# aclike/dynamic_multiview_3d

Measured on AMD Instinct MI355X. Metric: train images/sec, appearance-flow encoder-decoder 128x128x3 (fwd+bwd+Adam), higher is better.
Workload: dtype bf16x3; 1 GPU; appflow_offset: AppearanceFlowModel 128x128x3, batch 64 per GPU, Adam lr 1e-4, random-init weights (reference initialisers); global_batch=64, parallelism=dp1

## Files before the change

dynamic_multiview_3d_amd/_lib.py:

```python
import ctypes as C
import os

HERE = os.path.dirname(os.path.abspath(__file__))
LIB_PATH = os.environ.get("MV3D_LIB") or os.path.join(HERE, "libmv3d_hip.so")

ACT_NONE, ACT_LRELU, ACT_RELU, ACT_TANH = 0, 1, 2, 3
ACT_BY_NAME = {None: ACT_NONE, 'none': ACT_NONE, 'lrelu': ACT_LRELU, 'relu': ACT_RELU, 'tanh': ACT_TANH}
F32 = 0


class ConvGeom(C.Structure):
    _fields_ = [(n, C.c_int32) for n in
                ("N", "H", "W", "C", "Ho", "Wo", "K", "kh", "kw", "sh", "sw", "img_ld", "feat_ld", "dtype")]


class Epilogue(C.Structure):
    _fields_ = [("bias", C.c_void_p), ("act", C.c_int32), ("leak", C.c_float), ("gmask_act", C.c_int32),
                ("gmask_leak", C.c_float), ("gmask_ref", C.c_void_p), ("gmask_ld", C.c_int32)]


class FcChainLayer(C.Structure):
    _fields_ = [("M", C.c_void_p), ("bias", C.c_void_p), ("y", C.c_void_p), ("y_ld", C.c_int32), ("out", C.c_int32),
                ("act", C.c_int32), ("leak", C.c_float)]


class FcChain(C.Structure):
    _fields_ = [("B", C.c_int32), ("nlayers", C.c_int32), ("in_", C.c_int32), ("x_ld", C.c_int32), ("x", C.c_void_p),
                ("l", FcChainLayer * 4)]


class Mv3dError(RuntimeError):
    pass


_vp, _i, _i64, _f, _sz = C.c_void_p, C.c_int, C.c_int64, C.c_float, C.c_size_t
_G, _E = C.POINTER(ConvGeom), C.POINTER(Epilogue)

STATUS_FUNCS = {
    "mv3d_conv2d_fwd": [_G, _vp, _vp, _vp, _E, _vp, _sz, _vp],
    "mv3d_conv2d_dgrad": [_G, _vp, _vp, _vp, _E, _vp, _sz, _vp],
    "mv3d_conv2d_wgrad": [_G, _vp, _vp, _vp, _vp, _vp, _sz, _vp],
    "mv3d_deconv2d_fwd": [_G, _vp, _vp, _vp, _E, _vp, _sz, _vp],
    "mv3d_deconv2d_dgrad": [_G, _vp, _vp, _vp, _E, _vp, _sz, _vp],
    "mv3d_deconv2d_wgrad": [_G, _vp, _vp, _vp, _vp, _sz, _vp],
    "mv3d_fc_fwd": [_i, _i, _i, _vp, _i, _vp, _vp, _i, _E, _vp, _sz, _vp],
    "mv3d_fc_dgrad": [_i, _i, _i, _vp, _i, _vp, _vp, _i, _E, _vp, _sz, _vp],
    "mv3d_fc_wgrad": [_i, _i, _i, _vp, _i, _vp, _i, _vp, _vp, _vp, _sz, _vp],
    "mv3d_fc_wgrad_dgrad": [_i, _i, _i, _vp, _i, _vp, _i, _vp, _vp, _vp, _vp, _i, _E, _vp, _sz, _vp],
    "mv3d_fc_chain_fwd": [C.POINTER(FcChain), _vp],
    "mv3d_act_fwd": [_i64, _i, _vp, _i, _vp, _i, _i, _f, _vp],
    "mv3d_act_bwd": [_i64, _i, _vp, _i, _vp, _i, _vp, _i, _i, _f, _vp],
    "mv3d_copy2d": [_i64, _i, _vp, _i64, _i64, _vp, _i64, _i, _vp],
    "mv3d_group_sum": [_i64, _i, _i, _vp, _i64, _vp, _i64, _vp],
    "mv3d_warp_resample_fwd": [_i, _i, _i, _i, _i, _i, _vp, _vp, _i, _vp, _vp, _vp],
    "mv3d_warp_resample_bwd": [_i, _i, _i, _i, _i, _i, _vp, _vp, _i, _vp, _vp, _i, _vp],
    "mv3d_warp_resample_loss": [_i, _i, _i, _i, _i, _i, _vp, _vp, _i, _vp, _i, _i, _f, _vp, _vp, _vp, _i, _vp, _vp],
    "mv3d_resampler_fwd": [_i, _i, _i, _i, _i, _vp, _i, _vp, _i, _vp, _i, _vp],
    "mv3d_resampler_bwd": [_i, _i, _i, _i, _i, _vp, _i, _vp, _i, _vp, _i, _vp, _i, _vp, _i, _vp, _sz, _vp],
    "mv3d_image_metrics": [_i, _i, _i, _i, _vp, _i, _vp, _i, _f, _vp, _vp, _sz, _vp],
    "mv3d_ssim_loss": [_i, _i, _i, _i, _vp, _i, _vp, _i, _f, _f, _vp, _vp, _i, _i, _vp, _sz, _vp],
    "mv3d_flow_smoothness": [_i, _i, _i, _vp, _i, _vp, _i, _i, _f, _f, _f, _vp, _vp, _i, _i, _vp, _sz, _vp],
    "mv3d_pixel_loss": [_i64, _i, _vp, _vp, _vp, _i, _f, _vp, _vp, _vp],
    "mv3d_loss_overwrite_next": [],
    "mv3d_pixel_loss_strided": [_i64, _i, _vp, _i, _vp, _i, _f, _vp, _i, _i, _f, _vp, _vp, _i, _vp],
    "mv3d_tfrecord_open": [C.c_char_p, _i, C.POINTER(_vp)],
    "mv3d_tfrecord_read": [_vp, _i, _i, _i, C.POINTER(C.c_char_p), C.POINTER(C.c_int), C.POINTER(C.c_size_t), C.POINTER(_vp), C.POINTER(C.c_int)],
    "mv3d_u8_to_unit_f32": [_i64, _vp, _vp, _vp],
    "mv3d_u8_process_image": [_vp, _i, _i, _i, _i, _vp, _i, _i, _vp],
    "mv3d_fill": [_vp, _i64, _f, _vp],
    "mv3d_adam_step": [_i64, _vp, _vp, _vp, _vp, _f, _f, _f, _f, _f, _f, _f, _vp],
    "mv3d_adam_step_dev": [_i64, _vp, _vp, _vp, _vp, _vp, _i, C.POINTER(_i64), C.POINTER(_i64), _vp],
    "mv3d_adam_advance": [_vp, _vp],
    "mv3d_fc_wgrad_adam": [_i, _i, _i, _vp, _i, _vp, _i, _vp, _vp, _vp, _vp, _vp, _vp],
    "mv3d_sgd_step": [_i64, _vp, _vp, _vp, _f, _f, _i, _f, _vp],
    "mv3d_sgd_step_dev": [_i64, _vp, _vp, _vp, _vp, _i, C.POINTER(_i64), C.POINTER(_i64), _vp],
    "mv3d_fc_wgrad_sgd": [_i, _i, _i, _vp, _i, _vp, _i, _vp, _vp, _vp, _vp, _vp],
    "mv3d_grad_finalize_begin": [],
    "mv3d_grad_finalize_add": [_vp, _i64],
    "mv3d_grad_finalize_commit": [_vp, _sz, _vp, _vp, _vp, _vp, _vp, _vp],
    "mv3d_grad_finalize_commit_sgd": [_vp, _sz, _vp, _vp, _vp, _vp, _vp],
    "mv3d_grad_finalize_abort": [],
    "mv3d_comm_unique_id": [_vp],
    "mv3d_comm_init": [C.POINTER(_vp), _i, _i, _vp],
    "mv3d_comm_destroy": [_vp],
    "mv3d_comm_allreduce_sum": [_vp, _vp, _i64, _vp],
    "mv3d_comm_reduce_scatter_sum": [_vp, _vp, _vp, _i64, _vp],
    "mv3d_comm_allgather": [_vp, _vp, _vp, _i64, _vp],
    "mv3d_ipc_export": [_vp, _vp, C.POINTER(_i64)],
    "mv3d_ipc_open": [_vp, C.POINTER(_vp)],
    "mv3d_ipc_close": [_vp],
    "mv3d_mesh_reduce_sum": [C.POINTER(_vp), _i, _vp, _i64, _vp],
    "mv3d_mesh_copy": [_vp, _vp, _i64, _vp],
    "mv3d_filter_cache_bind": [_G, _i, _vp, _vp, _sz],
    "mv3d_filter_cache_commit": [_vp, _sz, _vp],
    "mv3d_filter_cache_refresh": [_vp],
    "mv3d_filter_cache_clear": [],
    "mv3d_plan_begin": [_vp],
    "mv3d_plan_end": [],
    "mv3d_plan_run": [_vp, _vp],
    "mv3d_plan_run_range": [_vp, _i, _i, _vp],
    "mv3d_plan_run_range_multi": [_vp, _i, _i, _vp, C.POINTER(_vp), _i, _i],
    "mv3d_plan_side": [_i],
    "mv3d_plan_profile": [_vp, _i],
    "mv3d_plan_profile_collect": [_vp],
    "mv3d_plan_profile_select": [_vp, C.c_char_p],
    "mv3d_plan_profile_reset": [_vp],
    "mv3d_plan_op_info": [_vp, _i, C.POINTER(C.c_char_p), C.POINTER(C.c_double), C.POINTER(C.c_double),
                          C.POINTER(C.c_double), C.POINTER(C.c_int)],
}
OTHER_FUNCS = {
    "mv3d_version": (C.c_char_p, []),
    "mv3d_last_error": (C.c_char_p, []),
    "mv3d_conv_workspace_bytes": (_sz, [_G]),
    "mv3d_conv_wgrad_workspace_bytes": (_sz, [_G]),
    "mv3d_fc_workspace_bytes": (_sz, [_i, _i, _i]),
    "mv3d_resampler_bwd_workspace_bytes": (_sz, [_i, _i, _i, _i, _i]),
    "mv3d_image_metrics_workspace_bytes": (_sz, [_i, _i, _i, _i]),
    "mv3d_ssim_loss_workspace_bytes": (_sz, [_i, _i, _i, _i]),
    "mv3d_flow_smoothness_workspace_bytes": (_sz, [_i, _i, _i]),
    "mv3d_crc32c": (C.c_uint32, [_vp, _sz]),
    "mv3d_set_diagnostics": (C.c_int, [_i]),
    "mv3d_set_wgrad_cus": (C.c_int, [_i]),
    "mv3d_tfrecord_close": (None, [_vp]),
    "mv3d_filter_prepared_bytes": (_sz, [_G, _i]),
    "mv3d_filter_cache_table_bytes": (_sz, []),
    "mv3d_grad_finalize_table_bytes": (_sz, []),
    "mv3d_plan_create": (_vp, []),
    "mv3d_plan_destroy": (None, [_vp]),
    "mv3d_plan_size": (_i, [_vp]),
    "mv3d_comm_available": (_i, []),
    "mv3d_fc_wgrad_adam_supported": (_i, [_i, _i, _i, _i, _i]),
    "mv3d_debug_cconv_stamps": (_i, [_vp, _sz]),
    "mv3d_debug_cwgrad_stamps": (_i, [_vp, _sz]),
    "mv3d_debug_band_stamps": (_i, [_vp, _sz]),
}
EXPORTS = sorted(list(STATUS_FUNCS) + list(OTHER_FUNCS))

_lib = None


class _Checked:

    def __init__(self, name, fn, dll):
        self.name, self.fn, self.dll = name, fn, dll

    def __call__(self, *args):
        rc = self.fn(*args)
        if rc != 0:
            raise Mv3dError("%s failed (%d): %s" % (self.name, rc, self.dll.mv3d_last_error().decode()))
        return rc


class _Lib:
    def __init__(self, path):
        if not os.path.exists(path):
            raise Mv3dError("%s not found: build it with `python -m dynamic_multiview_3d_amd.build` "
                            "(hipcc --offload-arch=gfx950); there is no fallback path" % path)
        import torch
        self.dll = C.CDLL(path)
        for name, (res, args) in OTHER_FUNCS.items():
            fn = getattr(self.dll, name)
            fn.restype, fn.argtypes = res, args
            if name[5:] != 'last_error':
                setattr(self, name[5:], fn)
        for name, args in STATUS_FUNCS.items():
            fn = getattr(self.dll, name)
            fn.restype, fn.argtypes = C.c_int, args
            setattr(self, name[5:], _Checked(name, fn, self.dll))
            setattr(self, "raw_" + name[5:], fn)

    def last_error(self):
        return self.dll.mv3d_last_error().decode()


def lib():
    global _lib
    if _lib is None:
        _lib = _Lib(LIB_PATH)
    return _lib


def plan_ops(plan):
    l = lib()
    out = []
    for i in range(l.plan_size(plan)):
        name, fl, by, ms, runs = C.c_char_p(), C.c_double(), C.c_double(), C.c_double(), C.c_int()
        l.plan_op_info(plan, i, C.byref(name), C.byref(fl), C.byref(by), C.byref(ms), C.byref(runs))
        out.append((name.value.decode(), fl.value, by.value, ms.value, runs.value))
    return out


def epilogue(bias=None, act=ACT_NONE, leak=0.2, gmask_act=ACT_NONE, gmask_leak=0.2, gmask_ref=None, gmask_ld=0):
    return Epilogue(bias, act, leak, gmask_act, gmask_leak, gmask_ref, gmask_ld)


def conv_geom(N, H, W, Cc, K, kh, kw, sh, sw, img_ld=None, feat_ld=None):
    Ho, Wo = -(-H // sh), -(-W // sw)
    return ConvGeom(N, H, W, Cc, Ho, Wo, K, kh, kw, sh, sw, Cc if img_ld is None else img_ld,
                    K if feat_ld is None else feat_ld, F32)
```

dynamic_multiview_3d_amd/csrc/common.h:

```cpp
#pragma once
#include <hip/hip_runtime.h>
#include <stdint.h>
#include <stdlib.h>
#include <functional>
#include "../../include/mv3d_hip.h"

namespace mv3d {

int fail(int code, const char* fmt, ...) __attribute__((format(printf, 2, 3)));
struct OpInfo {
    const char* name;
    double flops;
    double bytes;
};

const char* intern_label(const char* fmt, ...) __attribute__((format(printf, 1, 2)));

bool recording();
bool take_loss_overwrite();
void record(std::function<int(hipStream_t)> fn, const OpInfo& info);

enum OptKind { OPT_NONE = 0, OPT_ADAM = 1, OPT_MOMENTUM = 2, OPT_GD = 3 };

__device__ __forceinline__ void momentum_elem(float g, float& p, float& a, float lr, float mu, bool nesterov) {
#pragma clang fp contract(off)
    a = a * mu + g;
    if (nesterov) p = p - (g * lr + (a * mu) * lr);
    else p = p - a * lr;
}
__device__ __forceinline__ void gd_elem(float g, float& p, float lr) {
#pragma clang fp contract(off)
    p = p - g * lr;
}

template <class F>
inline int dispatch(void* stream, const OpInfo& info, F fn) {
    if (recording()) { record(std::function<int(hipStream_t)>(fn), info); return MV3D_OK; }
    return fn(reinterpret_cast<hipStream_t>(stream));
}

inline int launched(const char* what) {
    hipError_t e = hipGetLastError();
    if (e != hipSuccess) return fail(MV3D_E_HIP, "%s: %s", what, hipGetErrorString(e));
    return MV3D_OK;
}

struct FinSegHost { const float* part; int nslab; int64_t count; float* out; };
bool finalize_collecting();
void finalize_push(const float* part, int nslab, int64_t count, float* out);
void finalize_open();
}
#include <vector>
namespace mv3d {
const std::vector<FinSegHost>* finalize_peek();
void finalize_take(std::vector<FinSegHost>* out);

int disabled_paths();

static inline int cdiv(int a, int b) { return (a + b - 1) / b; }
static inline int64_t cdiv64(int64_t a, int64_t b) { return (a + b - 1) / b; }

static inline void same_pad(int size, int k, int s, int* out, int* before) {
    int o = (size + s - 1) / s;
    int total = (o - 1) * s + k - size;
    if (total < 0) total = 0;
    *out = o;
    *before = total / 2;
}

__device__ __forceinline__ float act_apply(float x, int act, float leak) {
    if (act == MV3D_ACT_LRELU) {
        float f1 = 0.5f * (1.0f + leak), f2 = 0.5f * (1.0f - leak);
        return __fadd_rn(__fmul_rn(f1, x), __fmul_rn(f2, fabsf(x)));
    }
    if (act == MV3D_ACT_RELU) {
        float y = __fadd_rn(__fmul_rn(0.5f, x), __fmul_rn(0.5f, fabsf(x)));
        return x < 0.0f ? -0.0f : y;
    }
    if (act == MV3D_ACT_TANH) return tanhf(x);
    return x;
}

__device__ __forceinline__ float act_grad_from_out(float y, int act, float leak) {
    if (act == MV3D_ACT_LRELU) {
        float f1 = 0.5f * (1.0f + leak), f2 = 0.5f * (1.0f - leak);
        float s = (y > 0.0f) ? 1.0f : ((y < 0.0f) ? -1.0f : 0.0f);
        return f1 + f2 * s;
    }
    if (act == MV3D_ACT_RELU) {
        if (y > 0.0f) return 1.0f;
        return (__float_as_uint(y) >> 31) ? 0.0f : 0.5f;
    }
    if (act == MV3D_ACT_TANH) return 1.0f - y * y;
    return 1.0f;
}

typedef float f32x16 __attribute__((ext_vector_type(16)));
typedef float f32x4 __attribute__((ext_vector_type(4)));

}
```

dynamic_multiview_3d_amd/csrc/conv.hip:

```cpp
#include "conv_common.h"
#include "reduce_common.h"
#include <algorithm>

namespace mv3d {

template <int WM, int MT, int NT, bool VEC, bool BKMAJOR>
__global__ __launch_bounds__(256) void igemm_kernel(const IgemmParams p) {
    constexpr int BK = 32;
    constexpr int WN = 4 / WM;
    constexpr int BM = WM * 32 * MT;
    constexpr int BN = WN * 32 * NT;
    constexpr int LDA = BK + 1;
    constexpr int LDB = BN + 1;
    constexpr int A_PASSES = VEC ? BM / 32 : BM / 8;
    constexpr int B_LOADS = BK * BN / 256;

    __shared__ float As[BM * LDA];
    __shared__ float Bs[BK * LDB];
    __shared__ int s_rowbase[BM], s_ih0[BM], s_iw0[BM], s_outpix[BM];

    const int tid = threadIdx.x;
    const int lane = tid & 63, wave = tid >> 6;
    const int li = lane & 31, lh = lane >> 5;
    const int wm = wave / WN, wn = wave % WN;
// ... 1225 lines not shown
            return dispatch(stream, OpInfo{"igemm_splitk_epilogue", 0.0, (double)total * 4.0 * (e.ksplit + 1)}, [=](hipStream_t s) {
                launch_splitk_epilogue(e, blocks, s);
                return launched("igemm_splitk_epilogue");
            });
        }
        if (hrc != 1) return hrc;
    }
    int cfg; dim3 grid;
    size_t need = igemm_plan(p, &cfg, &grid);
    if (need > ws_bytes || (need && !ws)) {
        p.ksplit = 1;
        grid.z = p.so_h * p.so_w;
        need = 0;
    }
    p.Part = (float*)ws;
    int rc = dispatch(stream, OpInfo{igemm_name(cfg, vec, bkmajor), flops, bytes}, [=](hipStream_t s) {
        if (cfg == 0) launch_igemm_cfg<4, 1, 1>(p, vec, bkmajor, grid, s);
        else if (cfg == 1) launch_igemm_cfg<4, 1, 2>(p, vec, bkmajor, grid, s);
        else launch_igemm_cfg<2, 1, 1>(p, vec, bkmajor, grid, s);
        return launched(who);
    });
    if (rc != MV3D_OK || p.ksplit == 1) return rc;
    const int64_t total = (int64_t)p.N * p.Hc * p.Wc * p.Cc;
    const int blocks = (int)std::min<int64_t>(cdiv64(total, 256), 4096);
    return dispatch(stream, OpInfo{"igemm_splitk_epilogue", 0.0, (double)total * 4.0 * (p.ksplit + 1)}, [=](hipStream_t s) {
        launch_splitk_epilogue(p, blocks, s);
        return launched("igemm_splitk_epilogue");
    });
}

static inline double conv_flops(const mv3d_conv_geom* g) {
    return 2.0 * g->N * g->Ho * g->Wo * g->kh * g->kw * (double)g->C * g->K;
}
static inline double conv_bytes(const mv3d_conv_geom* g) {
    return 4.0 * ((double)g->N * g->H * g->W * g->C + (double)g->N * g->Ho * g->Wo * g->K + (double)g->kh * g->kw * g->C * g->K);
}

static void i2f_params(const mv3d_conv_geom* g, IgemmParams& p, int* pt_out, int* pl_out) {
    int ho, wo, pt, pl;
    same_pad(g->H, g->kh, g->sh, &ho, &pt);
    same_pad(g->W, g->kw, g->sw, &wo, &pl);
    p.N = g->N; p.Ha = g->H; p.Wa = g->W; p.Ca = g->C; p.a_ld = g->img_ld;
    p.Hc = g->Ho; p.Wc = g->Wo; p.Cc = g->K; p.c_ld = g->feat_ld;
    p.sa_h = g->sh; p.sa_w = g->sw; p.so_h = 1; p.so_w = 1;
    p.Hp[0] = g->Ho; p.Wp[0] = g->Wo; p.Hp[1] = 0; p.Wp[1] = 0;
    p.fold = (g->C < 16 && g->img_ld == g->C && g->kw > 1) ? 1 : 0;
    int nt = 0;
    if (p.fold) {
        for (int pp = 0; pp < g->kh; ++pp) { p.taps[nt].dh = (int8_t)(pp - pt); p.taps[nt].dw = (int8_t)(-pl); p.taps[nt].widx = (int16_t)(pp * g->kw); ++nt; }
        p.Ka = g->kw * g->C;
    } else {
        for (int pp = 0; pp < g->kh; ++pp)
            for (int q = 0; q < g->kw; ++q) { p.taps[nt].dh = (int8_t)(pp - pt); p.taps[nt].dw = (int8_t)(q - pl); p.taps[nt].widx = (int16_t)(pp * g->kw + q); ++nt; }
        p.Ka = g->C;
    }
    p.tap_begin[0] = 0; p.tap_begin[1] = nt;
    p.w_tap_stride = g->C * g->K; p.w_ks = g->K; p.w_ns = 1;
    *pt_out = pt; *pl_out = pl;
}

static int img2feat(const mv3d_conv_geom* g, const void* img, const void* w, void* feat, const mv3d_epilogue* epi,
                    void* ws, size_t ws_bytes, void* stream, const char* who) {
    int rc = check_geom(g, who);
    if (rc == MV3D_OK) rc = check_epilogue(epi, who);
    if (rc != MV3D_OK) return rc;
    if (!img || !w || !feat) return fail(MV3D_E_INVAL, "%s: null tensor pointer", who);
    IgemmParams p = {};
    int pt, pl;
    i2f_params(g, p, &pt, &pl);
    p.A = (const float*)img; p.Wt = (const float*)w; p.Out = (float*)feat;
    fill_epilogue(p, epi);
    if (p.fold && g->C <= 4 && !(disabled_paths() & 64)) {
        const int brc = try_smallc_band(g, p, pt, pl, img, w, feat, stream, who, conv_flops(g), conv_bytes(g));
        if (brc != 1) return brc;
    }
    if (p.fold && g->C <= 4 && g->kw * g->C <= 20 && g->K <= 64 && !(disabled_paths() & 64)) {
        SmallCParams q = {};
        q.X = (const float*)img; q.Wt = (const float*)w; q.Y = (float*)feat;
        q.N = g->N; q.H = g->H; q.W = g->W; q.C = g->C; q.Ho = g->Ho; q.Wo = g->Wo; q.K = g->K; q.y_ld = g->feat_ld;
        q.kh = g->kh; q.kw = g->kw; q.sh = g->sh; q.sw = g->sw; q.pt = pt; q.pl = pl;
        q.wtiles = cdiv(g->Wo, 32);
        q.ep = p;
        const int items = g->N * g->Ho * q.wtiles;
        const bool two = g->K > 32;
        return dispatch(stream, OpInfo{two ? "smallc_img2feat<N64>" : "smallc_img2feat<N32>", conv_flops(g), conv_bytes(g)}, [=](hipStream_t s) {
            const bool b3 = !(disabled_paths() & 4096) && q.kw * q.C <= 16 && (q.kh == 5 || q.kh == 3) && !two;
            if (b3) {
                static int sc_blocks = -1;
                if (sc_blocks < 0) { const char* e = getenv("MV3D_SC_BLOCKS"); sc_blocks = e ? atoi(e) : 2048; }
                const int blocks = std::min(cdiv(items, 4), sc_blocks);
                auto pow2 = [](int v) { return v > 0 && (v & (v - 1)) == 0; };
                const bool lean = !(disabled_paths() & 8388608) && q.ep.gact == MV3D_ACT_NONE && q.Wo % 32 == 0 && q.K == 32 && pow2(q.wtiles) && pow2(q.Ho) &&
                                  (int64_t)q.N * q.H * q.W * q.C * 4 < 0x40000000 && (int64_t)q.N * q.Ho * q.Wo * q.y_ld * 4 < 0x7fffffff;
                if (lean) {
                    int ws_ = 0, hs_ = 0;
                    while ((1 << ws_) < q.wtiles) ++ws_;
                    while ((1 << hs_) < q.Ho) ++hs_;
                    if (q.kh == 5) smallc_b3s_kernel<5><<<blocks, 256, 0, s>>>(q, items, ws_, hs_);
                    else smallc_b3s_kernel<3><<<blocks, 256, 0, s>>>(q, items, ws_, hs_);
                } else if (q.kh == 5) smallc_b3_kernel<1, 5><<<blocks, 256, 0, s>>>(q, items);
                else smallc_b3_kernel<1, 3><<<blocks, 256, 0, s>>>(q, items);
            } else if (two) smallc_img2feat_kernel<2><<<cdiv(items, 4), 256, 0, s>>>(q);
            else smallc_img2feat_kernel<1><<<cdiv(items, 4), 256, 0, s>>>(q);
            return launched(who);
        });
    }
    return run_igemm(p, ws, ws_bytes, stream, who, conv_flops(g), conv_bytes(g));
}

static void f2i_params(const mv3d_conv_geom* g, IgemmParams& p) {
    int ho, wo, pt, pl;
    same_pad(g->H, g->kh, g->sh, &ho, &pt);
    same_pad(g->W, g->kw, g->sw, &wo, &pl);
    p.N = g->N; p.Ha = g->Ho; p.Wa = g->Wo; p.Ca = g->K; p.a_ld = g->feat_ld;
    p.Hc = g->H; p.Wc = g->W; p.Cc = g->C; p.c_ld = g->img_ld;
    p.sa_h = 1; p.sa_w = 1; p.so_h = g->sh; p.so_w = g->sw;
    for (int a = 0; a < 2; ++a) {
        p.Hp[a] = a < g->sh ? (g->H - a + g->sh - 1) / g->sh : 0;
        p.Wp[a] = a < g->sw ? (g->W - a + g->sw - 1) / g->sw : 0;
    }
    int nt = 0;
    for (int phh = 0; phh < g->sh; ++phh)
        for (int phw = 0; phw < g->sw; ++phw) {
            p.tap_begin[phh * g->sw + phw] = nt;
            const int p0 = (phh + pt) % g->sh, q0 = (phw + pl) % g->sw;
            for (int pp = p0; pp < g->kh; pp += g->sh)
                for (int q = q0; q < g->kw; q += g->sw) {
                    p.taps[nt].dh = (int8_t)((phh + pt - pp) / g->sh);
                    p.taps[nt].dw = (int8_t)((phw + pl - q) / g->sw);
                    p.taps[nt].widx = (int16_t)(pp * g->kw + q);
                    ++nt;
                }
        }
    p.tap_begin[g->sh * g->sw] = nt;
    p.fold = 0; p.Ka = g->K;
    p.w_tap_stride = g->C * g->K; p.w_ks = 1; p.w_ns = g->K;
}

static int feat2img(const mv3d_conv_geom* g, const void* feat, const void* w, void* img, const mv3d_epilogue* epi,
                    void* ws, size_t ws_bytes, void* stream, const char* who) {
    int rc = check_geom(g, who);
    if (rc == MV3D_OK) rc = check_epilogue(epi, who);
    if (rc != MV3D_OK) return rc;
    if (!img || !w || !feat) return fail(MV3D_E_INVAL, "%s: null tensor pointer", who);
    IgemmParams p = {};
    f2i_params(g, p);
    p.A = (const float*)feat; p.Wt = (const float*)w; p.Out = (float*)img;
    fill_epilogue(p, epi);
    return run_igemm(p, ws, ws_bytes, stream, who, conv_flops(g), conv_bytes(g));
}

struct WgTileParams;
bool wgrad_tile_plan(const mv3d_conv_geom* g, struct WgTileParams* out, int* nslab_out, int* cfg_out, size_t* lds_out);
int wgrad_tile_launch_erased(const mv3d_conv_geom* g, const void* img, const void* feat, void* out, void* bias_out, void* stream, const char* who, int* nslab_out);

static void filtgrad_plan(const mv3d_conv_geom* g, FiltgradParams& p, int* nt_out, int* nslab_out) {
    int ho, wo;
    same_pad(g->H, g->kh, g->sh, &ho, &p.pt);
    same_pad(g->W, g->kw, g->sw, &wo, &p.pl);
    p.N = g->N; p.H = g->H; p.W = g->W; p.C = g->C; p.img_ld = g->img_ld;
    p.Ho = g->Ho; p.Wo = g->Wo; p.K = g->K; p.feat_ld = g->feat_ld;
    p.kw = g->kw; p.sh = g->sh; p.sw = g->sw;
    p.fold = (g->C < 16 && g->img_ld == g->C && g->kw > 1) ? 1 : 0;
    p.Cf = p.fold ? g->kw * g->C : g->C;
    p.ntap = p.fold ? g->kh : g->kh * g->kw;
    const int NT = (g->K > 32) ? 2 : 1;
    p.ctiles = cdiv(p.Cf, 32);
    p.ktiles = cdiv(g->K, 32 * NT);
    p.rows_total = g->N * g->Ho;
    const int items = p.ctiles * p.ktiles * p.ntap;
    const int blocks_x = cdiv(items, 4);
    int nslab = cdiv(2048, blocks_x);
    if (nslab > p.rows_total) nslab = p.rows_total;
    int min_rows = cdiv(128, g->Wo);
    if (nslab > cdiv(p.rows_total, min_rows)) nslab = cdiv(p.rows_total, min_rows);
    if (nslab < 1) nslab = 1;
    p.rows_per_slab = cdiv(p.rows_total, nslab);
    nslab = cdiv(p.rows_total, p.rows_per_slab);
    *nt_out = NT;
    *nslab_out = nslab;
}

int wgrad_tile_nslab(const mv3d_conv_geom* g);
int set_wgrad_cus(int cus);

static size_t filtgrad_ws_bytes(const mv3d_conv_geom* g) {
    {
        const int tw = thin_wgrad_slabs(g);
        if (tw > 0) return (size_t)tw * ((size_t)g->kh * g->kw * g->C * g->K + g->K) * sizeof(float);
    }
    {
        ThinFgParams tp; int ns; size_t lds;
        if (thin_filtgrad_plan(g, tp, &ns, &lds)) return (size_t)ns * ((size_t)g->kh * g->kw * g->C * g->K + g->K) * sizeof(float);
    }
    FiltgradParams p = {};
    int NT, nslab;
    filtgrad_plan(g, p, &NT, &nslab);
    const int tiled = wgrad_tile_nslab(g);
    if (tiled > 0) nslab = tiled;
    if (nslab == 1) return 0;
    return (size_t)nslab * ((size_t)g->kh * g->kw * g->C * g->K + g->K) * sizeof(float);
}

static int filtgrad(const mv3d_conv_geom* g, const void* img, const void* feat, void* df, void* db,
                    void* ws, size_t ws_bytes, void* stream, const char* who) {
    int rc = check_geom(g, who);
    if (rc != MV3D_OK) return rc;
    if (!img || !feat || !df) return fail(MV3D_E_INVAL, "%s: null tensor pointer", who);
    const int64_t fcount = (int64_t)g->kh * g->kw * g->C * g->K;
    float* dfp = (float*)df; float* dbp = (float*)db;
    const int K = g->K;
    {
        const int tiled = wgrad_tile_nslab(g);
        if (tiled > 0 && (reinterpret_cast<uintptr_t>(img) & 15) == 0 && (reinterpret_cast<uintptr_t>(feat) & 15) == 0) {
            float* part = dfp; float* bpart = dbp;
            if (tiled > 1) {
                size_t need = (size_t)tiled * (fcount + K) * sizeof(float);
                if (!ws || ws_bytes < need) return fail(MV3D_E_WORKSPACE, "%s: workspace %zu < %zu bytes", who, ws_bytes, need);
                part = (float*)ws;
                bpart = db ? (float*)ws + (int64_t)tiled * fcount : nullptr;
            }
            int ns = 0;
            rc = wgrad_tile_launch_erased(g, img, feat, part, bpart, stream, who, &ns);
            if (rc == MV3D_OK && ns == 1 && finalize_collecting()) { finalize_push(nullptr, 0, fcount, dfp); if (dbp) finalize_push(nullptr, 0, K, dbp); }
            if (rc != MV3D_OK || ns == 1) return rc;
            return dispatch_reduce(stream, part, ns, fcount, dfp, bpart, K, dbp);
        }
    }
    {
        const int tw = thin_wgrad_slabs(g);
        if (tw > 0 && (reinterpret_cast<uintptr_t>(img) & 15) == 0) {
            const size_t need = (size_t)tw * (fcount + K) * sizeof(float);
            if (!ws || ws_bytes < need) return fail(MV3D_E_WORKSPACE, "%s: workspace %zu < %zu bytes", who, ws_bytes, need);
            float* part = (float*)ws;
            float* bpart = db ? (float*)ws + (int64_t)tw * fcount : nullptr;
            rc = thin_wgrad_launch(g, img, feat, part, bpart, stream, who, conv_flops(g), conv_bytes(g));
            if (rc == MV3D_OK) return dispatch_reduce(stream, part, tw, fcount, dfp, bpart, K, dbp);
            if (rc != 1) return rc;
        }
    }
    {
        ThinFgParams tp; int ns; size_t lds;
        if (thin_filtgrad_plan(g, tp, &ns, &lds) && (reinterpret_cast<uintptr_t>(feat) & 15) == 0) {
            const size_t need = (size_t)ns * (fcount + K) * sizeof(float);
            if (!ws || ws_bytes < need) return fail(MV3D_E_WORKSPACE, "%s: workspace %zu < %zu bytes", who, ws_bytes, need);
            tp.img = (const float*)img; tp.feat = (const float*)feat;
            tp.out = (float*)ws;
            tp.bias_out = db ? (float*)ws + (int64_t)ns * fcount : nullptr;
            dim3 grid(cdiv(g->K, 32), ns);
            const int nj = cdiv(tp.nrows, 16);
            rc = dispatch(stream, OpInfo{"thin_filtgrad", conv_flops(g), conv_bytes(g)}, [=](hipStream_t s) {
                if (nj <= 2) thin_filtgrad_kernel<2><<<grid, 256, lds, s>>>(tp);
                else if (nj <= 4) thin_filtgrad_kernel<4><<<grid, 256, lds, s>>>(tp);
                else if (nj <= 5) thin_filtgrad_kernel<5><<<grid, 256, lds, s>>>(tp);
                else thin_filtgrad_kernel<7><<<grid, 256, lds, s>>>(tp);
                return launched(who);
            });
            if (rc != MV3D_OK) return rc;
            return dispatch_reduce(stream, tp.out, ns, fcount, dfp, tp.bias_out, K, dbp);
        }
    }
    FiltgradParams p = {};
    int NT, nslab;
    filtgrad_plan(g, p, &NT, &nslab);
    p.img = (const float*)img; p.feat = (const float*)feat;
    if (nslab > 1) {
        size_t need = (size_t)nslab * (fcount + g->K) * sizeof(float);
        if (!ws || ws_bytes < need) return fail(MV3D_E_WORKSPACE, "%s: workspace %zu < %zu bytes", who, ws_bytes, need);
        p.out = (float*)ws;
        p.bias_out = db ? (float*)ws + (int64_t)nslab * fcount : nullptr;
    } else {
        p.out = (float*)df;
        p.bias_out = (float*)db;
    }
    dim3 grid(cdiv(p.ctiles * p.ktiles * p.ntap, 4), nslab);
    rc = dispatch(stream, OpInfo{NT == 2 ? "filtgrad<NT=2>" : "filtgrad<NT=1>", conv_flops(g), conv_bytes(g)}, [=](hipStream_t s) {
        const bool wide = p.Wo >= 16;
        if (NT == 2) { if (wide) filtgrad_kernel<2, 8><<<grid, 256, 0, s>>>(p); else filtgrad_kernel<2, 2><<<grid, 256, 0, s>>>(p); }
        else { if (wide) filtgrad_kernel<1, 8><<<grid, 256, 0, s>>>(p); else filtgrad_kernel<1, 2><<<grid, 256, 0, s>>>(p); }
        return launched(who);
    });
    if (rc == MV3D_OK && nslab == 1 && finalize_collecting()) { finalize_push(nullptr, 0, fcount, dfp); if (dbp) finalize_push(nullptr, 0, K, dbp); }
    if (rc != MV3D_OK || nslab == 1) return rc;
    return dispatch_reduce(stream, p.out, nslab, fcount, dfp, p.bias_out, K, dbp);
}

}

using namespace mv3d;

extern "C" {

int mv3d_conv2d_fwd(const mv3d_conv_geom* g, const void* x, const void* w, void* y, const mv3d_epilogue* epi,
                    void* ws, size_t wsb, void* stream) {
    return img2feat(g, x, w, y, epi, ws, wsb, stream, "mv3d_conv2d_fwd");
}
int mv3d_conv2d_dgrad(const mv3d_conv_geom* g, const void* dy, const void* w, void* dx, const mv3d_epilogue* epi,
                      void* ws, size_t wsb, void* stream) {
    return feat2img(g, dy, w, dx, epi, ws, wsb, stream, "mv3d_conv2d_dgrad");
}
int mv3d_conv2d_wgrad(const mv3d_conv_geom* g, const void* x, const void* dy, void* dw, void* db,
                      void* ws, size_t wsb, void* stream) {
    return filtgrad(g, x, dy, dw, db, ws, wsb, stream, "mv3d_conv2d_wgrad");
}
int mv3d_deconv2d_fwd(const mv3d_conv_geom* g, const void* x, const void* w, void* y, const mv3d_epilogue* epi,
                      void* ws, size_t wsb, void* stream) {
    return feat2img(g, x, w, y, epi, ws, wsb, stream, "mv3d_deconv2d_fwd");
}
int mv3d_deconv2d_dgrad(const mv3d_conv_geom* g, const void* dy, const void* w, void* dx, const mv3d_epilogue* epi,
                        void* ws, size_t wsb, void* stream) {
    return img2feat(g, dy, w, dx, epi, ws, wsb, stream, "mv3d_deconv2d_dgrad");
}
int mv3d_deconv2d_wgrad(const mv3d_conv_geom* g, const void* x, const void* dy, void* dw, void* ws, size_t wsb, void* stream) {
    return filtgrad(g, dy, x, dw, nullptr, ws, wsb, stream, "mv3d_deconv2d_wgrad");
}

static bool filter_op_params(const mv3d_conv_geom* g, int op, const void* w, IgemmParams& p, const char* who) {
    if (!g || check_geom(g, who) != MV3D_OK) return false;
    if (op == MV3D_FILTER_CONV_FWD || op == MV3D_FILTER_DECONV_DGRAD) { int pt, pl; i2f_params(g, p, &pt, &pl); }
    else if (op == MV3D_FILTER_CONV_DGRAD || op == MV3D_FILTER_DECONV_FWD) f2i_params(g, p);
    else { fail(MV3D_E_INVAL, "%s: unknown filter operation %d", who, op); return false; }
    p.Wt = (const float*)w;
    return true;
}

size_t mv3d_filter_prepared_bytes(const mv3d_conv_geom* g, int op) {
    IgemmParams p = {};
    if (!filter_op_params(g, op, nullptr, p, "mv3d_filter_prepared_bytes")) return 0;
    if (disabled_paths() & (1 | 4096)) return 0;
    return bconv_prepared_bytes(p);
}

int mv3d_filter_cache_bind(const mv3d_conv_geom* g, int op, const void* w, void* prepared, size_t prepared_bytes) {
    IgemmParams p = {};
    if (!w) return fail(MV3D_E_INVAL, "mv3d_filter_cache_bind: null filter pointer");
    if (!filter_op_params(g, op, w, p, "mv3d_filter_cache_bind")) return MV3D_E_INVAL;
    int rc = bconv_cache_bind(p, prepared, prepared_bytes);
    if (rc == 1) return fail(MV3D_E_UNSUPPORTED, "mv3d_filter_cache_bind: this operation does not take a prepared filter");
    return rc;
}

int mv3d_set_wgrad_cus(int cus) { return set_wgrad_cus(cus); }

size_t mv3d_conv_wgrad_workspace_bytes(const mv3d_conv_geom* g) {
    if (!g || check_geom(g, "mv3d_conv_wgrad_workspace_bytes") != MV3D_OK) return 0;
    return filtgrad_ws_bytes(g);
}

size_t mv3d_conv_workspace_bytes(const mv3d_conv_geom* g) {
    if (!g || check_geom(g, "mv3d_conv_workspace_bytes") != MV3D_OK) return 0;
    size_t out_img = (size_t)g->N * g->H * g->W * g->C, out_feat = (size_t)g->N * g->Ho * g->Wo * g->K;
    size_t big = out_img > out_feat ? out_img : out_feat;
    size_t igemm = 0;
    {
        IgemmParams p = {};
        int cfg; dim3 grid;
        p.N = g->N; p.Hc = g->Ho; p.Wc = g->Wo; p.Cc = g->K; p.so_h = p.so_w = 1; p.Hp[0] = g->Ho; p.Wp[0] = g->Wo;
        const bool fold = (g->C < 16 && g->img_ld == g->C && g->kw > 1);
        p.Ka = fold ? g->kw * g->C : g->C; p.tap_begin[0] = 0; p.tap_begin[1] = fold ? g->kh : g->kh * g->kw;
        size_t a = igemm_plan(p, &cfg, &grid);
        igemm = a;
        (void)big;
        IgemmParams q = {};
        q.N = g->N; q.Hc = g->H; q.Wc = g->W; q.Cc = g->C; q.so_h = g->sh; q.so_w = g->sw;
        for (int i = 0; i < 2; ++i) { q.Hp[i] = i < g->sh ? (g->H - i + g->sh - 1) / g->sh : 0; q.Wp[i] = i < g->sw ? (g->W - i + g->sw - 1) / g->sw : 0; }
        q.Ka = g->K;
        int ho, wo, pt, pl;
        same_pad(g->H, g->kh, g->sh, &ho, &pt);
        same_pad(g->W, g->kw, g->sw, &wo, &pl);
        int nt = 0;
        for (int phh = 0; phh < g->sh; ++phh)
            for (int phw = 0; phw < g->sw; ++phw) {
                q.tap_begin[phh * g->sw + phw] = nt;
                for (int pp = (phh + pt) % g->sh; pp < g->kh; pp += g->sh)
                    for (int qq = (phw + pl) % g->sw; qq < g->kw; qq += g->sw) ++nt;
            }
        q.tap_begin[g->sh * g->sw] = nt;
        size_t b = igemm_plan(q, &cfg, &grid);
        if (b > igemm) igemm = b;
    }
    size_t fg = filtgrad_ws_bytes(g);
    size_t filt = (size_t)g->kh * g->kw * ((g->C + 63) / 64 * 64) * ((g->K + 63) / 64 * 64) * sizeof(float);
    size_t m = igemm > fg ? igemm : fg;
    const size_t big_out = out_img > out_feat ? out_img : out_feat;
    size_t small = 0;
    if ((size_t)g->Ho * g->Wo <= 64 || (size_t)g->H * g->W <= 64) small = ((filt + 255) & ~(size_t)255) + 16 * big_out * sizeof(float);
    m = m > small ? m : small;
    return m > filt ? m : filt;
}

static void fc_geom(mv3d_conv_geom& g, int B, int in, int out, int x_ld, int y_ld) {
    g.N = 1; g.H = 1; g.W = B; g.C = in; g.Ho = 1; g.Wo = B; g.K = out;
    g.kh = g.kw = g.sh = g.sw = 1; g.img_ld = x_ld; g.feat_ld = y_ld; g.dtype = MV3D_F32;
}
int mv3d_fc_fwd(int B, int in, int out, const void* x, int x_ld, const void* M, void* y, int y_ld,
                const mv3d_epilogue* epi, void* ws, size_t wsb, void* stream) {
    mv3d_conv_geom g; fc_geom(g, B, in, out, x_ld, y_ld);
    if (B > 0 && in > 0 && out > 0 && x && M && y && is_small_fc(B, in, out)) {
        int rc = check_epilogue(epi, "mv3d_fc_fwd");
        if (rc != MV3D_OK) return rc;
        IgemmParams ep = {}; fill_epilogue(ep, epi);
        return dispatch(stream, OpInfo{"small_fc_fwd", 2.0 * B * in * out, 4.0 * (B * in + in * out + B * out)}, [=](hipStream_t s) {
            small_fc_fwd_kernel<<<cdiv(B * out, 256), 256, 0, s>>>(B, in, out, (const float*)x, x_ld, (const float*)M, (float*)y, y_ld, ep);
            return launched("small_fc_fwd_kernel");
        });
    }
    if (B > 0 && in > 0 && out > 0 && x && M && y && x_ld >= in && y_ld >= out && check_epilogue(epi, "mv3d_fc_fwd") == MV3D_OK) {
        int rc = try_fc_stream(false, B, in, out, x, x_ld, M, y, y_ld, epi, ws, wsb, stream, "mv3d_fc_fwd", fill_epilogue, launch_splitk_epilogue);
        if (rc != 1) return rc;
    }
    return img2feat(&g, x, M, y, epi, ws, wsb, stream, "mv3d_fc_fwd");
}
int mv3d_fc_dgrad(int B, int in, int out, const void* dy, int dy_ld, const void* M, void* dx, int dx_ld,
                  const mv3d_epilogue* epi, void* ws, size_t wsb, void* stream) {
    mv3d_conv_geom g; fc_geom(g, B, in, out, dx_ld, dy_ld);
    if (B > 0 && in > 0 && out > 0 && dy && M && dx && is_small_fc(B, in, out)) {
        int rc = check_epilogue(epi, "mv3d_fc_dgrad");
        if (rc != MV3D_OK) return rc;
        IgemmParams ep = {}; fill_epilogue(ep, epi);
        return dispatch(stream, OpInfo{"small_fc_dgrad", 2.0 * B * in * out, 4.0 * (B * in + in * out + B * out)}, [=](hipStream_t s) {
            small_fc_dgrad_kernel<<<cdiv(B * in, 256), 256, 0, s>>>(B, in, out, (const float*)dy, dy_ld, (const float*)M, (float*)dx, dx_ld, ep);
            return launched("small_fc_dgrad_kernel");
        });
    }
    if (B > 0 && in > 0 && out > 0 && dy && M && dx && dy_ld >= out && dx_ld >= in && check_epilogue(epi, "mv3d_fc_dgrad") == MV3D_OK) {
        int rc = try_fc_stream(true, B, in, out, dy, dy_ld, M, dx, dx_ld, epi, ws, wsb, stream, "mv3d_fc_dgrad", fill_epilogue, launch_splitk_epilogue);
        if (rc != 1) return rc;
    }
    return feat2img(&g, dy, M, dx, epi, ws, wsb, stream, "mv3d_fc_dgrad");
}
int mv3d_fc_wgrad(int B, int in, int out, const void* x, int x_ld, const void* dy, int dy_ld, void* dM, void* db,
                  void* ws, size_t wsb, void* stream) {
    mv3d_conv_geom g; fc_geom(g, B, in, out, x_ld, dy_ld);
    if (B > 0 && in > 0 && out > 0 && x && dy && dM && is_small_fc(B, in, out)) {
        return dispatch(stream, OpInfo{"small_fc_wgrad", 2.0 * B * in * out, 4.0 * (B * in + in * out + B * out)}, [=](hipStream_t s) {
            small_fc_wgrad_kernel<<<cdiv((in + 1) * out, 256), 256, 0, s>>>(B, in, out, (const float*)x, x_ld, (const float*)dy, dy_ld, (float*)dM, (float*)db);
            return launched("small_fc_wgrad_kernel");
        });
    }
    if (B > 0 && in > 0 && out > 0 && x && dy && dM && x_ld >= in && dy_ld >= out) {
        int rc = try_fc_wgrad(B, in, out, x, x_ld, dy, dy_ld, dM, db, stream, "mv3d_fc_wgrad");
        if (rc != 1) return rc;
    }
    return filtgrad(&g, x, dy, dM, db, ws, wsb, stream, "mv3d_fc_wgrad");
}
int mv3d_fc_wgrad_dgrad(int B, int in, int out, const void* x, int x_ld, const void* dy, int dy_ld, const void* M,
                        void* dM, void* db, void* dx, int dx_ld, const mv3d_epilogue* dx_epi, void* ws, size_t wsb, void* stream) {
    if (B > 0 && in > 0 && out > 0 && x && dy && M && dM && dx && is_small_fc(B, in, out)) {
        int rc = check_epilogue(dx_epi, "mv3d_fc_wgrad_dgrad");
        if (rc != MV3D_OK) return rc;
        IgemmParams ep = {}; fill_epilogue(ep, dx_epi);
        const int wblocks = cdiv((in + 1) * out, 256), dblocks = cdiv(B * in, 256);
        const size_t lds = ((size_t)B * out + std::max((size_t)B * in, (size_t)in * (out + 1))) * sizeof(float);
        if (lds <= 64 * 1024) {
            (void)hipFuncSetAttribute(reinterpret_cast<const void*>(&small_fc_bwd_kernel), hipFuncAttributeMaxDynamicSharedMemorySize, 64 * 1024);
            (void)hipGetLastError();
        }
        if (lds <= 64 * 1024)
        return dispatch(stream, OpInfo{"small_fc_bwd", 4.0 * B * in * out, 4.0 * (2.0 * B * in + 2.0 * in * out + 2.0 * B * out)}, [=](hipStream_t s) {
            small_fc_bwd_kernel<<<wblocks + dblocks, 256, lds, s>>>(B, in, out, (const float*)x, x_ld, (const float*)dy, dy_ld, (const float*)M,
                                                                  (float*)dM, (float*)db, (float*)dx, dx_ld, ep, wblocks);
            return launched("small_fc_bwd_kernel");
        });
    }
    int rc = mv3d_fc_wgrad(B, in, out, x, x_ld, dy, dy_ld, dM, db, ws, wsb, stream);
    if (rc != MV3D_OK) return rc;
    return mv3d_fc_dgrad(B, in, out, dy, dy_ld, M, dx, dx_ld, dx_epi, ws, wsb, stream);
// ... 60 lines not shown
```

dynamic_multiview_3d_amd/csrc/core.hip:

```cpp
#include "common.h"
#include <atomic>
#include <cstdlib>
#include <stdarg.h>
#include <stdio.h>
#include <string.h>
#include <vector>
#include <mutex>
#include <set>
#include <string>

struct PlanOp {
    std::function<int(hipStream_t)> fn;
    mv3d::OpInfo info;
    double total_ms;
    int runs;
    bool selected = true;
    int side = 0;
};

struct mv3d_plan {
    std::vector<PlanOp> ops;
    bool profile = false;
    std::vector<hipEvent_t> pool;
    size_t used = 0;
    hipEvent_t fork[MV3D_MAX_SIDE] = {}, join[MV3D_MAX_SIDE] = {};
    bool pass_open = false;
};

namespace mv3d {

static std::atomic<int> g_disabled{-1};
int disabled_paths() {
    int v = g_disabled.load(std::memory_order_relaxed);
    if (v < 0) {
        const char* e = getenv("MV3D_DISABLE");
        v = e ? atoi(e) : 0;
        g_disabled.store(v, std::memory_order_relaxed);
    }
    return v;
}

static thread_local char g_err[512] = "";
static thread_local mv3d_plan* g_rec = nullptr;
static thread_local int g_side = 0;

int fail(int code, const char* fmt, ...) {
    va_list ap;
    va_start(ap, fmt);
    vsnprintf(g_err, sizeof(g_err), fmt, ap);
    va_end(ap);
    return code;
}
const char* intern_label(const char* fmt, ...) {
    char buf[128];
    va_list ap;
    va_start(ap, fmt);
    vsnprintf(buf, sizeof(buf), fmt, ap);
    va_end(ap);
    static std::mutex mu;
    static std::set<std::string>* labels = new std::set<std::string>();
    std::lock_guard<std::mutex> lk(mu);
    return labels->insert(buf).first->c_str();
}
static thread_local std::vector<FinSegHost>* g_fin = nullptr;
bool finalize_collecting() { return g_fin != nullptr; }
void finalize_open() { if (!g_fin) g_fin = new std::vector<FinSegHost>(); }
void finalize_push(const float* part, int nslab, int64_t count, float* out) { if (g_fin) g_fin->push_back(FinSegHost{part, nslab, count, out}); }
const std::vector<FinSegHost>* finalize_peek() { return g_fin; }
void finalize_take(std::vector<FinSegHost>* out) {
    if (!g_fin) return;
    if (out) out->swap(*g_fin);
    delete g_fin;
    g_fin = nullptr;
}
bool recording() { return g_rec != nullptr; }
void record(std::function<int(hipStream_t)> fn, const OpInfo& info) { g_rec->ops.push_back(PlanOp{std::move(fn), info, 0.0, 0, true, g_side}); }
}

extern "C" {

const char* mv3d_version(void) { return "mv3d_hip 0.3 (gfx950, split-bf16 / fp32 MFMA)"; }
const char* mv3d_last_error(void) { return mv3d::g_err; }

mv3d_plan* mv3d_plan_create(void) { return new mv3d_plan(); }
void mv3d_plan_destroy(mv3d_plan* p) {
    if (!p) return;
    if (mv3d::g_rec == p) mv3d::g_rec = nullptr;
    for (hipEvent_t e : p->pool) (void)hipEventDestroy(e);
    for (int k = 0; k < MV3D_MAX_SIDE; ++k) {
        if (p->fork[k]) (void)hipEventDestroy(p->fork[k]);
        if (p->join[k]) (void)hipEventDestroy(p->join[k]);
    }
    delete p;
}
int mv3d_plan_begin(mv3d_plan* p) {
    if (!p) return mv3d::fail(MV3D_E_INVAL, "mv3d_plan_begin: null plan");
    if (mv3d::g_rec) return mv3d::fail(MV3D_E_INVAL, "mv3d_plan_begin: a plan is already recording on this thread");
    p->ops.clear();
    p->used = 0;
    mv3d::g_rec = p;
    mv3d::g_side = 0;
    return MV3D_OK;
}
int mv3d_plan_side(int side) {
    if (side < 0 || side > MV3D_MAX_SIDE) return mv3d::fail(MV3D_E_INVAL, "mv3d_plan_side: side %d not in [0, %d]", side, MV3D_MAX_SIDE);
    mv3d::g_side = side;
    return MV3D_OK;
}
int mv3d_plan_end(void) {
    if (!mv3d::g_rec) return mv3d::fail(MV3D_E_INVAL, "mv3d_plan_end: nothing is recording");
    mv3d::g_rec = nullptr;
    return MV3D_OK;
}
int mv3d_plan_size(const mv3d_plan* p) { return p ? (int)p->ops.size() : 0; }

int mv3d_plan_run_range(mv3d_plan* p, int begin, int end, void* stream) {
    return mv3d_plan_run_range_multi(p, begin, end, stream, nullptr, 0, 0);
}

int mv3d_plan_run_range_multi(mv3d_plan* p, int begin, int end, void* stream, void* const* side_streams, int nside, int flags) {
    if (!p) return mv3d::fail(MV3D_E_INVAL, "mv3d_plan_run_range: null plan");
    if (mv3d::g_rec) return mv3d::fail(MV3D_E_INVAL, "mv3d_plan_run_range: cannot run while recording");
    const int n = (int)p->ops.size();
    if (begin < 0 || end > n || begin > end) return mv3d::fail(MV3D_E_INVAL, "mv3d_plan_run_range: bad range [%d, %d) of %d", begin, end, n);
    if (nside < 0 || nside > MV3D_MAX_SIDE || (nside > 0 && !side_streams)) return mv3d::fail(MV3D_E_INVAL, "mv3d_plan_run_range_multi: bad side stream list");
    hipStream_t s = reinterpret_cast<hipStream_t>(stream);
    for (int k = 0; k < nside; ++k)
        if (!p->fork[k]) {
            if (hipEventCreateWithFlags(&p->fork[k], hipEventDisableTiming) != hipSuccess ||
                hipEventCreateWithFlags(&p->join[k], hipEventDisableTiming) != hipSuccess)
                return mv3d::fail(MV3D_E_HIP, "mv3d_plan_run_range_multi: hipEventCreate failed");
        }
    int prev_side = 0;
    bool used[MV3D_MAX_SIDE] = {};
    auto stream_of = [&](int i) -> hipStream_t {
        const int tag = p->ops[i].side;
        const int sd = (nside > 0 && tag > 0) ? 1 + (tag - 1) % nside : 0;
        hipStream_t so = sd ? reinterpret_cast<hipStream_t>(side_streams[sd - 1]) : s;
        if (sd && so == s) { prev_side = 0; return s; }
        if (sd && sd != prev_side) {
            (void)hipEventRecord(p->fork[sd - 1], s);
            (void)hipStreamWaitEvent(so, p->fork[sd - 1], 0);
            used[sd - 1] = true;
        }
        prev_side = sd;
        return so;
    };
    auto join = [&]() {
        if (flags & MV3D_RUN_NO_JOIN) return;
        for (int k = 0; k < nside; ++k)
            if (used[k]) {
                (void)hipEventRecord(p->join[k], reinterpret_cast<hipStream_t>(side_streams[k]));
                (void)hipStreamWaitEvent(s, p->join[k], 0);
            }
    };
    if (!p->profile) {
        for (int i = begin; i < end; ++i) {
            int rc = p->ops[i].fn(stream_of(i));
            if (rc != MV3D_OK) return rc;
        }
        join();
        return MV3D_OK;
    }
    const size_t need = p->used + 2 * (size_t)n;
    while (p->pool.size() < need) {
        hipEvent_t e;
        if (hipEventCreate(&e) != hipSuccess) return mv3d::fail(MV3D_E_HIP, "mv3d_plan_run: hipEventCreate failed");
        p->pool.push_back(e);
    }
    if (!p->pass_open) {
        for (int i = 0; i < begin; ++i)
            if (p->ops[i].selected) { (void)hipEventRecord(p->pool[p->used + 2 * i], s); (void)hipEventRecord(p->pool[p->used + 2 * i + 1], s); }
        p->pass_open = true;
    }
    for (int i = begin; i < end; ++i) {
        const bool sel = p->ops[i].selected;
        hipStream_t so = stream_of(i);
        if (sel) (void)hipEventRecord(p->pool[p->used + 2 * i], so);
        int rc = p->ops[i].fn(so);
        if (sel) (void)hipEventRecord(p->pool[p->used + 2 * i + 1], so);
        if (rc != MV3D_OK) return rc;
    }
    join();
    if (end == n) { p->used = need; p->pass_open = false; }
    return MV3D_OK;
}

int mv3d_plan_run(mv3d_plan* p, void* stream) {
    if (!p) return mv3d::fail(MV3D_E_INVAL, "mv3d_plan_run: null plan");
    return mv3d_plan_run_range(p, 0, (int)p->ops.size(), stream);
}

int mv3d_plan_profile(mv3d_plan* p, int enable) {
    if (!p) return mv3d::fail(MV3D_E_INVAL, "mv3d_plan_profile: null plan");
    p->profile = enable != 0;
    return MV3D_OK;
}

int mv3d_plan_profile_collect(mv3d_plan* p) {
    if (!p) return mv3d::fail(MV3D_E_INVAL, "mv3d_plan_profile_collect: null plan");
    const size_t n = p->ops.size();
    if (n == 0 || p->used == 0) return MV3D_OK;
    size_t last = n;
    for (size_t i = 0; i < n; ++i) if (p->ops[i].selected) last = i;
    if (last == n) { p->used = 0; return MV3D_OK; }
    if (hipEventSynchronize(p->pool[p->used - 2 * n + 2 * last + 1]) != hipSuccess)
        return mv3d::fail(MV3D_E_HIP, "mv3d_plan_profile_collect: hipEventSynchronize failed");
    for (size_t base = 0; base + 2 * n <= p->used; base += 2 * n)
        for (size_t i = 0; i < n; ++i) {
            if (!p->ops[i].selected) continue;
            float ms = 0.f;
            if (hipEventElapsedTime(&ms, p->pool[base + 2 * i], p->pool[base + 2 * i + 1]) == hipSuccess) {
                p->ops[i].total_ms += ms;
                p->ops[i].runs += 1;
            }
        }
    p->used = 0;
    (void)hipGetLastError();
    return MV3D_OK;
}

static bool label_matches(const char* label, const char* pats) {
    const size_t ll = strlen(label);
    for (const char* p = pats; *p;) {
        const char* e = strchr(p, '|');
        size_t n = e ? (size_t)(e - p) : strlen(p);
        if (n > 0 && p[n - 1] == '*') { if (ll >= n - 1 && strncmp(label, p, n - 1) == 0) return true; }
        else if (ll == n && strncmp(label, p, n) == 0) return true;
        p += n + (e ? 1 : 0);
    }
    return false;
}

int mv3d_plan_profile_select(mv3d_plan* p, const char* name) {
    if (!p) return mv3d::fail(MV3D_E_INVAL, "mv3d_plan_profile_select: null plan");
    if (p->used) return mv3d::fail(MV3D_E_INVAL, "mv3d_plan_profile_select: collect pending runs first");
    for (auto& o : p->ops) o.selected = (name == nullptr) || label_matches(o.info.name, name);
    return MV3D_OK;
}

int mv3d_plan_profile_reset(mv3d_plan* p) {
    if (!p) return mv3d::fail(MV3D_E_INVAL, "mv3d_plan_profile_reset: null plan");
    for (auto& o : p->ops) { o.total_ms = 0.0; o.runs = 0; }
    p->used = 0;
    return MV3D_OK;
}

int mv3d_set_diagnostics(int mask) {
    const int old = mv3d::disabled_paths();
    mv3d::g_disabled.store(mask < 0 ? 0 : mask, std::memory_order_relaxed);
    return old;
}

uint32_t mv3d_crc32c(const void* data, size_t n) {
    static uint32_t T[8][256];
    static bool ready = false;
    if (!ready) {
        for (uint32_t i = 0; i < 256; ++i) {
            uint32_t c = i;
            for (int k = 0; k < 8; ++k) c = (c & 1) ? (c >> 1) ^ 0x82F63B78u : c >> 1;
            T[0][i] = c;
        }
        for (uint32_t i = 0; i < 256; ++i)
            for (int t = 1; t < 8; ++t) T[t][i] = (T[t - 1][i] >> 8) ^ T[0][T[t - 1][i] & 0xFF];
// ... 29 lines not shown
```

dynamic_multiview_3d_amd/csrc/elem.hip:

```cpp
#include "common.h"
#include "reduce_common.h"
#include <vector>
#include <algorithm>
#include <cstdlib>
#include <atomic>

namespace mv3d {

constexpr int LOSS_ROWS = 32, LOSS_MAXB = 1024;
__device__ unsigned g_loss_part[LOSS_ROWS][LOSS_MAXB];
__device__ unsigned g_loss_ticket[LOSS_ROWS];

static thread_local bool g_loss_overwrite = false;
bool take_loss_overwrite() {
    const bool v = g_loss_overwrite;
    g_loss_overwrite = false;
    return v;
}
static int next_loss_row() {
    static std::atomic<unsigned> n{0};
    const int flag = take_loss_overwrite() ? 256 : 0;
    return (int)(n.fetch_add(1) % LOSS_ROWS) | flag;
}

// ... 679 lines not shown
    });
}

int mv3d_sgd_step(int64_t count, void* p, const void* g, void* accum, float lr, float momentum, int use_nesterov, float grad_scale,
                  void* stream) {
    if (count <= 0 || !p || !g) return fail(MV3D_E_INVAL, "mv3d_sgd_step: bad arguments");
    if (((uintptr_t)p | (uintptr_t)g | (uintptr_t)accum) & 15) return fail(MV3D_E_INVAL, "mv3d_sgd_step: buffers must be 16-byte aligned");
    if (!accum && (momentum != 0.0f || use_nesterov))
        return fail(MV3D_E_INVAL, "mv3d_sgd_step: momentum / use_nesterov need the accumulator (accum == NULL is gradient descent)");
    const bool mom = accum != nullptr;
    const int nest = use_nesterov ? 1 : 0;
    const int blocks = (int)std::min<int64_t>(cdiv64(count / 4 + 1, 256), 4096);
    return dispatch(stream, OpInfo{mom ? "momentum" : "sgd", 0.0, (mom ? 20.0 : 12.0) * count}, [=](hipStream_t s) {
        if (mom) sgd_kernel<true><<<blocks, 256, 0, s>>>(count, (float*)p, (const float*)g, (float*)accum, lr, momentum, nest, grad_scale);
        else sgd_kernel<false><<<blocks, 256, 0, s>>>(count, (float*)p, (const float*)g, nullptr, lr, 0.0f, 0, grad_scale);
        return launched("sgd_kernel");
    });
}

int mv3d_sgd_step_dev(int64_t count, void* p, const void* g, void* accum, const void* sgd_state, int nskip, const int64_t* skip_lo,
                      const int64_t* skip_hi, void* stream) {
    if (count <= 0 || (count & 3) || !p || !g || !sgd_state) return fail(MV3D_E_INVAL, "mv3d_sgd_step_dev: bad arguments (count must be a multiple of 4)");
    if (((uintptr_t)p | (uintptr_t)g | (uintptr_t)accum) & 15) return fail(MV3D_E_INVAL, "mv3d_sgd_step_dev: buffers must be 16-byte aligned");
    AdamSkips sk;
    int64_t skipped;
    if (int rc = parse_skips("mv3d_sgd_step_dev", count, nskip, skip_lo, skip_hi, sk, skipped)) return rc;
    const bool mom = accum != nullptr;
    const int blocks = (int)std::min<int64_t>(cdiv64((count - skipped) / 4 + 1, 256), 4096);
    return dispatch(stream, OpInfo{mom ? "momentum" : "sgd", 0.0, (mom ? 20.0 : 12.0) * (count - skipped)}, [=](hipStream_t s) {
        if (mom) sgd_dev_kernel<true><<<blocks, 256, 0, s>>>(count, (float*)p, (const float*)g, (float*)accum, (const float*)sgd_state, sk);
        else sgd_dev_kernel<false><<<blocks, 256, 0, s>>>(count, (float*)p, (const float*)g, nullptr, (const float*)sgd_state, sk);
        return launched("sgd_dev_kernel");
    });
}

int mv3d_act_fwd(int64_t rows, int ch, const void* x, int x_ld, void* y, int y_ld, int act, float leak, void* stream) {
    if (rows <= 0 || ch <= 0 || !x || !y || x_ld < ch || y_ld < ch) return fail(MV3D_E_INVAL, "mv3d_act_fwd: bad arguments");
    return dispatch(stream, OpInfo{"act_fwd", 0.0, 8.0 * rows * ch}, [=](hipStream_t s) {
        act_fwd_kernel<<<grid_for(rows * ch), 256, 0, s>>>(rows, ch, (const float*)x, x_ld, (float*)y, y_ld, act, leak);
        return launched("act_fwd_kernel");
    });
}

int mv3d_act_bwd(int64_t rows, int ch, const void* dy, int dy_ld, const void* ref, int ref_ld, void* dx, int dx_ld,
                 int act, float leak, void* stream) {
    if (rows <= 0 || ch <= 0 || !dy || !ref || !dx || dy_ld < ch || ref_ld < ch || dx_ld < ch) return fail(MV3D_E_INVAL, "mv3d_act_bwd: bad arguments");
    return dispatch(stream, OpInfo{"act_bwd", 0.0, 12.0 * rows * ch}, [=](hipStream_t s) {
        act_bwd_kernel<<<grid_for(rows * ch), 256, 0, s>>>(rows, ch, (const float*)dy, dy_ld, (const float*)ref, ref_ld, (float*)dx, dx_ld, act, leak);
        return launched("act_bwd_kernel");
    });
}

int mv3d_copy2d(int64_t rows, int ch, const void* src, int64_t src_ld, int64_t src_row_div, void* dst, int64_t dst_ld,
                int accumulate, void* stream) {
    if (rows <= 0 || ch <= 0 || !src || !dst || src_row_div < 1) return fail(MV3D_E_INVAL, "mv3d_copy2d: bad arguments");
    return dispatch(stream, OpInfo{"copy2d", 0.0, 8.0 * rows * ch}, [=](hipStream_t s) {
        copy2d_kernel<<<grid_for(rows * ch), 256, 0, s>>>(rows, ch, (const float*)src, src_ld, src_row_div, (float*)dst, dst_ld, accumulate);
        return launched("copy2d_kernel");
    });
}

int mv3d_group_sum(int64_t groups, int group, int ch, const void* src, int64_t src_ld, void* dst, int64_t dst_ld, void* stream) {
    if (groups <= 0 || group <= 0 || ch <= 0 || !src || !dst) return fail(MV3D_E_INVAL, "mv3d_group_sum: bad arguments");
    return dispatch(stream, OpInfo{"group_sum", 0.0, 4.0 * groups * ch * (group + 1)}, [=](hipStream_t s) {
        group_sum_kernel<<<grid_for(groups * ch), 256, 0, s>>>(groups, group, ch, (const float*)src, src_ld, (float*)dst, dst_ld);
        return launched("group_sum_kernel");
    });
}

int mv3d_loss_overwrite_next(void) { g_loss_overwrite = true; return MV3D_OK; }

int mv3d_grad_finalize_begin(void) {
    if (finalize_collecting()) return fail(MV3D_E_INVAL, "mv3d_grad_finalize_begin: a collection is already open on this thread");
    finalize_open();
    return MV3D_OK;
}
int mv3d_grad_finalize_add(void* grad, int64_t count) {
    if (!finalize_collecting()) return fail(MV3D_E_INVAL, "mv3d_grad_finalize_add: no open collection");
    if (!grad || count <= 0 || ((uintptr_t)grad & 15)) return fail(MV3D_E_INVAL, "mv3d_grad_finalize_add: bad range (16-byte aligned, count > 0)");
    finalize_push(nullptr, 0, count, (float*)grad);
    return MV3D_OK;
}
int mv3d_grad_finalize_abort(void) { finalize_take(nullptr); return MV3D_OK; }

static int fin_blocks(const FinSegHost& h) {
    if (h.nslab == 0) return (int)cdiv64(cdiv64(h.count, 4), 256);
    const bool vec = h.count % 4 == 0 && ((uintptr_t)h.part & 15) == 0;
    return (int)cdiv64(h.count, vec ? 64 : 16);
}
size_t mv3d_grad_finalize_table_bytes(void) {
    const std::vector<FinSegHost>* v = finalize_peek();
    if (!v) return 0;
    size_t blocks = 0;
    for (const FinSegHost& h : *v) blocks += fin_blocks(h);
    return ((v->size() * sizeof(FinSeg) + 255) & ~(size_t)255) + blocks * sizeof(int);
}
static int grad_finalize_launch(std::vector<FinSegHost>& segs, size_t need, void* table, size_t table_bytes, void* grads, void* params,
                                void* slot1, void* slot2, const void* state, int opt, void* stream) {
    const bool upd = opt != OPT_NONE;
    std::vector<FinSegHost> keep;
    for (size_t a = 0; a < segs.size(); ++a) {
        const FinSegHost& h = segs[a];
        bool dup = false;
        for (size_t b = 0; b < segs.size(); ++b) {
            if (b == a || segs[b].out != h.out) continue;
            if (h.nslab == 0 && (segs[b].nslab > 0 || b < a)) dup = true;
            if (h.nslab > 0 && segs[b].nslab > 0 && b < a) return fail(MV3D_E_INVAL, "mv3d_grad_finalize_commit: two filter gradients write the same range");
        }
        if (!dup && (upd || h.nslab > 0)) keep.push_back(h);
    }
    if (keep.empty()) return MV3D_OK;
    const bool dry = !table && recording();
    if (!dry && (!table || table_bytes < need || ((uintptr_t)table & 15))) return fail(MV3D_E_WORKSPACE, "mv3d_grad_finalize_commit: table %zu < %zu bytes", table_bytes, need);
    std::vector<FinSeg> dev(keep.size());
    std::vector<int> seg_of;
    double bytes = 0.0;
    for (size_t j = 0; j < keep.size(); ++j) {
        const FinSegHost& h = keep[j];
        FinSeg& d = dev[j];
        d.part = h.part; d.out = h.out; d.count = h.count; d.nslab = h.nslab; d.pad = 0;
        d.vec = h.nslab > 0 && h.count % 4 == 0 && ((uintptr_t)h.part & 15) == 0;
        d.off = 0;
        if (upd) {
            const int64_t off = h.out - (float*)grads;
            if (off < 0 || (h.nslab == 0 && (off & 3))) return fail(MV3D_E_INVAL, "mv3d_grad_finalize_commit: segment %zu is not inside the flat gradient buffer", j);
            d.off = off;
        }
        d.blk0 = (int)seg_of.size();
        const int nb = fin_blocks(h);
        seg_of.insert(seg_of.end(), nb, (int)j);
        bytes += 4.0 * h.count * (h.nslab + (opt == OPT_ADAM ? 6 : opt == OPT_MOMENTUM ? 4 : opt == OPT_GD ? 2 : 1));
    }
    const size_t seg_bytes = (dev.size() * sizeof(FinSeg) + 255) & ~(size_t)255;
    if (!dry && (hipMemcpy(table, dev.data(), dev.size() * sizeof(FinSeg), hipMemcpyHostToDevice) != hipSuccess ||
                 hipMemcpy((char*)table + seg_bytes, seg_of.data(), seg_of.size() * sizeof(int), hipMemcpyHostToDevice) != hipSuccess))
        return fail(MV3D_E_HIP, "mv3d_grad_finalize_commit: table upload failed");
    const FinSeg* dsegs = (const FinSeg*)table;
    const int* dmap = (const int*)((char*)table + seg_bytes);
    const int blocks = (int)seg_of.size();
    const char* label = opt == OPT_ADAM ? "grad_finalize_adam" : opt == OPT_MOMENTUM ? "grad_finalize_momentum" : opt == OPT_GD ? "grad_finalize_sgd" : "grad_finalize";
    return dispatch(stream, OpInfo{label, 0.0, bytes}, [=](hipStream_t s) {
        const float* G = (const float*)grads; float* P = (float*)params; const float* st = (const float*)state;
        if (opt == OPT_ADAM) grad_finalize_kernel<OPT_ADAM><<<blocks, 256, 0, s>>>(dsegs, dmap, G, P, (float*)slot1, (float*)slot2, st);
        else if (opt == OPT_MOMENTUM) grad_finalize_kernel<OPT_MOMENTUM><<<blocks, 256, 0, s>>>(dsegs, dmap, G, P, (float*)slot1, nullptr, st);
        else if (opt == OPT_GD) grad_finalize_kernel<OPT_GD><<<blocks, 256, 0, s>>>(dsegs, dmap, G, P, nullptr, nullptr, st);
        else grad_finalize_kernel<OPT_NONE><<<blocks, 256, 0, s>>>(dsegs, dmap, nullptr, nullptr, nullptr, nullptr, nullptr);
        return launched("grad_finalize_kernel");
    });
}

int mv3d_grad_finalize_commit(void* table, size_t table_bytes, void* grads, void* params, void* adam_m, void* adam_v,
                              const void* adam_state, void* stream) {
    if (!finalize_collecting()) return fail(MV3D_E_INVAL, "mv3d_grad_finalize_commit: no open collection");
    const size_t need = mv3d_grad_finalize_table_bytes();
    std::vector<FinSegHost> segs;
    finalize_take(&segs);
    const bool adam = adam_state != nullptr;
    if (adam && (!grads || !params || !adam_m || !adam_v || (((uintptr_t)grads | (uintptr_t)params | (uintptr_t)adam_m | (uintptr_t)adam_v) & 15)))
        return fail(MV3D_E_INVAL, "mv3d_grad_finalize_commit: the optimiser needs the four flat buffers (16-byte aligned)");
    return grad_finalize_launch(segs, need, table, table_bytes, grads, params, adam_m, adam_v, adam_state, adam ? OPT_ADAM : OPT_NONE, stream);
}

int mv3d_grad_finalize_commit_sgd(void* table, size_t table_bytes, void* grads, void* params, void* accum, const void* sgd_state,
                                  void* stream) {
    if (!finalize_collecting()) return fail(MV3D_E_INVAL, "mv3d_grad_finalize_commit_sgd: no open collection");
    const size_t need = mv3d_grad_finalize_table_bytes();
    std::vector<FinSegHost> segs;
    finalize_take(&segs);
    if (!grads || !params || !sgd_state || (((uintptr_t)grads | (uintptr_t)params | (uintptr_t)accum) & 15))
        return fail(MV3D_E_INVAL, "mv3d_grad_finalize_commit_sgd: the optimiser needs the flat gradient, parameter (and momentum) buffers, 16-byte aligned, and the state");
    return grad_finalize_launch(segs, need, table, table_bytes, grads, params, accum, nullptr, sgd_state, accum ? OPT_MOMENTUM : OPT_GD, stream);
}

}
```

dynamic_multiview_3d_amd/csrc/wgrad_tile.hip:

```cpp
#include "conv_common.h"
#include <algorithm>

namespace mv3d {

struct WgTileParams {
    const float* img; const float* feat;
    float* out; float* bias_out;
    int N, H, W, C, img_ld;
    int Ho, Wo, K, feat_ld;
    int sh, sw, pt, pl, kw;
    int TH, TW, tw_shift, tiles_h, tiles_w, HR, HC;
    int TPIX;
    int ntaps, nitems, ipw;
    int IW, PH;
    int ctiles;
    int ntiles_total, tiles_per_slab;
    int b3;
    int inv_hc, tpix8_shift;
    int G, img_shift, HRi, inv_hri;
    int tsplit;
};

__device__ float4 g_zero16[4];

// ... 25 lines not shown
    int offA[TPW], offB[TPW], item_tap[TPW], item_kt[TPW];
    bool item_ok[TPW];
#pragma unroll
    for (int i = 0; i < TPW; ++i) {
        int it = iw * p.ipw + i;
        item_ok[i] = (i < p.ipw) && (it < p.nitems);
        if (it >= p.nitems) it = p.nitems - 1;
        const int tap = it % p.ntaps, kt = it / p.ntaps;
        item_tap[i] = tap; item_kt[i] = kt;
        offA[i] = ((tap / p.kw) * p.HC + (tap % p.kw)) * 32 + lh * p.sw * 32 + li;
        offB[i] = (n_img_rows + kt * p.TPIX + lh) * 32 + li;
    }

    f32x16 acc[TPW];
#pragma unroll
    for (int i = 0; i < TPW; ++i)
#pragma unroll
        for (int r = 0; r < 16; ++r) acc[i][r] = 0.f;
    float sb[NKT];
#pragma unroll
    for (int y = 0; y < NKT; ++y) sb[y] = 0.f;
    const bool do_bias = p.bias_out != nullptr && ct == 0;

    auto stage = [&](int tile, float* buf) {
        int b = tile;
        const int tw_i = b % p.tiles_w; b /= p.tiles_w;
        const int th_i = b % p.tiles_h;
        const int n = b / p.tiles_h;
        const int oh0 = th_i * p.TH, ow0 = tw_i * p.TW;
        const int ih0 = oh0 * p.sh - p.pt, iw0 = ow0 * p.sw - p.pl;
        const int c4 = lane & 7;
        for (int chunk = wave; chunk < n_chunks; chunk += 8) {
            const int row = chunk * 8 + (lane >> 3);
            const float* src = reinterpret_cast<const float*>(g_zero16);
            if (row < n_img_rows) {
                const int hr = row / p.HC, hc = row - hr * p.HC;
                const int ih = ih0 + hr, iwc = iw0 + hc, ch = c0 + c4 * 4;
                if ((unsigned)ih < (unsigned)p.H && (unsigned)iwc < (unsigned)p.W && ch < p.C)
                    src = p.img + (int64_t)((n * p.H + ih) * p.W + iwc) * p.img_ld + ch;
            } else if (row < n_rows) {
                const int j = row - n_img_rows;
                const int kt = j / p.TPIX, q = j - kt * p.TPIX;
                const int oh = oh0 + (q >> p.tw_shift), ow = ow0 + (q & (p.TW - 1)), kk = k0 + kt * 32 + c4 * 4;
                if (oh < p.Ho && ow < p.Wo && kk < p.K)
                    src = p.feat + (int64_t)((n * p.Ho + oh) * p.Wo + ow) * p.feat_ld + kk;
            }
            dma16(src, buf + chunk * 256);
        }
    };

    const int jshift = p.tw_shift - 1;
    const int jmask = (p.TW >> 1) - 1;
    const int strideA = 2 * p.sw * 32, rowA = p.sh * p.HC * 32;
    const int nsteps = (p.TPIX >> 1) / p.PH;
    const int s_begin = ph * nsteps;

    if (tile_begin < tile_end) stage(tile_begin, smem);
    int cur = 0;
    for (int tile = tile_begin; tile < tile_end; ++tile, cur ^= 1) {
        asm volatile("s_waitcnt vmcnt(0)" ::: "memory");
        __syncthreads();
        const float* buf = smem + cur * buf_floats;
        if (tile + 1 < tile_end) stage(tile + 1, smem + (cur ^ 1) * buf_floats);

        float a0[TPW], b0[TPW], a1[TPW], b1[TPW];
        auto ld = [&](float (&a)[TPW], float (&b)[TPW], int s) {
            const float* pa = buf + (s >> jshift) * rowA + (s & jmask) * strideA;
            const float* pb = buf + s * 64;
#pragma unroll
            for (int i = 0; i < TPW; ++i) { a[i] = pa[offA[i]]; b[i] = pb[offB[i]]; }
        };
        auto mma = [&](const float (&a)[TPW], const float (&b)[TPW]) {
#pragma unroll
            for (int i = 0; i < TPW; ++i) acc[i] = __builtin_amdgcn_mfma_f32_32x32x2f32(a[i], b[i], acc[i], 0, 0, 0);
        };
        ld(a0, b0, s_begin);
        for (int s = 0; s < nsteps; s += 2) {
            ld(a1, b1, s_begin + s + 1);
            mma(a0, b0);
            ld(a0, b0, s_begin + ((s + 2) & (nsteps - 1)));
            mma(a1, b1);
        }
        if (do_bias && wave == 0) {
#pragma unroll
            for (int y = 0; y < NKT; ++y) {
                const float* pb = buf + (n_img_rows + y * p.TPIX + lh) * 32 + li;
                float t = 0.f;
                for (int s = 0; s < (p.TPIX >> 1); ++s) t += pb[s * 64];
                sb[y] += t;
            }
        }
    }

    __syncthreads();
    for (int r = 1; r < p.PH; ++r) {
        float* xch = smem + (iw * TPW) * 1024 + lane;
        if (ph == r) {
#pragma unroll
            for (int i = 0; i < TPW; ++i)
#pragma unroll
                for (int q = 0; q < 16; ++q) xch[(i * 16 + q) * 64] = acc[i][q];
        }
        __syncthreads();
        if (ph == 0) {
#pragma unroll
            for (int i = 0; i < TPW; ++i)
#pragma unroll
                for (int q = 0; q < 16; ++q) acc[i][q] += xch[(i * 16 + q) * 64];
        }
        __syncthreads();
    }
    if (ph == 0) {
#pragma unroll
        for (int i = 0; i < TPW; ++i) {
            if (!item_ok[i]) continue;
            float* out = p.out + ((int64_t)slab * p.ntaps + item_tap[i]) * p.C * p.K;
            const int k = k0 + item_kt[i] * 32 + li;
#pragma unroll
            for (int r = 0; r < 16; ++r) {
                const int c = c0 + (r & 3) + 8 * (r >> 2) + 4 * lh;
                if (c < p.C && k < p.K) out[(int64_t)c * p.K + k] = acc[i][r];
            }
        }
    }
    if (do_bias && wave == 0) {
#pragma unroll
        for (int y = 0; y < NKT; ++y) {
            const float s = sb[y] + __shfl_xor(sb[y], 32);
            const int k = k0 + y * 32 + li;
            if (lh == 0 && k < p.K) p.bias_out[(int64_t)slab * p.K + k] = s;
        }
    }
}


typedef __bf16 wbf16x8 __attribute__((ext_vector_type(8)));
typedef __bf16 wbf16x4 __attribute__((ext_vector_type(4)));
typedef short ws16x4 __attribute__((ext_vector_type(4)));

__device__ __forceinline__ void wsplit4(const float4& v, uint2& hi, uint2& lo) {
    wbf16x4 h, l;
    h[0] = (__bf16)v.x; h[1] = (__bf16)v.y; h[2] = (__bf16)v.z; h[3] = (__bf16)v.w;
    l[0] = (__bf16)(v.x - (float)h[0]); l[1] = (__bf16)(v.y - (float)h[1]);
    l[2] = (__bf16)(v.z - (float)h[2]); l[3] = (__bf16)(v.w - (float)h[3]);
    hi = __builtin_bit_cast(uint2, h);
    lo = __builtin_bit_cast(uint2, l);
}

__device__ __forceinline__ uint2 tr_read(const unsigned char* lds_ptr) {
    ws16x4 v = __builtin_amdgcn_ds_read_tr16_b64_v4i16((__attribute__((address_space(3))) ws16x4*)lds_ptr);
    return __builtin_bit_cast(uint2, v);
}

template <int TPW, int NKT, int NI>
__global__ __launch_bounds__(512) void wgrad_b3_kernel(const WgTileParams p) {
    extern __shared__ __attribute__((aligned(16))) unsigned char smb[];
    constexpr int NF = 4;
    const int tid = threadIdx.x;
    const int lane = tid & 63;
    const int wave = __builtin_amdgcn_readfirstlane(tid >> 6);
    const int iw = wave % p.IW;
    const int ph = wave / p.IW;
    const int tg_per_kt = p.IW / NKT;
    const int kt_w = iw / tg_per_kt, tg = iw - kt_w * tg_per_kt;
    const int li = lane & 31, lh = lane >> 5;
    const int ct = blockIdx.x % p.ctiles, kg = blockIdx.x / p.ctiles;
    const int c0 = ct * 32, k0 = kg * 32 * NKT;
    const int slab = blockIdx.y;
    const int tile_begin = slab * p.tiles_per_slab;
    const int tile_end = min(tile_begin + p.tiles_per_slab, p.ntiles_total);

    const int halo_pix = p.HR * p.HC;
    const int img_plane = halo_pix * 64;
    const int feat_plane = p.TPIX * 64;
    const int buf_bytes = 2 * img_plane + 2 * NKT * feat_plane;
    const int HCh = (p.HC + 1) >> 1;

    int tapoff[TPW], item_tap[TPW];
    bool item_ok[TPW];
    const int tg_total = tg_per_kt * p.tsplit, tgi = (int)blockIdx.z * tg_per_kt + tg;
    const int tap_lo = (p.ntaps * tgi) / tg_total, tap_n = (p.ntaps * (tgi + 1)) / tg_total - tap_lo;
#pragma unroll
    for (int i = 0; i < TPW; ++i) {
        int tap = tap_lo + i;
        item_ok[i] = i < tap_n;
        if (tap >= p.ntaps) tap = p.ntaps - 1;
        item_tap[i] = tap;
        const int dh = tap / p.kw, dw = tap - dh * p.kw;
        const int cs = (p.sw == 2) ? (dw & 1) * HCh + (dw >> 1) : dw;
        tapoff[i] = (dh * p.HC + cs) * 64;
    }

    f32x16 acc[TPW];
#pragma unroll
    for (int i = 0; i < TPW; ++i)
#pragma unroll
        for (int r = 0; r < 16; ++r) acc[i][r] = 0.f;

    const int g16 = (lane >> 4) & 1, q = (lane >> 2) & 3, pp = lane & 3;
    const int col_bytes = (16 * g16 + 4 * pp) * 2;

    float4 vi[NI], vf[NF];
    float4 bsum[NF];
#pragma unroll
    for (int j = 0; j < NF; ++j) bsum[j] = make_float4(0.f, 0.f, 0.f, 0.f);
    const bool do_bias = p.bias_out != nullptr && ct == 0 && blockIdx.z == 0;
    const int n_img4 = halo_pix * 8, n_feat4 = p.TPIX * NKT * 8;
    auto fetch = [&](int tile) {
        int b = tile;
        const int tw_i = b % p.tiles_w; b /= p.tiles_w;
        const int th_i = b % p.tiles_h;
        const int n = (b / p.tiles_h) * p.G;
        const int oh0 = th_i * p.TH, ow0 = tw_i * p.TW;
        const int ih0 = oh0 * p.sh - p.pt, iw0 = ow0 * p.sw - p.pl;
#pragma unroll
        for (int j = 0; j < NI; ++j) {
            const int idx = j * 512 + tid;
            const int pix = idx >> 3, c4 = idx & 7;
            const int hrt = (int)(((unsigned)pix * (unsigned)p.inv_hc) >> 20), hc = pix - hrt * p.HC;
            const int gi = p.G > 1 ? (int)(((unsigned)hrt * (unsigned)p.inv_hri) >> 20) : 0;
            const int hr = hrt - gi * p.HRi;
            const int ih = ih0 + hr, iwc = iw0 + hc, ch = c0 + c4 * 4;
            const bool ok = idx < n_img4 && n + gi < p.N && (unsigned)ih < (unsigned)p.H && (unsigned)iwc < (unsigned)p.W && ch < p.C;
            const float* src = ok ? p.img + (int64_t)(((n + gi) * p.H + ih) * p.W + iwc) * p.img_ld + ch : p.img;
            const float4 t4 = *reinterpret_cast<const float4*>(src);
            vi[j] = ok ? t4 : make_float4(0.f, 0.f, 0.f, 0.f);
        }
#pragma unroll
        for (int j = 0; j < NF; ++j) {
            const int idx = j * 512 + tid;
            const int kt = idx >> p.tpix8_shift, rem = idx & ((1 << p.tpix8_shift) - 1);
            const int pq = rem >> 3, c4 = rem & 7;
            const int gi = pq >> p.img_shift, pr = pq & ((1 << p.img_shift) - 1);
            const int oh = oh0 + (pr >> p.tw_shift), ow = ow0 + (pr & (p.TW - 1)), kk = k0 + kt * 32 + c4 * 4;
            const bool ok = idx < n_feat4 && n + gi < p.N && oh < p.Ho && ow < p.Wo && kk < p.K;
            const float* src = ok ? p.feat + (int64_t)(((n + gi) * p.Ho + oh) * p.Wo + ow) * p.feat_ld + kk : p.feat;
            const float4 t4 = *reinterpret_cast<const float4*>(src);
            vf[j] = ok ? t4 : make_float4(0.f, 0.f, 0.f, 0.f);
        }
    };
    auto commit = [&](unsigned char* buf) {
#pragma unroll
        for (int j = 0; j < NI; ++j) {
            const int idx = j * 512 + tid;
            if (idx < n_img4) {
                const int pix = idx >> 3, c4 = idx & 7;
                const int hr = (int)(((unsigned)pix * (unsigned)p.inv_hc) >> 20), hc = pix - hr * p.HC;
                const int cs = (p.sw == 2) ? (hc & 1) * HCh + (hc >> 1) : hc;
                unsigned char* d = buf + (hr * p.HC + cs) * 64 + c4 * 8;
                uint2 hi, lo;
                wsplit4(vi[j], hi, lo);
                *reinterpret_cast<uint2*>(d) = hi;
                *reinterpret_cast<uint2*>(d + img_plane) = lo;
            }
        }
#pragma unroll
        for (int j = 0; j < NF; ++j) {
            const int idx = j * 512 + tid;
            if (idx < n_feat4) {
                const int kt = idx >> p.tpix8_shift, rem = idx & ((1 << p.tpix8_shift) - 1);
                unsigned char* d = buf + 2 * img_plane + kt * 2 * feat_plane + (rem >> 3) * 64 + (rem & 7) * 8;
                uint2 hi, lo;
                wsplit4(vf[j], hi, lo);
                *reinterpret_cast<uint2*>(d) = hi;
                *reinterpret_cast<uint2*>(d + feat_plane) = lo;
                bsum[j].x += vf[j].x; bsum[j].y += vf[j].y; bsum[j].z += vf[j].z; bsum[j].w += vf[j].w;
            }
        }
    };

    const int steps_total = p.TPIX >> 4;
    const int nsteps = steps_total / p.PH;
    const int s_begin = ph * nsteps;

    if (tile_begin < tile_end) { fetch(tile_begin); commit(smb); }
    int cur = 0;
    for (int tile = tile_begin; tile < tile_end; ++tile, cur ^= 1) {
        __syncthreads();
        const unsigned char* buf = smb + cur * buf_bytes;
        const bool has_next = tile + 1 < tile_end;
        if (has_next) fetch(tile + 1);

        const unsigned char* fb = buf + 2 * img_plane + kt_w * 2 * feat_plane + col_bytes;
        for (int s = s_begin; s < s_begin + nsteps; ++s) {
            const int px0 = 16 * s + 8 * lh + q, px1 = px0 + 4;
            const int im = (1 << p.img_shift) - 1;
            const int r0 = px0 & im, r1 = px1 & im;
            const int a0 = (((px0 >> p.img_shift) * p.HRi + (r0 >> p.tw_shift) * p.sh) * p.HC + (r0 & (p.TW - 1))) * 64 + col_bytes;
            const int a1 = (((px1 >> p.img_shift) * p.HRi + (r1 >> p.tw_shift) * p.sh) * p.HC + (r1 & (p.TW - 1))) * 64 + col_bytes;
            const uint2 bh0 = tr_read(fb + px0 * 64), bh1 = tr_read(fb + px1 * 64);
            const uint2 bl0 = tr_read(fb + feat_plane + px0 * 64), bl1 = tr_read(fb + feat_plane + px1 * 64);
            const wbf16x8 bh = __builtin_bit_cast(wbf16x8, make_uint4(bh0.x, bh0.y, bh1.x, bh1.y));
            const wbf16x8 bl = __builtin_bit_cast(wbf16x8, make_uint4(bl0.x, bl0.y, bl1.x, bl1.y));
            uint2 ar[2][4];
            auto lda = [&](int i, uint2 (&a)[4]) {
                const unsigned char* pa = buf + tapoff[i];
                a[0] = tr_read(pa + a0); a[1] = tr_read(pa + a1);
                a[2] = tr_read(pa + img_plane + a0); a[3] = tr_read(pa + img_plane + a1);
            };
            lda(0, ar[0]);
#pragma unroll
            for (int i = 0; i < TPW; ++i) {
                if (i + 1 < TPW) lda(i + 1, ar[(i + 1) & 1]);
                const uint2 (&a)[4] = ar[i & 1];
                const wbf16x8 ah = __builtin_bit_cast(wbf16x8, make_uint4(a[0].x, a[0].y, a[1].x, a[1].y));
                const wbf16x8 al = __builtin_bit_cast(wbf16x8, make_uint4(a[2].x, a[2].y, a[3].x, a[3].y));
                acc[i] = __builtin_amdgcn_mfma_f32_32x32x16_bf16(al, bh, acc[i], 0, 0, 0);
                acc[i] = __builtin_amdgcn_mfma_f32_32x32x16_bf16(ah, bl, acc[i], 0, 0, 0);
                acc[i] = __builtin_amdgcn_mfma_f32_32x32x16_bf16(ah, bh, acc[i], 0, 0, 0);
            }
        }
        if (has_next) commit(smb + (cur ^ 1) * buf_bytes);
    }

    __syncthreads();
    float* smem = reinterpret_cast<float*>(smb);
    for (int r = 1; r < p.PH; ++r) {
        float* xch = smem + (iw * TPW) * 1024 + lane;
        if (ph == r) {
#pragma unroll
            for (int i = 0; i < TPW; ++i)
#pragma unroll
                for (int e = 0; e < 16; ++e) xch[(i * 16 + e) * 64] = acc[i][e];
        }
        __syncthreads();
        if (ph == 0) {
#pragma unroll
            for (int i = 0; i < TPW; ++i)
#pragma unroll
                for (int e = 0; e < 16; ++e) acc[i][e] += xch[(i * 16 + e) * 64];
        }
        __syncthreads();
    }
    if (ph == 0) {
#pragma unroll
        for (int i = 0; i < TPW; ++i) {
            if (!item_ok[i]) continue;
            float* out = p.out + ((int64_t)slab * p.ntaps + item_tap[i]) * p.C * p.K;
            const int k = k0 + kt_w * 32 + li;
#pragma unroll
            for (int r = 0; r < 16; ++r) {
                const int c = c0 + (r & 3) + 8 * (r >> 2) + 4 * lh;
                if (c < p.C && k < p.K) out[(int64_t)c * p.K + k] = acc[i][r];
            }
        }
    }
    if (do_bias) {
        __syncthreads();
        float4* bx = reinterpret_cast<float4*>(smb);
#pragma unroll
        for (int j = 0; j < NF; ++j) bx[j * 512 + tid] = bsum[j];
        __syncthreads();
        if (tid < 32 * NKT) {
            const int kt = tid >> 5, kk = tid & 31;
            const float* bf = reinterpret_cast<const float*>(smb);
            float t = 0.f;
            for (int pq = 0; pq < p.TPIX; ++pq) t += bf[((kt * p.TPIX + pq) * 8 + (kk >> 2)) * 4 + (kk & 3)];
            const int k = k0 + kt * 32 + kk;
            if (k < p.K) p.bias_out[(int64_t)slab * p.K + k] = t;
        }
    }
}

struct CwParams {
    const float* img; const float* feat; float* out; float* bias_out;
    int N, H, W, C, img_ld, Ho, Wo, K, feat_ld;
    int pt, pl, tiles_h, tiles_w, ctiles, ntiles_total, tiles_per_slab, ntaps;
    int dbg;
};

constexpr int CW_NSTAMP = 64;
__device__ unsigned long long w_stamps[128 * 8 * CW_NSTAMP];
__device__ __forceinline__ void wstamp(bool on, int wave, int lane, int& k) {
    if (on) {
        const unsigned long long t = __builtin_readcyclecounter();
        if (lane == 0 && k < CW_NSTAMP && blockIdx.x == 0 && blockIdx.y < 128) w_stamps[((int)blockIdx.y * 8 + wave) * CW_NSTAMP + k] = t;
        ++k;
    }
}

__device__ __forceinline__ void cw_barrier() { asm volatile("s_waitcnt lgkmcnt(0)\n\ts_barrier" ::: "memory"); }

template <int KW>
__global__ __launch_bounds__(512) void cwgrad_kernel(const CwParams p) {
    constexpr int NTAPS = KW * KW;
    constexpr int TPW = (NTAPS + 3) / 4;
    constexpr int HR = 7 + KW, HC = 15 + KW;
    constexpr int HPIX = HR * HC;
    constexpr int XPL = HPIX * 64, FPL = 128 * 64;
    constexpr int BUF = 2 * XPL + 2 * FPL;
    constexpr int XPIECES = (HPIX + 7) / 8, NPIECES = XPIECES + 16;
    constexpr int PPW = (NPIECES + 3) / 4;
    extern __shared__ __attribute__((aligned(16))) unsigned char smc[];
    const int tid = threadIdx.x;
    const int lane = tid & 63;
    const int wave = __builtin_amdgcn_readfirstlane(tid >> 6);
    const int ct = blockIdx.x % p.ctiles, kt = blockIdx.x / p.ctiles;
    const int c0 = ct * 32, k0 = kt * 32;
    const int slab = blockIdx.y;
    const int tile_begin = slab * p.tiles_per_slab;
    const int tile_end = min(tile_begin + p.tiles_per_slab, p.ntiles_total);
    const int nstages = max(tile_end - tile_begin, 0);
    auto origin = [&](int stage, int& n, int& oh0, int& ow0) {
        int b = tile_begin + stage;
        const int tw_i = b % p.tiles_w; b /= p.tiles_w;
        const int th_i = b % p.tiles_h;
        n = b / p.tiles_h; oh0 = th_i * 8; ow0 = tw_i * 16;
    };

    if (wave >= 4) {
        const int dwv = wave - 4;
        __builtin_amdgcn_s_setprio(2);
        const int c4 = lane & 7, psub = lane >> 3;
        const int64_t xb = (int64_t)p.N * p.H * p.W * p.img_ld * 4, fb = (int64_t)p.N * p.Ho * p.Wo * p.feat_ld * 4;
        const __amdgpu_buffer_rsrc_t xr = __builtin_amdgcn_make_buffer_rsrc(const_cast<float*>(p.img), 0, (int)(xb < 0x7fffffff ? xb : 0x7fffffff), 0x00020000);
        const __amdgpu_buffer_rsrc_t fr = __builtin_amdgcn_make_buffer_rsrc(const_cast<float*>(p.feat), 0, (int)(fb < 0x7fffffff ? fb : 0x7fffffff), 0x00020000);
        constexpr int NXJ = (XPIECES + 3) / 4, NFJ = 4;
        int xvoff[NXJ], xrc[NXJ];
        int fvoff[NFJ], frc[NFJ];
#pragma unroll
        for (int j = 0; j < NXJ; ++j) {
            const int pix = (dwv + 4 * j) * 8 + psub;
            const int hr = pix / HC, hc = pix - hr * HC;
            xvoff[j] = ((hr * p.W + hc) * p.img_ld + c4 * 4) * 4;
            xrc[j] = pix < HPIX ? (hr << 8 | hc) : 0x7fff00;
        }
#pragma unroll
        for (int j = 0; j < NFJ; ++j) {
            const int pq = (dwv + 4 * j) * 8 + psub;
            const int r = pq >> 4, c = pq & 15;
            fvoff[j] = ((r * p.Wo + c) * p.feat_ld + c4 * 4) * 4;
            frc[j] = r << 8 | c;
        }
        const bool xch_ok = c0 + c4 * 4 < p.C, fch_ok = k0 + c4 * 4 < p.K;
        typedef unsigned int wu4 __attribute__((ext_vector_type(4)));
        struct Regs { wu4 x[NXJ]; wu4 f[NFJ]; };
        auto fetch = [&](int stage, Regs& R) {
            int n, oh0, ow0;
            origin(stage, n, oh0, ow0);
            const int ih0 = oh0 - p.pt, iw0 = ow0 - p.pl;
            const int xso = (((n * p.H + ih0) * p.W + iw0) * p.img_ld + c0) * 4;
            const int fso = (((n * p.Ho + oh0) * p.Wo + ow0) * p.feat_ld + k0) * 4;
#pragma unroll
            for (int j = 0; j < NXJ; ++j) {
                const int r = xrc[j] >> 8, c = xrc[j] & 255;
                const bool ok = xch_ok && (unsigned)(ih0 + r) < (unsigned)p.H && (unsigned)(iw0 + c) < (unsigned)p.W;
                const int off = ok ? xvoff[j] + xso : (int)0x80000000;
                R.x[j] = __builtin_amdgcn_raw_buffer_load_b128(xr, off, 0, 0);
            }
#pragma unroll
            for (int j = 0; j < NFJ; ++j) {
                const int r = frc[j] >> 8, c = frc[j] & 255;
                const bool ok = fch_ok && oh0 + r < p.Ho && ow0 + c < p.Wo;
                const int off = ok ? fvoff[j] + fso : (int)0x80000000;
                R.f[j] = __builtin_amdgcn_raw_buffer_load_b128(fr, off, 0, 0);
            }
        };
        float4 bsum[NFJ];
#pragma unroll
        for (int j = 0; j < NFJ; ++j) bsum[j] = make_float4(0.f, 0.f, 0.f, 0.f);
        auto convert = [&](int stage, const Regs& R) {
            unsigned char* const b = smc + (stage & 1) * BUF;
#pragma unroll
            for (int j = 0; j < NXJ; ++j) {
                const float4 v = make_float4(__uint_as_float(R.x[j][0]), __uint_as_float(R.x[j][1]), __uint_as_float(R.x[j][2]), __uint_as_float(R.x[j][3]));
                uint2 hi, lo;
                wsplit4(v, hi, lo);
                if (xrc[j] != 0x7fff00) {
                    unsigned char* d = b + ((dwv + 4 * j) * 8 + psub) * 64 + c4 * 8;
                    *reinterpret_cast<uint2*>(d) = hi;
                    *reinterpret_cast<uint2*>(d + XPL) = lo;
                }
            }
#pragma unroll
            for (int j = 0; j < NFJ; ++j) {
                const float4 v = make_float4(__uint_as_float(R.f[j][0]), __uint_as_float(R.f[j][1]), __uint_as_float(R.f[j][2]), __uint_as_float(R.f[j][3]));
                uint2 hi, lo;
                wsplit4(v, hi, lo);
                unsigned char* d = b + 2 * XPL + ((dwv + 4 * j) * 8 + psub) * 64 + c4 * 8;
                *reinterpret_cast<uint2*>(d) = hi;
                *reinterpret_cast<uint2*>(d + FPL) = lo;
                bsum[j].x += v.x; bsum[j].y += v.y; bsum[j].z += v.z; bsum[j].w += v.w;
            }
        };
        const bool stp = (p.dbg & 32) != 0;
        int sk = 0;
        wstamp(stp, wave, lane, sk);
        Regs R0, R1;
        auto clamp = [&](int st) { return st < nstages ? st : nstages - 1; };
        if (nstages > 0) {
            fetch(0, R0);
            fetch(clamp(1), R1);
            convert(0, R0);
            fetch(clamp(2), R0);
        }
        cw_barrier();
        wstamp(stp, wave, lane, sk);
        for (int s = 0; s < nstages; s += 2) {
#ifdef CW_EXP_WAITSTAMP
            asm volatile("s_waitcnt vmcnt(%0)" :: "n"(NXJ + NFJ) : "memory");
            wstamp(stp, wave, lane, sk);
#endif
            if (s + 1 < nstages) convert(s + 1, R1);
            wstamp(stp, wave, lane, sk);
            fetch(clamp(s + 3), R1);
            cw_barrier();
            wstamp(stp, wave, lane, sk);
            if (s + 1 >= nstages) break;
            if (s + 2 < nstages) convert(s + 2, R0);
            wstamp(stp, wave, lane, sk);
            fetch(clamp(s + 4), R0);
            cw_barrier();
            wstamp(stp, wave, lane, sk);
        }
// ... 30 lines not shown
    }
    f32x16 acc[TPW];
#pragma unroll
    for (int i = 0; i < TPW; ++i)
#pragma unroll
        for (int r = 0; r < 16; ++r) acc[i][r] = 0.f;

    cw_barrier();
    const bool stp = (p.dbg & 32) != 0;
    int stk = 0;
    wstamp(stp, wave, lane, stk);
    for (int s = 0; s < nstages; ++s) {
        const unsigned char* const buf = smc + (s & 1) * BUF;
        const unsigned char* va[TPW];
#pragma unroll
        for (int i = 0; i < TPW; ++i) va[i] = buf + lane_a + tapoff[i];
        const unsigned char* const vb = buf + 2 * XPL + lane_a;
        constexpr int PD = 2;
        constexpr int NSEQ = 8 * TPW;
        uint2 ar[PD + 1][4];
        uint2 br[2][4];
        auto lda = [&](int seq, uint2 (&a)[4]) {
            const int st = seq / TPW, i = seq % TPW;
            const unsigned char* pa = va[i] + st * HC * 64;
            a[0] = tr_read(pa); a[1] = tr_read(pa + 256);
            a[2] = tr_read(pa + XPL); a[3] = tr_read(pa + XPL + 256);
        };
        auto ldb = [&](int st, uint2 (&b)[4]) {
            b[0] = tr_read(vb + st * 1024); b[1] = tr_read(vb + st * 1024 + 256);
            b[2] = tr_read(vb + FPL + st * 1024); b[3] = tr_read(vb + FPL + st * 1024 + 256);
        };
        auto live = [&](int seq) { return seq % TPW < BASE || ((seq / TPW) >> 1) == wave; };
        ldb(0, br[0]);
#pragma unroll
        for (int u = 0; u < PD; ++u) if (live(u)) lda(u, ar[u]);
#pragma unroll
        for (int seq = 0; seq < NSEQ; ++seq) {
            const int st = seq / TPW, i = seq % TPW;
            if (seq + PD < NSEQ && live(seq + PD)) lda(seq + PD, ar[(seq + PD) % (PD + 1)]);
            if (i == 0 && st + 1 < 8) ldb(st + 1, br[(st + 1) & 1]);
            __builtin_amdgcn_sched_barrier(0);
            if (!live(seq)) continue;
            const uint2 (&a)[4] = ar[seq % (PD + 1)];
            const uint2 (&b)[4] = br[st & 1];
            const wbf16x8 ah = __builtin_bit_cast(wbf16x8, make_uint4(a[0].x, a[0].y, a[1].x, a[1].y));
            const wbf16x8 al = __builtin_bit_cast(wbf16x8, make_uint4(a[2].x, a[2].y, a[3].x, a[3].y));
            const wbf16x8 bh = __builtin_bit_cast(wbf16x8, make_uint4(b[0].x, b[0].y, b[1].x, b[1].y));
            const wbf16x8 bl = __builtin_bit_cast(wbf16x8, make_uint4(b[2].x, b[2].y, b[3].x, b[3].y));
            acc[i] = __builtin_amdgcn_mfma_f32_32x32x16_bf16(al, bh, acc[i], 0, 0, 0);
            acc[i] = __builtin_amdgcn_mfma_f32_32x32x16_bf16(ah, bl, acc[i], 0, 0, 0);
            acc[i] = __builtin_amdgcn_mfma_f32_32x32x16_bf16(ah, bh, acc[i], 0, 0, 0);
        }
        wstamp(stp, wave, lane, stk);
        cw_barrier();
        wstamp(stp, wave, lane, stk);
    }
    float* const tp = reinterpret_cast<float*>(smc + 8192);
#pragma unroll
    for (int r = 0; r < 16; ++r) tp[(wave * 16 + r) * 64 + lane] = acc[BASE][r];
    cw_barrier();
    cw_barrier();
    const int k = k0 + li;
#pragma unroll
    for (int i = 0; i < BASE; ++i) {
        float* out = p.out + ((int64_t)slab * p.ntaps + tap_lo + i) * p.C * p.K;
#pragma unroll
        for (int r = 0; r < 16; ++r) {
            const int c = c0 + (r & 3) + 8 * (r >> 2) + 4 * lh;
            if (c < p.C && k < p.K) out[(int64_t)c * p.K + k] = acc[i][r];
        }
    }
    {
        float* out = p.out + ((int64_t)slab * p.ntaps + NTAPS - 1) * p.C * p.K;
#pragma unroll
        for (int q = 0; q < 4; ++q) {
            const int r = wave * 4 + q;
            const float v = ((tp[(0 * 16 + r) * 64 + lane] + tp[(1 * 16 + r) * 64 + lane]) + tp[(2 * 16 + r) * 64 + lane]) + tp[(3 * 16 + r) * 64 + lane];
            const int c = c0 + (r & 3) + 8 * (r >> 2) + 4 * lh;
            if (c < p.C && k < p.K) out[(int64_t)c * p.K + k] = v;
        }
    }
}

static int g_wg_cus_override = 0;
static int wgrad_cus(int kh = 5) {
    static int wg_cus = -1, wg_cus3 = -1;
    if (wg_cus < 0) { const char* e = getenv("MV3D_WG_CUS"); wg_cus = e ? atoi(e) : 128; }
    if (wg_cus3 < 0) { const char* e = getenv("MV3D_WG_CUS_3X3"); wg_cus3 = e ? atoi(e) : wg_cus; }
    return g_wg_cus_override > 0 ? g_wg_cus_override : (kh == 3 ? wg_cus3 : wg_cus);
}
int set_wgrad_cus(int cus) { const int old = g_wg_cus_override; g_wg_cus_override = cus > 0 ? cus : 0; return old; }

static int cwgrad_plan(const mv3d_conv_geom* g, CwParams* out) {
    if ((disabled_paths() & (2 | 4096 | 2097152)) || g->sh != 1 || g->sw != 1 || g->kh != g->kw || (g->kh != 5 && g->kh != 3)) return 0;
    if (g->Ho < 8 || g->Wo < 16 || g->Ho % 8 || g->Wo % 16 || g->C % 32 || g->K % 32 || g->img_ld % 4 || g->feat_ld % 4) return 0;
    if ((int64_t)g->N * g->H * g->W * g->img_ld * 4 >= 0x7fffffff || (int64_t)g->N * g->Ho * g->Wo * g->feat_ld * 4 >= 0x7fffffff) return 0;
    CwParams p = {};
    int ho, wo;
    same_pad(g->H, g->kh, 1, &ho, &p.pt);
    same_pad(g->W, g->kw, 1, &wo, &p.pl);
    p.N = g->N; p.H = g->H; p.W = g->W; p.C = g->C; p.img_ld = g->img_ld; p.Ho = g->Ho; p.Wo = g->Wo; p.K = g->K; p.feat_ld = g->feat_ld;
    p.tiles_h = g->Ho / 8; p.tiles_w = g->Wo / 16; p.ctiles = g->C / 32; p.ntaps = g->kh * g->kw;
    p.ntiles_total = g->N * p.tiles_h * p.tiles_w;
    { static int d = -1; if (d < 0) { const char* e = getenv("MV3D_DBG"); d = e ? atoi(e) : 0; } p.dbg = d; }
    static int min_tiles = -1;
    if (min_tiles < 0) { const char* e = getenv("MV3D_CW_MINTILES"); min_tiles = e ? atoi(e) : 64; }
    if (p.ntiles_total < min_tiles) return 0;
    const int blocks_xy = p.ctiles * (g->K / 32);
    int nslab = std::max(1, wgrad_cus(g->kh) / blocks_xy);
    if (nslab > p.ntiles_total) nslab = p.ntiles_total;
    p.tiles_per_slab = cdiv(p.ntiles_total, nslab);
    nslab = cdiv(p.ntiles_total, p.tiles_per_slab);
    *out = p;
    return nslab;
}

template <int KW>
static int cwgrad_launch_t(const mv3d_conv_geom* g, CwParams p, int nslab, void* stream, const char* who) {
    const double flops = 2.0 * g->N * g->Ho * g->Wo * g->kh * g->kw * (double)g->C * g->K;
    const double bytes = 4.0 * ((double)g->N * g->H * g->W * g->C + (double)g->N * g->Ho * g->Wo * g->K + (double)g->kh * g->kw * g->C * g->K);
    dim3 grid(p.ctiles * (g->K / 32), nslab);
    constexpr int hpix = (7 + KW) * (15 + KW);
    const size_t lds = 2 * (size_t)(2 * hpix * 64 + 2 * 128 * 64);
    static bool attr_set = false;
    if (!attr_set) {
        (void)hipFuncSetAttribute(reinterpret_cast<const void*>(&cwgrad_kernel<KW>), hipFuncAttributeMaxDynamicSharedMemorySize, 160 * 1024);
        attr_set = true;
    }
    return dispatch(stream, OpInfo{KW == 5 ? "cwgrad<5x5>" : "cwgrad<3x3>", flops, bytes}, [=](hipStream_t s) {
        cwgrad_kernel<KW><<<grid, 512, lds, s>>>(p);
        return launched(who);
    });
}

static int cwgrad_launch(const mv3d_conv_geom* g, CwParams p, int nslab, void* stream, const char* who) {
    return g->kw == 5 ? cwgrad_launch_t<5>(g, p, nslab, stream, who) : cwgrad_launch_t<3>(g, p, nslab, stream, who);
}

template <int TPW, int NKT>
static int launch_wgt(const WgTileParams& p, dim3 grid, size_t lds, void* stream, const char* name, const char* who,
                      double flops, double bytes) {
    static bool attr_set = false;
    if (!attr_set) {
        (void)hipFuncSetAttribute(reinterpret_cast<const void*>(&wgrad_tile_kernel<TPW, NKT>),
                                  hipFuncAttributeMaxDynamicSharedMemorySize, 160 * 1024);
        attr_set = true;
    }
    return dispatch(stream, OpInfo{name, flops, bytes}, [=](hipStream_t s) {
        wgrad_tile_kernel<TPW, NKT><<<grid, 512, lds, s>>>(p);
        return launched(who);
    });
}

template <int TPW, int NKT, int NI>
static int launch_wgb(const WgTileParams& p, dim3 grid, size_t lds, void* stream, const char* name, const char* who,
                      double flops, double bytes) {
    static bool attr_set = false;
    if (!attr_set) {
        (void)hipFuncSetAttribute(reinterpret_cast<const void*>(&wgrad_b3_kernel<TPW, NKT, NI>),
                                  hipFuncAttributeMaxDynamicSharedMemorySize, 160 * 1024);
        attr_set = true;
    }
    return dispatch(stream, OpInfo{name, flops, bytes}, [=](hipStream_t s) {
        wgrad_b3_kernel<TPW, NKT, NI><<<grid, 512, lds, s>>>(p);
        return launched(who);
    });
}

bool wgrad_tile_plan(const mv3d_conv_geom* g, WgTileParams* out, int* nslab_out, int* cfg_out, size_t* lds_out) {
    if (disabled_paths() & 2) return false;
    if (g->C < 16 || g->C % 4 != 0 || g->K % 4 != 0 || g->img_ld % 4 != 0 || g->feat_ld % 4 != 0) return false;
    const bool b3_on = !(disabled_paths() & 4096);
    const bool small = b3_on && ((g->Ho == 4 && g->Wo == 4 && g->N >= 8) || (g->Ho == 8 && g->Wo == 8 && g->N >= 2));
    if (!small && (g->Ho * g->Wo < 64 || g->Wo < 8)) return false;
    const int ntaps = g->kh * g->kw;
    int NKT, TPW, IW, PH, cfg;
    if (ntaps == 25) {
        if (g->K > 32) { NKT = 2; IW = 8; PH = 1; TPW = 7; cfg = 1; }
        else { NKT = 1; IW = 4; PH = 2; TPW = 7; cfg = 0; }
    } else if (ntaps == 9) {
        if (g->K > 32) { NKT = 2; IW = 4; PH = 2; TPW = 5; cfg = 3; }
        else { NKT = 1; IW = 2; PH = 4; TPW = 5; cfg = 2; }
    } else return false;
    const bool b3 = !(disabled_paths() & 4096);
    WgTileParams p = {};
    p.b3 = b3 ? 1 : 0;
    int ho, wo;
    same_pad(g->H, g->kh, g->sh, &ho, &p.pt);
    same_pad(g->W, g->kw, g->sw, &wo, &p.pl);
    int64_t best = -1;
    const size_t xchg = (PH > 1) ? (size_t)IW * TPW * 4096 : 0;
    p.G = 1; p.img_shift = 7; p.HRi = 0;
    if (small) {
        const int side = g->Ho, ipx = side * side, sshift = side == 4 ? 2 : 3;
        for (int G = 128 / ipx; G >= std::max(1, 64 / ipx) && best < 0; G >>= 1) {
            const int tpix = G * ipx;
            if ((tpix >> 4) % PH != 0) continue;
            const int HRi = (side - 1) * g->sh + g->kh, HC = (side - 1) * g->sw + g->kw, HR = G * HRi;
            const size_t lds = std::max(2 * (size_t)(((HR * HC + tpix * NKT + 7) / 8) * 1024), xchg);
            if (lds > 160 * 1024 || HR * HC * 8 > 8 * 512) continue;
            p.G = G; p.img_shift = 2 * sshift; p.TH = side; p.TW = side; p.tw_shift = sshift; p.tiles_h = p.tiles_w = 1; p.TPIX = tpix;
            p.HRi = HRi; p.HC = HC; p.HR = HR;
            best = 1;
        }
    }
    for (int tpix = 128; tpix >= 64 && best < 0; tpix >>= 1) {
        if (b3 ? ((tpix >> 4) % PH != 0) : ((tpix >> 1) / PH < 2)) break;
        for (int sh = 3; sh <= 6; ++sh) {
            const int TW = 1 << sh, TH = tpix / TW;
            if (TH < 1 || TH > g->Ho * 2 || TW > g->Wo * 2) continue;
            const int th = cdiv(g->Ho, TH), tw = cdiv(g->Wo, TW);
            const int HR = (TH - 1) * g->sh + g->kh, HC = (TW - 1) * g->sw + g->kw;
            const size_t lds = std::max(2 * (size_t)(((HR * HC + tpix * NKT + 7) / 8) * 1024), xchg);
            if (lds > 160 * 1024) continue;
            if (b3 && HR * HC * 8 > 8 * 512) continue;
            const int64_t cost = (int64_t)th * tw * (tpix * 64 + HR * HC);
            if (best < 0 || cost < best) {
                best = cost;
                p.TH = TH; p.TW = TW; p.tw_shift = sh; p.tiles_h = th; p.tiles_w = tw; p.HR = HR; p.HC = HC; p.TPIX = tpix;
            }
        }
    }
    if (best < 0) return false;
    p.N = g->N; p.H = g->H; p.W = g->W; p.C = g->C; p.img_ld = g->img_ld;
    p.Ho = g->Ho; p.Wo = g->Wo; p.K = g->K; p.feat_ld = g->feat_ld;
    p.sh = g->sh; p.sw = g->sw; p.kw = g->kw;
    p.ntaps = ntaps; p.nitems = ntaps * NKT; p.ipw = cdiv(p.nitems, IW); p.IW = IW; p.PH = PH;
    (void)TPW;
    p.ctiles = cdiv(g->C, 32);
    const int kgroups = cdiv(g->K, 32 * NKT);
    if (p.G == 1) { p.HRi = p.HR; p.img_shift = p.TPIX == 128 ? 7 : 6; }
    p.inv_hri = ((1 << 20) + p.HRi - 1) / p.HRi;
    p.ntiles_total = cdiv(g->N, p.G) * p.tiles_h * p.tiles_w;
    const int blocks_xy = p.ctiles * kgroups;
    int nslab = std::max(1, wgrad_cus(g->kh) / blocks_xy);
    if (nslab > p.ntiles_total) nslab = p.ntiles_total;
    p.tiles_per_slab = cdiv(p.ntiles_total, nslab);
    nslab = cdiv(p.ntiles_total, p.tiles_per_slab);
    p.inv_hc = ((1 << 20) + p.HC - 1) / p.HC;
    p.tpix8_shift = p.TPIX == 128 ? 10 : 9;
    p.tsplit = 1;
    {
        static int ts = -1;
        if (ts < 0) { const char* e = getenv("MV3D_WG_TAPSPLIT"); ts = e ? atoi(e) : 2; }
        if (b3 && ts == 2) p.tsplit = 2;
    }
    *out = p;
    *nslab_out = nslab;
    *cfg_out = cfg;
    *lds_out = std::max(2 * (size_t)(((p.HR * p.HC + p.TPIX * NKT + 7) / 8) * 1024), xchg);
    if (b3) *lds_out = std::max(*lds_out, (size_t)32 * 1024);
    return true;
}

int wgrad_tile_launch(const mv3d_conv_geom* g, WgTileParams p, int nslab, int cfg, size_t lds, void* stream, const char* who) {
    const double flops = 2.0 * g->N * g->Ho * g->Wo * g->kh * g->kw * (double)g->C * g->K;
    const double bytes = 4.0 * ((double)g->N * g->H * g->W * g->C + (double)g->N * g->Ho * g->Wo * g->K + (double)g->kh * g->kw * g->C * g->K);
    const int NKTv = (cfg & 1) ? 2 : 1;
    dim3 grid(p.ctiles * cdiv(g->K, 32 * NKTv), nslab, p.b3 ? p.tsplit : 1);
    if (p.b3) {
        const bool ni4 = p.HR * p.HC * 8 <= 4 * 512;
        if (p.tsplit == 2) {
            if (cfg == 0) return ni4 ? launch_wgb<4, 1, 4>(p, grid, lds, stream, "wgrad_b3<5x5,K32,taps/2>", who, flops, bytes) : launch_wgb<4, 1, 8>(p, grid, lds, stream, "wgrad_b3<5x5,K32,taps/2>", who, flops, bytes);
            if (cfg == 1) return ni4 ? launch_wgb<4, 2, 4>(p, grid, lds, stream, "wgrad_b3<5x5,K64,taps/2>", who, flops, bytes) : launch_wgb<4, 2, 8>(p, grid, lds, stream, "wgrad_b3<5x5,K64,taps/2>", who, flops, bytes);
            if (cfg == 2) return ni4 ? launch_wgb<3, 1, 4>(p, grid, lds, stream, "wgrad_b3<3x3,K32,taps/2>", who, flops, bytes) : launch_wgb<3, 1, 8>(p, grid, lds, stream, "wgrad_b3<3x3,K32,taps/2>", who, flops, bytes);
            return ni4 ? launch_wgb<3, 2, 4>(p, grid, lds, stream, "wgrad_b3<3x3,K64,taps/2>", who, flops, bytes) : launch_wgb<3, 2, 8>(p, grid, lds, stream, "wgrad_b3<3x3,K64,taps/2>", who, flops, bytes);
        }
        switch (cfg) {
            case 0: return ni4 ? launch_wgb<7, 1, 4>(p, grid, lds, stream, "wgrad_b3<5x5,K32>", who, flops, bytes) : launch_wgb<7, 1, 8>(p, grid, lds, stream, "wgrad_b3<5x5,K32>", who, flops, bytes);
            case 1: return ni4 ? launch_wgb<7, 2, 4>(p, grid, lds, stream, "wgrad_b3<5x5,K64>", who, flops, bytes) : launch_wgb<7, 2, 8>(p, grid, lds, stream, "wgrad_b3<5x5,K64>", who, flops, bytes);
            case 2: return ni4 ? launch_wgb<5, 1, 4>(p, grid, lds, stream, "wgrad_b3<3x3,K32>", who, flops, bytes) : launch_wgb<5, 1, 8>(p, grid, lds, stream, "wgrad_b3<3x3,K32>", who, flops, bytes);
            default: return ni4 ? launch_wgb<5, 2, 4>(p, grid, lds, stream, "wgrad_b3<3x3,K64>", who, flops, bytes) : launch_wgb<5, 2, 8>(p, grid, lds, stream, "wgrad_b3<3x3,K64>", who, flops, bytes);
        }
    }
    switch (cfg) {
        case 0: return launch_wgt<7, 1>(p, grid, lds, stream, "wgrad_tile<5x5,K32>", who, flops, bytes);
        case 1: return launch_wgt<7, 2>(p, grid, lds, stream, "wgrad_tile<5x5,K64>", who, flops, bytes);
        case 2: return launch_wgt<5, 1>(p, grid, lds, stream, "wgrad_tile<3x3,K32>", who, flops, bytes);
        default: return launch_wgt<5, 2>(p, grid, lds, stream, "wgrad_tile<3x3,K64>", who, flops, bytes);
    }
}

int wgrad_tile_nslab(const mv3d_conv_geom* g) {
    { CwParams cp; const int ns = cwgrad_plan(g, &cp); if (ns > 0) return ns; }
    WgTileParams p; int nslab, cfg; size_t lds;
    return wgrad_tile_plan(g, &p, &nslab, &cfg, &lds) ? nslab : 0;
}

int wgrad_tile_launch_erased(const mv3d_conv_geom* g, const void* img, const void* feat, void* out, void* bias_out, void* stream,
                             const char* who, int* nslab_out) {
    {
        CwParams cp;
        const int ns = cwgrad_plan(g, &cp);
        if (ns > 0) {
            cp.img = (const float*)img; cp.feat = (const float*)feat; cp.out = (float*)out; cp.bias_out = (float*)bias_out;
            *nslab_out = ns;
            return cwgrad_launch(g, cp, ns, stream, who);
        }
    }
    WgTileParams p; int nslab, cfg; size_t lds;
    if (!wgrad_tile_plan(g, &p, &nslab, &cfg, &lds)) return fail(MV3D_E_INVAL, "%s: tiled wgrad not applicable", who);
    p.img = (const float*)img; p.feat = (const float*)feat; p.out = (float*)out; p.bias_out = (float*)bias_out;
    *nslab_out = nslab;
    return wgrad_tile_launch(g, p, nslab, cfg, lds, stream, who);
}

}

extern "C" int mv3d_debug_cwgrad_stamps(void* dst, size_t bytes) {
    if (!dst || bytes > sizeof(unsigned long long) * 128 * 8 * mv3d::CW_NSTAMP) return mv3d::fail(MV3D_E_INVAL, "mv3d_debug_cwgrad_stamps: bad buffer");
    hipError_t e = hipMemcpyFromSymbol(dst, HIP_SYMBOL(mv3d::w_stamps), bytes, 0, hipMemcpyDeviceToHost);
    if (e != hipSuccess) return mv3d::fail(MV3D_E_HIP, "mv3d_debug_cwgrad_stamps: %s", hipGetErrorString(e));
    return MV3D_OK;
}
```

dynamic_multiview_3d_amd/graph.py:

```python
import ctypes as C
import os
import math
from collections import OrderedDict

import numpy as np
import torch

from . import _lib
from ._lib import ACT_NONE, ACT_LRELU, ACT_RELU, ACT_TANH

_current = []


def current_graph():
    if not _current:
        raise RuntimeError("no Graph is active: build models inside `with Graph(...) as g:`")
    return _current[-1]


class Storage:

    def __init__(self, rows, ch, alias_of=None):
        self.rows, self.ch = rows, ch
        self.parent, self.ch_off = None, 0
        self.alias_of = alias_of
        self.has_alias = False
        self.data = None
        self.grad = None
        self.needs_grad = False
        self.external = False
        if alias_of is not None:
            alias_of.has_alias = True

    def resolve(self):
        s, off = self, 0
        while s.parent is not None:
            off += s.ch_off
            s = s.parent
        return s, off

    def can_be_adopted(self):
        return self.parent is None and self.alias_of is None and not self.has_alias and not self.external


class Tensor:
    def __init__(self, graph, shape, storage=None, ch_off=0, producer=None, act=ACT_NONE, leak=0.2,
                 requires_grad=False, name=None):
        self.graph = graph
        self.shape = tuple(int(s) for s in shape)
        self.C = self.shape[-1]
        self.rows = int(np.prod(self.shape[:-1])) if len(self.shape) > 1 else 1
        self.storage = storage if storage is not None else Storage(self.rows, self.C)
        self.ch_off = ch_off
        self.producer = producer
        self.act, self.leak = act, leak
        self.requires_grad = requires_grad
        self.name = name
        self.fused_into = None
        self.grad_consumers = 0
        self.grad_written = False
        self.grad_masked = False
        if requires_grad:
            self.storage.needs_grad = True

    def get_shape(self):
        return list(self.shape)

    def _root(self):
        s = self.storage
        if s.alias_of is not None:
            root, off = s.alias_of.resolve()
            assert off == 0 and root.ch == s.alias_of.ch
            return root, 0, s.ch
        root, off = s.resolve()
        return root, off, root.ch

    @property
    def ld(self):
        return self._root()[2]

    @property
    def ptr(self):
        root, off, _ = self._root()
        return root.data.data_ptr() + 4 * (off + self.ch_off)

    @property
    def grad_ptr(self):
        root, off, _ = self._root()
        return root.grad.data_ptr() + 4 * (off + self.ch_off)

    def _view(self, buf):
        root, off, ld = self._root()
        v = buf.view(-1, ld)[:, off + self.ch_off: off + self.ch_off + self.C]
        return v.reshape(self.shape) if v.is_contiguous() else v.unflatten(0, self.shape[:-1])

    def value(self):
        return self._view(self._root()[0].data)

    def grad_value(self):
        return self._view(self._root()[0].grad)

    def numpy(self):
        return self.value().detach().cpu().numpy().copy()

    def set(self, array):
        t = torch.as_tensor(np.ascontiguousarray(array, dtype=np.float32)) if not torch.is_tensor(array) else array
        self.value().copy_(t.reshape(self.shape), non_blocking=True)


class Variable:
    def __init__(self, name, shape, init):
        self.name, self.shape, self.init = name, tuple(shape), init
        self.size = int(np.prod(shape))
        self.offset = None
        self.graph = None
        self.has_grad = False

    @property
    def ptr(self):
        return self.graph.params.data_ptr() + 4 * self.offset

    @property
    def grad_ptr(self):
        return self.graph.grads.data_ptr() + 4 * self.offset

    def value(self):
        self.graph._settle()
        return self.graph.params[self.offset:self.offset + self.size].view(self.shape)

    def grad_value(self):
        self.graph._settle()
        return self.graph.grads[self.offset:self.offset + self.size].view(self.shape)


class ScalarExpr:

    def __init__(self, terms=()):
        self.terms = list(terms)

    def __add__(self, o):
        if isinstance(o, (int, float)):
            if o != 0:
                raise NotImplementedError("adding a non-zero constant to a loss")
            return ScalarExpr(self.terms)
        return ScalarExpr(self.terms + o.terms)

    __radd__ = __add__

    def __mul__(self, c):
        return ScalarExpr([(w * float(c), t) for w, t in self.terms])

    __rmul__ = __mul__


# ... 206 lines not shown
                    _ensure_premasked(g, o)
        for i in self.ins:
            if i.requires_grad:
                if want_mask and i.act == ACT_NONE:
                    raise RuntimeError("view of mixed activation / linear tensors cannot carry a masked gradient")
                _note_grad_written(i, want_mask)


class CopyConcatNode(Node):

    def __init__(self, ins, out):
        self.ins, self.out = ins, out

    def forward(self, g):
        off = 0
        for t in self.ins:
            g.lib.copy2d(t.rows, t.C, t.ptr, t.ld, 1, self.out.ptr + 4 * off, self.out.ld, 0, g.stream)
            off += t.C

    def backward(self, g):
        o = self.out
        if not o.grad_written:
            return
        off = 0
        for t in self.ins:
            if t.requires_grad:
                g.lib.copy2d(t.rows, t.C, o.grad_ptr + 4 * off, o.ld, 1, t.grad_ptr, t.ld, 0, g.stream)
                _note_grad_written(t, o.grad_masked and t.act != ACT_NONE)
                if o.grad_masked and t.act == ACT_NONE:
                    raise RuntimeError("masked gradient reached a linear tensor through concat")
            off += t.C


class TileNode(Node):

    def __init__(self, x, y, reps):
        self.x, self.y, self.reps = x, y, reps

    def forward(self, g):
        x, y = self.x, self.y
        g.lib.copy2d(y.rows, y.C, x.ptr, x.ld, self.reps, y.ptr, y.ld, 0, g.stream)

    def backward(self, g):
        x, y = self.x, self.y
        if not y.grad_written or not x.requires_grad:
            return
        g.lib.group_sum(x.rows, self.reps, x.C, y.grad_ptr, y.ld, x.grad_ptr, x.ld, g.stream)
        _note_grad_written(x, y.grad_masked)


class ResampleNode(Node):

    def __init__(self, src, flow, warp, gen):
        self.src, self.flow, self.warp, self.gen = src, flow, warp, gen
        self.fused_loss = None

    def workspace_bytes(self, g):
        if not self.src.requires_grad:
            return 0
        n, h, w, _ = self.flow.shape
        _, hs, ws, c = self.src.shape
        return g.lib.resampler_bwd_workspace_bytes(n, h * w, hs, ws, c)

    def forward(self, g):
        n, h, w, _ = self.flow.shape
        _, hs, ws, c = self.src.shape
        if self.fused_loss is not None:
            wgt, term = self.fused_loss
            want_grad = self.flow.requires_grad
            g.lib.warp_resample_loss(n, h, w, hs, ws, c, self.src.ptr, self.flow.ptr, self.flow.ld, term.b.ptr, term.b.ld,
                                     term.kind, float(wgt), self.warp.ptr, self.gen.ptr,
                                     self.flow.grad_ptr if want_grad else None, self.flow.ld, g.loss_buf.data_ptr(), g.stream)
            if want_grad:
                _note_grad_written(self.flow, False)
            return
        g.lib.warp_resample_fwd(n, h, w, hs, ws, c, self.src.ptr, self.flow.ptr, self.flow.ld,
                                self.warp.ptr, self.gen.ptr, g.stream)

    def backward(self, g):
        if self.fused_loss is not None or not self.gen.grad_written:
            return
        n, h, w, _ = self.flow.shape
        _, hs, ws, c = self.src.shape
        if self.flow.requires_grad:
            g.lib.warp_resample_bwd(n, h, w, hs, ws, c, self.src.ptr, self.flow.ptr, self.flow.ld,
                                    self.gen.grad_ptr, self.flow.grad_ptr, self.flow.ld, g.stream)
            _note_grad_written(self.flow, False)
        if self.src.requires_grad:
            g.lib.resampler_bwd(n, h * w, hs, ws, c, self.src.ptr, self.src.ld, self.warp.ptr, 2, self.gen.grad_ptr, self.gen.ld,
                                None, 0, self.src.grad_ptr, self.src.ld, g.ws_ptr, g.ws_bytes, g.stream)
            _note_grad_written(self.src, False)


class ResamplerNode(Node):

    def __init__(self, src, warp, out):
        self.src, self.warp, self.out = src, warp, out

    def _dims(self):
        n, hs, ws, c = self.src.shape
        return n, self.warp.rows // n, hs, ws, c

    def workspace_bytes(self, g):
        return g.lib.resampler_bwd_workspace_bytes(*self._dims()) if self.src.requires_grad else 0

    def forward(self, g):
        src, warp, out = self.src, self.warp, self.out
        g.lib.resampler_fwd(*self._dims(), src.ptr, src.ld, warp.ptr, warp.ld, out.ptr, out.ld, g.stream)

    def backward(self, g):
        src, warp, out = self.src, self.warp, self.out
        if not out.grad_written or not (warp.requires_grad or src.requires_grad):
            return
        g.lib.resampler_bwd(*self._dims(), src.ptr, src.ld, warp.ptr, warp.ld, out.grad_ptr, out.ld,
                            warp.grad_ptr if warp.requires_grad else None, warp.ld,
                            src.grad_ptr if src.requires_grad else None, src.ld, g.ws_ptr, g.ws_bytes, g.stream)
        for t in (warp, src):
            if t.requires_grad:
                _note_grad_written(t, False)


class Graph:

    ALIGN = 64

    def __init__(self, device=None, seed=1234):
        self.device = torch.device(device if device is not None else 'cuda')
        self.rng = np.random.default_rng(seed)
        self.nodes = []
        self.tensors = []
        self.inputs = OrderedDict()
        self.variables = OrderedDict()
        self._scope = []
        self.loss_expr = None
        self.lr = None
        self.finalized = False
        self.lib = None
        self.stream = None
        self.ws = None
        self.ws_ptr, self.ws_bytes = None, 0
        self.n_side = max(0, min(4, int(os.environ.get('MV3D_SIDE_STREAMS', '2'))))
        self.ws_side = []
        self.side_streams = None
        self.adam_stream = None
        self.adam_timing = None
        self.overlap_adam = os.environ.get('MV3D_OVERLAP_ADAM', '1') != '0'
        self.fuse_fc_adam = os.environ.get('MV3D_FUSE_FC_ADAM', '1') != '0'
        self._fusing = False
        self.fuse_finalize = os.environ.get('MV3D_FUSE_FINALIZE', '1') != '0'
        self.finalize_chunk_bytes = int(float(os.environ.get('MV3D_FINALIZE_CHUNK_MB', '48')) * 1e6)
        self._finalizing = False
        self._finalized_in_plan = False
        self._part_arena = self._fin_table = None
        self._fused_vars = []
        self.pipeline_fc = os.environ.get('MV3D_PIPELINE_FCADAM', '1') != '0'
        self.pipeline_dp = os.environ.get('MV3D_PIPELINE_DP', '1') != '0'
        self.pipeline_dp_min_idx = 8
        self._fused_nodes = []
        self._fwd_wait_idx = 0
        self._fc_event = None
        self._fc_pending = False
        self._pending_idx = 0
        self.plan_bwd_fused = None
        self.opt_state = None
        self.plan_fwd = self.plan_bwd = None
        self._smooth_deferred = []
        self.optimizer = 'adam'
        self.momentum, self.use_nesterov = 0.0, False
        self.adam_m = self.adam_v = self.accum = None
        self.beta1, self.beta2, self.eps = 0.9, 0.999, 1e-8
        self.beta1_power = np.float32(self.beta1)
        self.beta2_power = np.float32(self.beta2)
        self.world_size, self.dist_group = 1, None
        self.comm = None
        self.dp_mode = 'sharded'
        self.comm_stream = None
        self.bucket_elems = 16 * 1024 * 1024

    OPTIMIZERS = ('adam', 'momentum', 'sgd')

    @property
    def adam_state(self):
        return self.opt_state

    def __enter__(self):
        _current.append(self)
        return self

    def __exit__(self, *a):
        _current.pop()

    def scope_name(self, name):
        return '/'.join(self._scope + [name])

    def variable(self, name, shape, init):
        full = self.scope_name(name)
        if full in self.variables:
            raise ValueError("variable %s already exists" % full)
        v = Variable(full, shape, init)
        v.graph = self
        self.variables[full] = v
        return v

    def placeholder(self, shape, name):
        t = Tensor(self, shape, name=name)
        t.storage.external = True
        self.inputs[name] = t
        self.tensors.append(t)
        return t

    def new_tensor(self, shape, **kw):
        t = Tensor(self, shape, **kw)
        self.tensors.append(t)
        return t

    def add(self, node):
        self.nodes.append(node)
        return node

    def finalize(self):
        if self.finalized:
            return
        self.lib = _lib.lib()
        dev = self.device
        roots = []
        for t in self.tensors:
            s = t.storage
            base = s.alias_of if s.alias_of is not None else s
            root, _ = base.resolve()
            if s.needs_grad:
                root.needs_grad = True
            if root not in roots:
                roots.append(root)
        act_bytes = 0
        for r in roots:
            r.data = torch.zeros(r.rows * r.ch, dtype=torch.float32, device=dev)
            act_bytes += r.rows * r.ch * 4
            if r.needs_grad:
                r.grad = torch.zeros(r.rows * r.ch, dtype=torch.float32, device=dev)
                act_bytes += r.rows * r.ch * 4
        self.activation_bytes = act_bytes
        off = 0
        for v in self.variables.values():
            v.offset = off
            off += -(-v.size // self.ALIGN) * self.ALIGN
        self.flat_size = off
        host = np.zeros(off, dtype=np.float32)
        for v in self.variables.values():
            host[v.offset:v.offset + v.size] = v.init(self.rng, v.shape).reshape(-1)
        self.params = torch.from_numpy(host).to(dev)
        self.grads = torch.zeros(off, dtype=torch.float32, device=dev)
        if self.optimizer not in self.OPTIMIZERS:
            raise ValueError("unknown optimizer %r (have %s)" % (self.optimizer, ', '.join(self.OPTIMIZERS)))
        if self.optimizer == 'adam':
            self.adam_m = torch.zeros(off, dtype=torch.float32, device=dev)
            self.adam_v = torch.zeros(off, dtype=torch.float32, device=dev)
        elif self.optimizer == 'momentum':
            self.accum = torch.zeros(off, dtype=torch.float32, device=dev)
        self.opt_state = torch.zeros(16, dtype=torch.float32, device=dev)
        self.loss_buf = torch.zeros(4, dtype=torch.float32, device=dev)
        self.zero_buf = torch.zeros(1024, dtype=torch.float32, device=dev)
        self.zero_ptr = self.zero_buf.data_ptr()
        self.finalized = True
        need = 0
        for n in self.nodes:
            if hasattr(n, 'workspace_bytes'):
                need = max(need, int(n.workspace_bytes(self)))
        self.ws_bytes = need
        self.ws = torch.empty(max(need // 4, 4), dtype=torch.float32, device=dev)
        self.ws_ptr = self.ws.data_ptr()
        self.ws_side = [torch.empty(max(need // 4, 4), dtype=torch.float32, device=dev) for _ in range(self.n_side)]

    def _fuse_resample_losses(self):
        self.fused_terms = set()
        enabled = os.environ.get('MV3D_FUSE_RESAMPLE', '1') != '0'
        for n in self.nodes:
            if not isinstance(n, ResampleNode):
                continue
            n.fused_loss = None
            if not enabled or self.loss_expr is None or n.src.requires_grad:
                continue
            gen = n.gen
            uses = [(w, t) for w, t in self.loss_expr.terms if t.a is gen or t.b is gen or t.mask is gen]
            if len(uses) != 1:
                continue
            w, t = uses[0]
            if t.kind == LOSS_SSIM:
                continue
            if t.a is not gen or t.mask is not None or t.b_scale != 1.0 or t.b.requires_grad or t.b.rows != gen.rows or t.b.C != gen.C:
                continue
            if gen.C > 4 or gen.ld != gen.C or gen.storage.has_alias or gen.storage.alias_of is not None:
                continue
            read_elsewhere = False
            for m in self.nodes:
                if m is n:
                    continue
                for v in vars(m).values():
                    vs = v if isinstance(v, (list, tuple)) else (v,)
                    if any(x is gen for x in vs):
                        read_elsewhere = True
            if read_elsewhere:
                continue
            n.fused_loss = (w, t)
            self.fused_terms.add(id(t))

    def _find_fc_chains(self):
# ... 58 lines not shown
                self.lib.ssim_loss(n, h, wd, c, a.ptr, a.ld, b.ptr, b.ld, term.max_val, float(w), self.loss_buf.data_ptr(), grad, a.ld,
                                   1 if grad in written else 0, term.ws.data_ptr(), term.ws.numel(), self.stream)
            else:
                self.lib.pixel_loss_strided(a.rows, a.C, a.ptr, a.ld, b.ptr, b.ld, term.b_scale,
                                            m.ptr if m is not None else None, m.ld if m is not None else 1,
                                            term.kind, float(w), self.loss_buf.data_ptr(), grad, a.ld, self.stream)
            if grad is not None:
                written.add(grad)
                _note_grad_written(a, False)

    def _smooth_launch(self, w, term, value, grad, accumulate):
        a, b = term.a, term.b
        if grad and accumulate and a.grad_masked:
            raise NotImplementedError("flow_smoothness_loss on a tensor whose gradient buffer already holds d/d(pre-activation)")
        n, h, wd, _ = a.shape
        self.lib.flow_smoothness(n, h, wd, a.ptr, a.ld, b.ptr if b is not None else None, b.C if b is not None else 0,
                                 b.ld if b is not None else 0, term.edge_alpha, term.eps, float(w),
                                 self.loss_buf.data_ptr() if value else None, a.grad_ptr if grad else None, a.ld,
                                 1 if (grad and accumulate) else 0, term.ws.data_ptr(), term.ws.numel(), self.stream)
        if grad:
            _note_grad_written(a, False)

    def _smooth_before(self, n, pending):
        for wt in [wt for wt in pending if wt[1].a.producer is n]:
            self._smooth_launch(wt[0], wt[1], value=False, grad=True, accumulate=wt[1].a.grad_written)
            pending.remove(wt)

    def _smooth_after(self, pending):
        for wt in [wt for wt in pending if wt[1].a.grad_written]:
            self._smooth_launch(wt[0], wt[1], value=False, grad=True, accumulate=True)
            pending.remove(wt)

    def _backward_node(self, n, pending):
        self._smooth_before(n, pending)
        n.backward(self)
        self._smooth_after(pending)

    @staticmethod
    def _smooth_all_placed(pending):
        if pending:
            raise RuntimeError("flow_smoothness_loss: the reverse pass has no place for the gradient of %d term(s): no node of "
                               "this graph produces the tensor" % len(pending))

    def compile(self, stream=None):
        self.finalize()
        self.stream = stream
        lib = self.lib
        for t in self.tensors:
            t.grad_written = t.grad_masked = False
        self._smooth_deferred = []
        self._bind_prepared_filters()
        self._fuse_resample_losses()
        for _, term in (self.loss_expr.terms if self.loss_expr is not None else ()):
            if term.kind == LOSS_SSIM and term.ws is None:
                nbytes = int(lib.ssim_loss_workspace_bytes(*term.a.shape))
                if not nbytes:
                    raise ValueError("ssim_loss: operands of shape %s are outside what mv3d_ssim_loss takes" % (term.a.shape,))
                term.ws = torch.empty(nbytes, dtype=torch.uint8, device=self.device)
            if term.kind == LOSS_SMOOTH and term.ws is None:
                nbytes = int(lib.flow_smoothness_workspace_bytes(*term.a.shape[:3]))
                if not nbytes:
                    raise ValueError("flow_smoothness_loss: a flow of shape %s is outside what mv3d_flow_smoothness takes" % (term.a.shape,))
                term.ws = torch.empty(nbytes, dtype=torch.uint8, device=self.device)
        self._find_fc_chains()
        self.plan_fwd = lib.plan_create()
        lib.plan_begin(self.plan_fwd)
        try:
            lib.filter_cache_refresh(None)
            if self.loss_expr is not None and self.loss_expr.terms:
                lib.loss_overwrite_next()
            else:
                lib.fill(self.loss_buf.data_ptr(), 1, 0.0, self.stream)
            self._fwd_first_op = {}
            for n in self.nodes:
                self._fwd_first_op[id(n)] = lib.plan_size(self.plan_fwd)
                n.forward(self)
            self._emit_losses(with_grad=True)
        finally:
            lib.plan_end()
        flags_after_forward = [(t.grad_written, t.grad_masked) for t in self.tensors]
        self.plan_bwd = lib.plan_create()
        lib.plan_begin(self.plan_bwd)
        self.grad_buckets = []
        try:
            done = set()
            order = list(self.variables.values())
            suffix = len(order)
            cut_hi = self.flat_size
            gate = 0
            pending = list(self._smooth_deferred)
            for n in reversed(self.nodes):
                self._backward_node(n, pending)
                if isinstance(n, LinearNode):
                    gate = lib.plan_size(self.plan_bwd)
                for v in (getattr(n, 'w', None), getattr(n, 'b', None), getattr(n, 'm', None)):
                    if isinstance(v, Variable):
                        done.add(v.name)
                while suffix > 0 and order[suffix - 1].name in done:
                    suffix -= 1
                lo = order[suffix].offset if suffix < len(order) else self.flat_size
                boundary = False
                if isinstance(n, ConvNode) and cut_hi > lo:
                    for prev in reversed(self.nodes[:self.nodes.index(n)]):
                        if any(isinstance(v, Variable) for v in vars(prev).values()):
                            boundary = isinstance(prev, LinearNode)
                            break
                if cut_hi - lo >= self.bucket_elems or boundary:
                    self.grad_buckets.append((lib.plan_size(self.plan_bwd), lo, cut_hi))
                    cut_hi = lo
            self._smooth_all_placed(pending)
        finally:
            lib.plan_end()
        nbwd = lib.plan_size(self.plan_bwd)
        if cut_hi > 0 or not self.grad_buckets:
            self.grad_buckets.append((nbwd, 0, cut_hi))
        else:
            end, lo, hi = self.grad_buckets[-1]
            self.grad_buckets[-1] = (nbwd, lo, hi)
        mode = os.environ.get('MV3D_ADAM_GATE', '0.9')
        if mode == 'none':
            gate = 0
        elif mode != 'fc':
            gate = int(float(mode) * nbwd)
        self.adam_gate = gate if 0 < gate < nbwd else 0
        if self.adam_gate and all(b[0] != self.adam_gate for b in self.grad_buckets):
            i = next(j for j, b in enumerate(self.grad_buckets) if b[0] > self.adam_gate)
            hi = self.grad_buckets[i][2]
            self.grad_buckets.insert(i, (self.adam_gate, hi, hi))
        self.n_launch_fwd = lib.plan_size(self.plan_fwd)
        self.n_launch_bwd = lib.plan_size(self.plan_bwd)
        self._bucket_first_use = [self._first_param_use(lo, hi) for _, lo, hi in self.grad_buckets]
        self.plan_bwd_fused = None
        self._fused_vars = []
        self._fused_nodes = []
        if self.fuse_fc_adam and self.lr is not None and any(isinstance(n, LinearNode) for n in self.nodes):
            for t, (gw, gm) in zip(self.tensors, flags_after_forward):
                t.grad_written, t.grad_masked = gw, gm
            plan = lib.plan_create()
            self._finalized_in_plan = False
            if self.fuse_finalize:
                off = 0
                for n in self.nodes:
                    if isinstance(n, ConvNode):
                        n._part_off, n._part_bytes = off, n.wgrad_partial_bytes(self)
                        off += -(-n._part_bytes // 256) * 256
                self._part_arena = torch.empty(max(off // 4, 4), dtype=torch.float32, device=self.device)
                lib.grad_finalize_begin()
                self._finalizing = True
                self._fin_pending, self._fin_vars, self._fin_done, self._fin_tables = 0, [], set(), []
            lib.plan_begin(plan)
            self._fusing = True
            pending = list(self._smooth_deferred)
            try:
                for n in reversed(self.nodes):
                    self._backward_node(n, pending)
                    if self._finalizing and isinstance(n, ConvNode) and n.w.has_grad:
                        self._fin_pending += n._part_bytes
                        self._fin_vars += [n.w] + ([n.b] if n.b is not None else [])
                        if self._fin_pending >= self.finalize_chunk_bytes:
                            self._finalize_commit()
                            lib.grad_finalize_begin()
                self._smooth_all_placed(pending)
                for n in self._fused_nodes:
                    n.record_fused_update(self)
                if self._finalizing and self._fused_vars:
                    fused = {id(v) for v in self._fused_vars} | {id(n.b) for n in self._fused_nodes}
                    for v in self.variables.values():
                        if v.has_grad and id(v) not in fused and id(v) not in self._fin_done:
                            lib.grad_finalize_add(v.grad_ptr, -(-v.size // 4) * 4)
                    self._finalize_commit()
                    self._finalizing = False
                    self._finalized_in_plan = True
            finally:
                self._fusing = False
                if self._finalizing:
                    lib.grad_finalize_abort()
                    self._finalizing = False
                lib.plan_end()
            if self._fused_vars:
                self.plan_bwd_fused = plan
                self.n_launch_bwd_fused = lib.plan_size(plan)
                def merged(ranges):
                    out = []
                    for lo, hi in sorted(ranges):
                        if out and lo <= out[-1][1]:
                            out[-1][1] = max(out[-1][1], hi)
                        else:
                            out.append([lo, hi])
                    return out
                pad4 = lambda v: (v.offset, v.offset + -(-v.size // 4) * 4)
                biases = merged(pad4(n.b) for n in self._fused_nodes)
                skips = merged([pad4(v) for v in self._fused_vars] + [tuple(b) for b in biases])
                assert len(skips) <= 8, "mv3d_adam_step_dev leaves at most 8 ranges untouched"
                self._skip_lo = (C.c_int64 * len(skips))(*[a for a, _ in skips])
                self._skip_hi = (C.c_int64 * len(skips))(*[b for _, b in skips])
                self._bias_span = (biases[0][0], biases[-1][1])
                gaps = [(biases[i][1] - biases[0][0], biases[i + 1][0] - biases[0][0]) for i in range(len(biases) - 1)]
                assert len(gaps) <= 8
                self._bias_skip = (len(gaps), (C.c_int64 * max(1, len(gaps)))(*[a for a, _ in gaps] or [0]),
                                   (C.c_int64 * max(1, len(gaps)))(*[b for _, b in gaps] or [0]))
                self._fwd_wait_idx = self._first_fc_hazard()
            else:
                lib.plan_destroy(plan)
        self.upload_optimizer_state()
        return self

    def _finalize_commit(self):
        lib = self.lib
        on_gpu = torch.device(self.device).type == 'cuda'
        tb = int(lib.grad_finalize_table_bytes())
        table = torch.empty(max(tb, 16), dtype=torch.uint8, device=self.device) if on_gpu else None
        self._fin_tables.append(table)
        self.begin_side()
        try:
            tp = table.data_ptr() if on_gpu else None
            if self.optimizer == 'adam':
                lib.grad_finalize_commit(tp, tb, self.grads.data_ptr(), self.params.data_ptr(),
                                         self.adam_m.data_ptr(), self.adam_v.data_ptr(), self.opt_state.data_ptr(), self.stream)
            else:
                lib.grad_finalize_commit_sgd(tp, tb, self.grads.data_ptr(), self.params.data_ptr(),
                                             self.accum.data_ptr() if self.accum is not None else None, self.opt_state.data_ptr(),
                                             self.stream)
        finally:
            self.end_side()
        self._fin_done |= {id(v) for v in self._fin_vars}
        self._fin_pending, self._fin_vars = 0, []

    def _bind_prepared_filters(self):
        lib = self.lib
        lib.filter_cache_clear()
        self._prepared = []
        if torch.device(self.device).type != 'cuda':
            return
        for n in self.nodes:
            if not isinstance(n, ConvNode):
                continue
            geom = n.geom()
            ops = [2 if n.transposed else 0]
            if n.x.requires_grad:
                ops.append(3 if n.transposed else 1)
            for op in ops:
                nbytes = int(lib.filter_prepared_bytes(C.byref(geom), op))
                if nbytes > 0:
                    buf = torch.empty(nbytes, dtype=torch.uint8, device=self.device)
                    self._prepared.append(buf)
                    lib.filter_cache_bind(C.byref(geom), op, n.w.ptr, buf.data_ptr(), nbytes)
        tb = int(lib.filter_cache_table_bytes())
        self._prepared_table = torch.empty(max(tb, 16), dtype=torch.uint8, device=self.device)
        lib.filter_cache_commit(self._prepared_table.data_ptr(), tb, None)

    def _stream_ptr(self):
        return torch.cuda.current_stream(self.device).cuda_stream

    def _first_param_use(self, lo, hi):
        first = self.n_launch_fwd
        for n in self.nodes:
            for name, val in vars(n).items():
                if isinstance(val, Variable) and val.offset is not None and lo <= val.offset < hi:
                    first = min(first, 0 if (isinstance(n, ConvNode) and name == 'w') else self._fwd_first_op[id(n)])
        return first

    def _first_fc_hazard(self):
        roots = set()
        for n in self._fused_nodes:
            root = n.x._root()[0]
            if root.external or n.x.storage.external:
                return None
            roots.add(id(root))
        def tensors_of(node):
            for val in vars(node).values():
                for t in (val if isinstance(val, (list, tuple)) else (val,)):
                    if isinstance(t, Tensor):
                        yield t
        fused = {id(n) for n in self._fused_nodes}
        idx = self.n_launch_fwd
        for n in self.nodes:
            if id(n) in fused or any(id(t._root()[0]) in roots for t in tensors_of(n)):
                idx = min(idx, self._fwd_first_op[id(n)])
        return idx

    def _settle(self):
        if self._fc_pending:
            torch.cuda.current_stream(self.device).wait_event(self._fc_event)
            self._fc_pending = False

    settle = _settle

    def run_forward(self):
        st = self._stream_ptr()
        if self._fc_pending and 0 < self._pending_idx < self.n_launch_fwd:
            self.lib.plan_run_range(self.plan_fwd, 0, self._pending_idx, st)
            self._settle()
            self.lib.plan_run_range(self.plan_fwd, self._pending_idx, self.n_launch_fwd, st)
            return
        self._settle()
        self.lib.plan_run(self.plan_fwd, st)

    def begin_side(self, cls=1):
        if self.n_side == 0:
            return self.ws_ptr
        k = (cls - 1) % self.n_side
        self.lib.plan_side(k + 1)
        return self.ws_side[k].data_ptr()

    def end_side(self):
        if self.n_side:
            self.lib.plan_side(0)

    def _side_ptrs(self):
        if self.n_side == 0 or torch.device(self.device).type != 'cuda':
            return None, 0
        if self.side_streams is None:
            self.side_streams = [torch.cuda.Stream(device=self.device) for _ in range(self.n_side)]
            self._side_arr = (C.c_void_p * self.n_side)(*[st.cuda_stream for st in self.side_streams])
        return self._side_arr, self.n_side

    def run_backward(self):
        self._settle()
        sides, ns = self._side_ptrs()
        self.lib.plan_run_range_multi(self.plan_bwd, 0, self.n_launch_bwd, self._stream_ptr(), sides, ns, 0)

    def allreduce_grads(self):
        self._settle()
        if self.world_size > 1:
            self.comm.allreduce_sum_(self.grads, 0, self.flat_size, self._stream_ptr())

    def upload_optimizer_state(self):
        if self.opt_state is None or self.lr is None:
            return
        if self.optimizer == 'adam':
            vals = [self.lr, self.beta1, self.beta2, self.eps, self.beta1_power, self.beta2_power]
        else:
            vals = [self.lr, self.momentum, 1.0 if self.use_nesterov else 0.0, 0.0, 0.0, 0.0]
        vals = np.array(vals + [1.0 / self.world_size, 0.0], np.float32)
        self._settle()
        self.opt_state.copy_(torch.from_numpy(np.concatenate([vals, vals])))

    upload_adam_state = upload_optimizer_state

    def _opt_range(self, lo, hi, stream, skips=None, state=None):
        off = lo * 4
        n, slo, shi = (0, None, None) if skips is None else skips
        state = self.opt_state.data_ptr() if state is None else state
        if self.optimizer == 'adam':
            self.lib.adam_step_dev(hi - lo, self.params.data_ptr() + off, self.grads.data_ptr() + off, self.adam_m.data_ptr() + off,
                                   self.adam_v.data_ptr() + off, state, n, slo, shi, stream)
        else:
            self.lib.sgd_step_dev(hi - lo, self.params.data_ptr() + off, self.grads.data_ptr() + off,
                                  self.accum.data_ptr() + off if self.accum is not None else None, state, n, slo, shi, stream)

    _adam_range = _opt_range

    def _adam_advance(self, stream=None, both=True):
        if self.optimizer != 'adam':
            return
        st = self._stream_ptr() if stream is None else stream
        self.lib.adam_advance(self.opt_state.data_ptr(), st)
        if both:
# ... 247 lines not shown
```

include/mv3d_hip.h:

```cpp
#ifndef MV3D_HIP_H
#define MV3D_HIP_H
#include <stddef.h>
#include <stdint.h>

#ifdef __cplusplus
extern "C" {
#endif

enum { MV3D_OK = 0, MV3D_E_INVAL = -1, MV3D_E_HIP = -2, MV3D_E_WORKSPACE = -3, MV3D_E_UNSUPPORTED = -4 };
enum { MV3D_F32 = 0 };
enum { MV3D_ACT_NONE = 0, MV3D_ACT_LRELU = 1, MV3D_ACT_RELU = 2, MV3D_ACT_TANH = 3 };

typedef struct mv3d_conv_geom {
    int32_t N;
    int32_t H, W, C;
    int32_t Ho, Wo, K;
    int32_t kh, kw, sh, sw;
    int32_t img_ld, feat_ld;
    int32_t dtype;
} mv3d_conv_geom;

typedef struct mv3d_epilogue {
    const void* bias;
    int32_t act;
    float leak;
    int32_t gmask_act;
    float gmask_leak;
    const void* gmask_ref;
    int32_t gmask_ld;
} mv3d_epilogue;

const char* mv3d_version(void);
const char* mv3d_last_error(void);
int mv3d_set_diagnostics(int mask);
int mv3d_set_wgrad_cus(int cus);

typedef struct mv3d_tfrecord_reader mv3d_tfrecord_reader;
int mv3d_tfrecord_open(const char* path, int verify_crc, mv3d_tfrecord_reader** out);
int mv3d_tfrecord_read(mv3d_tfrecord_reader* r, int max_records, int first, int nfeat, const char* const* names, const int* kinds,
                       const size_t* sizes, void* const* dst, int* nread);
void mv3d_tfrecord_close(mv3d_tfrecord_reader* r);
int mv3d_u8_to_unit_f32(int64_t count, const void* src, void* dst, void* stream);

int mv3d_u8_process_image(const void* src, int n, int hs, int ws, int c, void* dst, int ho, int wo, void* stream);

uint32_t mv3d_crc32c(const void* data, size_t n);

int mv3d_conv2d_fwd(const mv3d_conv_geom* g, const void* x, const void* w, void* y,
                    const mv3d_epilogue* epi, void* workspace, size_t workspace_bytes, void* stream);
int mv3d_conv2d_dgrad(const mv3d_conv_geom* g, const void* dy, const void* w, void* dx,
                      const mv3d_epilogue* epi, void* workspace, size_t workspace_bytes, void* stream);
int mv3d_conv2d_wgrad(const mv3d_conv_geom* g, const void* x, const void* dy, void* dw, void* db,
                      void* workspace, size_t workspace_bytes, void* stream);

int mv3d_deconv2d_fwd(const mv3d_conv_geom* g, const void* x, const void* w, void* y,
                      const mv3d_epilogue* epi, void* workspace, size_t workspace_bytes, void* stream);
int mv3d_deconv2d_dgrad(const mv3d_conv_geom* g, const void* dy, const void* w, void* dx,
                        const mv3d_epilogue* epi, void* workspace, size_t workspace_bytes, void* stream);
int mv3d_deconv2d_wgrad(const mv3d_conv_geom* g, const void* x, const void* dy, void* dw,
                        void* workspace, size_t workspace_bytes, void* stream);
size_t mv3d_conv_workspace_bytes(const mv3d_conv_geom* g);
size_t mv3d_conv_wgrad_workspace_bytes(const mv3d_conv_geom* g);

enum { MV3D_FILTER_CONV_FWD = 0, MV3D_FILTER_CONV_DGRAD = 1, MV3D_FILTER_DECONV_FWD = 2, MV3D_FILTER_DECONV_DGRAD = 3 };
size_t mv3d_filter_prepared_bytes(const mv3d_conv_geom* g, int op);
int mv3d_filter_cache_bind(const mv3d_conv_geom* g, int op, const void* w, void* prepared, size_t prepared_bytes);
size_t mv3d_filter_cache_table_bytes(void);
int mv3d_filter_cache_commit(void* table_dev, size_t table_bytes, void* stream);
int mv3d_filter_cache_refresh(void* stream);
int mv3d_filter_cache_clear(void);

int mv3d_fc_fwd(int B, int in, int out, const void* x, int x_ld, const void* M, void* y, int y_ld,
                const mv3d_epilogue* epi, void* workspace, size_t workspace_bytes, void* stream);
int mv3d_fc_dgrad(int B, int in, int out, const void* dy, int dy_ld, const void* M, void* dx, int dx_ld,
                  const mv3d_epilogue* epi, void* workspace, size_t workspace_bytes, void* stream);
int mv3d_fc_wgrad(int B, int in, int out, const void* x, int x_ld, const void* dy, int dy_ld,
                  void* dM, void* db, void* workspace, size_t workspace_bytes, void* stream);
int mv3d_fc_wgrad_dgrad(int B, int in, int out, const void* x, int x_ld, const void* dy, int dy_ld, const void* M,
                        void* dM, void* db, void* dx, int dx_ld, const mv3d_epilogue* dx_epi,
                        void* workspace, size_t workspace_bytes, void* stream);
#define MV3D_FC_CHAIN_MAX 4
typedef struct mv3d_fc_chain_layer {
    const void* M;
    const void* bias;
    void* y;
    int32_t y_ld, out;
    int32_t act;
    float leak;
} mv3d_fc_chain_layer;
typedef struct mv3d_fc_chain {
    int32_t B, nlayers, in, x_ld;
    const void* x;
    mv3d_fc_chain_layer l[MV3D_FC_CHAIN_MAX];
} mv3d_fc_chain;
int mv3d_fc_chain_fwd(const mv3d_fc_chain* chain, void* stream);
size_t mv3d_fc_workspace_bytes(int B, int in, int out);

int mv3d_act_fwd(int64_t rows, int ch, const void* x, int x_ld, void* y, int y_ld, int act, float leak, void* stream);
int mv3d_act_bwd(int64_t rows, int ch, const void* dy, int dy_ld, const void* ref, int ref_ld,
                 void* dx, int dx_ld, int act, float leak, void* stream);
int mv3d_copy2d(int64_t rows, int ch, const void* src, int64_t src_ld, int64_t src_row_div,
                void* dst, int64_t dst_ld, int accumulate, void* stream);
int mv3d_group_sum(int64_t groups, int group, int ch, const void* src, int64_t src_ld, void* dst, int64_t dst_ld, void* stream);

int mv3d_warp_resample_fwd(int N, int H, int W, int Hs, int Ws, int C, const void* src, const void* flow, int flow_ld,
                           void* warp_out, void* gen, void* stream);
int mv3d_warp_resample_bwd(int N, int H, int W, int Hs, int Ws, int C, const void* src, const void* flow, int flow_ld,
                           const void* dgen, void* dflow, int dflow_ld, void* stream);
int mv3d_warp_resample_loss(int N, int H, int W, int Hs, int Ws, int C, const void* src, const void* flow, int flow_ld,
                            const void* target, int target_ld, int kind, float weight, void* warp_out, void* gen,
                            void* dflow, int dflow_ld, void* loss_accum, void* stream);

int mv3d_resampler_fwd(int N, int P, int Hs, int Ws, int C, const void* data, int data_ld,
                       const void* warp, int warp_ld, void* out, int out_ld, void* stream);
size_t mv3d_resampler_bwd_workspace_bytes(int N, int P, int Hs, int Ws, int C);
int mv3d_resampler_bwd(int N, int P, int Hs, int Ws, int C, const void* data, int data_ld,
                       const void* warp, int warp_ld, const void* dout, int dout_ld,
                       void* dwarp, int dwarp_ld, void* ddata, int ddata_ld,
                       void* workspace, size_t workspace_bytes, void* stream);

int mv3d_pixel_loss(int64_t pixels, int ch, const void* a, const void* b, const void* mask, int kind, float weight,
                    void* loss_accum, void* grad, void* stream);
int mv3d_pixel_loss_strided(int64_t pixels, int ch, const void* a, int a_ld, const void* b, int b_ld, float b_scale,
                            const void* mask, int mask_ld, int kind, float weight, void* loss_accum, void* grad, int grad_ld,
                            void* stream);
int mv3d_fill(void* dst, int64_t count, float value, void* stream);
int mv3d_loss_overwrite_next(void);

size_t mv3d_image_metrics_workspace_bytes(int N, int H, int W, int C);
int mv3d_image_metrics(int N, int H, int W, int C, const void* a, int a_ld, const void* b, int b_ld, float max_val, void* out,
                       void* workspace, size_t workspace_bytes, void* stream);

size_t mv3d_ssim_loss_workspace_bytes(int N, int H, int W, int C);
int mv3d_ssim_loss(int N, int H, int W, int C, const void* a, int a_ld, const void* b, int b_ld, float max_val, float weight,
                   void* loss_accum, void* grad, int grad_ld, int grad_accumulate, void* workspace, size_t workspace_bytes,
                   void* stream);

size_t mv3d_flow_smoothness_workspace_bytes(int N, int H, int W);
int mv3d_flow_smoothness(int N, int H, int W, const void* flow, int flow_ld, const void* guide, int guide_c, int guide_ld,
                         float edge_alpha, float eps, float weight, void* loss_accum, void* grad, int grad_ld, int grad_accumulate,
                         void* workspace, size_t workspace_bytes, void* stream);

int mv3d_adam_step(int64_t count, void* p, const void* g, void* m, void* v, float lr, float beta1, float beta2,
                   float eps, float beta1_power, float beta2_power, float grad_scale, void* stream);

enum { MV3D_ADAM_LR = 0, MV3D_ADAM_BETA1 = 1, MV3D_ADAM_BETA2 = 2, MV3D_ADAM_EPS = 3, MV3D_ADAM_BETA1_POWER = 4, MV3D_ADAM_BETA2_POWER = 5,
       MV3D_ADAM_GSCALE = 6, MV3D_ADAM_STATE_FLOATS = 8 };
int mv3d_adam_step_dev(int64_t count, void* p, const void* g, void* m, void* v, const void* adam_state, int nskip,
                       const int64_t* skip_lo, const int64_t* skip_hi, void* stream);
int mv3d_adam_advance(void* adam_state, void* stream);
int mv3d_fc_wgrad_adam(int B, int in, int out, const void* x, int x_ld, const void* dy, int dy_ld, void* M, void* adam_m, void* adam_v,
                       void* db, const void* adam_state, void* stream);
int mv3d_fc_wgrad_adam_supported(int B, int in, int out, int x_ld, int dy_ld);

int mv3d_sgd_step(int64_t count, void* p, const void* g, void* accum, float lr, float momentum, int use_nesterov,
                  float grad_scale, void* stream);
enum { MV3D_SGD_LR = 0, MV3D_SGD_MOMENTUM = 1, MV3D_SGD_NESTEROV = 2, MV3D_SGD_GSCALE = 6, MV3D_SGD_STATE_FLOATS = 8 };
int mv3d_sgd_step_dev(int64_t count, void* p, const void* g, void* accum, const void* sgd_state, int nskip,
                      const int64_t* skip_lo, const int64_t* skip_hi, void* stream);
int mv3d_fc_wgrad_sgd(int B, int in, int out, const void* x, int x_ld, const void* dy, int dy_ld, void* M, void* accum,
                      void* db, const void* sgd_state, void* stream);

int mv3d_grad_finalize_begin(void);
int mv3d_grad_finalize_add(void* grad, int64_t count);
size_t mv3d_grad_finalize_table_bytes(void);
int mv3d_grad_finalize_commit(void* table, size_t table_bytes, void* grads, void* params, void* adam_m, void* adam_v,
                              const void* adam_state, void* stream);
int mv3d_grad_finalize_commit_sgd(void* table, size_t table_bytes, void* grads, void* params, void* accum, const void* sgd_state,
                                  void* stream);
int mv3d_grad_finalize_abort(void);

typedef struct mv3d_comm mv3d_comm;
int mv3d_comm_available(void);
int mv3d_comm_unique_id(void* id128);
int mv3d_comm_init(mv3d_comm** out, int rank, int world, const void* id128);
int mv3d_comm_destroy(mv3d_comm* comm);
int mv3d_comm_allreduce_sum(mv3d_comm* comm, void* buf, int64_t count, void* stream);
int mv3d_comm_reduce_scatter_sum(mv3d_comm* comm, const void* send, void* recv, int64_t recv_count, void* stream);
int mv3d_comm_allgather(mv3d_comm* comm, const void* send, void* recv, int64_t send_count, void* stream);

#define MV3D_MESH_MAX_RANKS 8
int mv3d_ipc_export(const void* ptr, void* handle64, int64_t* offset);
int mv3d_ipc_open(const void* handle64, void** base);
int mv3d_ipc_close(void* base);
int mv3d_mesh_reduce_sum(const void* const* srcs, int nsrc, void* dst, int64_t count, void* stream);
int mv3d_mesh_copy(void* dst, const void* src, int64_t count, void* stream);

typedef struct mv3d_plan mv3d_plan;
mv3d_plan* mv3d_plan_create(void);
void mv3d_plan_destroy(mv3d_plan* p);
int mv3d_plan_begin(mv3d_plan* p);
int mv3d_plan_end(void);
int mv3d_plan_size(const mv3d_plan* p);
int mv3d_plan_run(mv3d_plan* p, void* stream);
int mv3d_plan_run_range(mv3d_plan* p, int begin, int end, void* stream);
#define MV3D_MAX_SIDE 4
int mv3d_plan_side(int side);
#define MV3D_RUN_NO_JOIN 1
int mv3d_plan_run_range_multi(mv3d_plan* p, int begin, int end, void* stream, void* const* side_streams, int nside, int flags);
int mv3d_plan_profile(mv3d_plan* p, int enable);
int mv3d_plan_profile_collect(mv3d_plan* p);
int mv3d_plan_profile_select(mv3d_plan* p, const char* name);
int mv3d_plan_profile_reset(mv3d_plan* p);
int mv3d_plan_op_info(const mv3d_plan* p, int i, const char** name, double* flops, double* bytes,
                      double* total_ms, int* runs);

int mv3d_debug_cconv_stamps(void* host_dst, size_t bytes);
int mv3d_debug_cwgrad_stamps(void* host_dst, size_t bytes);
int mv3d_debug_band_stamps(void* host_dst, size_t bytes);

#ifdef __cplusplus
}
#endif
#endif
```

Before: 40060 images/sec.

## Batch consecutive conv weight-gradient kernels into one grouped launch

Adds a grouping mechanism that queues up to four consecutive tiled wgrad (b3) jobs sharing the same kernel configuration and launches them as one kernel. Each block looks up its job from a block-range table. The aim is to cut launch overhead and fill the GPU better when individual small wgrad grids underfill it. The grouped launch is issued on the side stream inside the recorded plan. It adds host-side queue state, error-path cleanup, and a runtime NI branch inside the kernel that may raise register pressure.

```diff
diff --git a/dynamic_multiview_3d_amd/_lib.py b/dynamic_multiview_3d_amd/_lib.py
--- a/dynamic_multiview_3d_amd/_lib.py
+++ b/dynamic_multiview_3d_amd/_lib.py
@@ -43,6 +43,8 @@
     "mv3d_deconv2d_fwd": [_G, _vp, _vp, _vp, _E, _vp, _sz, _vp],
     "mv3d_deconv2d_dgrad": [_G, _vp, _vp, _vp, _E, _vp, _sz, _vp],
     "mv3d_deconv2d_wgrad": [_G, _vp, _vp, _vp, _vp, _sz, _vp],
+    "mv3d_conv_wgrad_group_begin": [],
+    "mv3d_conv_wgrad_group_end": [_vp],
     "mv3d_fc_fwd": [_i, _i, _i, _vp, _i, _vp, _vp, _i, _E, _vp, _sz, _vp],
     "mv3d_fc_dgrad": [_i, _i, _i, _vp, _i, _vp, _vp, _i, _E, _vp, _sz, _vp],
     "mv3d_fc_wgrad": [_i, _i, _i, _vp, _i, _vp, _i, _vp, _vp, _vp, _sz, _vp],
@@ -113,6 +115,7 @@
     "mv3d_last_error": (C.c_char_p, []),
     "mv3d_conv_workspace_bytes": (_sz, [_G]),
     "mv3d_conv_wgrad_workspace_bytes": (_sz, [_G]),
+    "mv3d_conv_wgrad_group_key": (_i, [_G]),
     "mv3d_fc_workspace_bytes": (_sz, [_i, _i, _i]),
     "mv3d_resampler_bwd_workspace_bytes": (_sz, [_i, _i, _i, _i, _i]),
     "mv3d_image_metrics_workspace_bytes": (_sz, [_i, _i, _i, _i]),
diff --git a/dynamic_multiview_3d_amd/csrc/common.h b/dynamic_multiview_3d_amd/csrc/common.h
--- a/dynamic_multiview_3d_amd/csrc/common.h
+++ b/dynamic_multiview_3d_amd/csrc/common.h
@@ -55,6 +55,11 @@
 const std::vector<FinSegHost>* finalize_peek();
 void finalize_take(std::vector<FinSegHost>* out);
 
+bool wgrad_group_collecting();
+int wgrad_group_pending();
+int wgrad_group_open();
+int wgrad_group_close(void* stream, bool launch);
+
 int disabled_paths();
 
 static inline int cdiv(int a, int b) { return (a + b - 1) / b; }
diff --git a/dynamic_multiview_3d_amd/csrc/conv.hip b/dynamic_multiview_3d_amd/csrc/conv.hip
--- a/dynamic_multiview_3d_amd/csrc/conv.hip
+++ b/dynamic_multiview_3d_amd/csrc/conv.hip
@@ -1401,7 +1401,8 @@
 
 struct WgTileParams;
 bool wgrad_tile_plan(const mv3d_conv_geom* g, struct WgTileParams* out, int* nslab_out, int* cfg_out, size_t* lds_out);
-int wgrad_tile_launch_erased(const mv3d_conv_geom* g, const void* img, const void* feat, void* out, void* bias_out, void* stream, const char* who, int* nslab_out);
+int wgrad_tile_launch_erased(const mv3d_conv_geom* g, const void* img, const void* feat, void* out, void* bias_out, void* stream, const char* who, int* nslab_out, bool own_ws);
+int wgrad_group_key(const mv3d_conv_geom* g);
 
 static void filtgrad_plan(const mv3d_conv_geom* g, FiltgradParams& p, int* nt_out, int* nslab_out) {
     int ho, wo;
@@ -1470,7 +1471,7 @@
                 bpart = db ? (float*)ws + (int64_t)tiled * fcount : nullptr;
             }
             int ns = 0;
-            rc = wgrad_tile_launch_erased(g, img, feat, part, bpart, stream, who, &ns);
+            rc = wgrad_tile_launch_erased(g, img, feat, part, bpart, stream, who, &ns, finalize_collecting());
             if (rc == MV3D_OK && ns == 1 && finalize_collecting()) { finalize_push(nullptr, 0, fcount, dfp); if (dbp) finalize_push(nullptr, 0, K, dbp); }
             if (rc != MV3D_OK || ns == 1) return rc;
             return dispatch_reduce(stream, part, ns, fcount, dfp, bpart, K, dbp);
@@ -1548,9 +1549,13 @@
                       void* ws, size_t wsb, void* stream) {
     return feat2img(g, dy, w, dx, epi, ws, wsb, stream, "mv3d_conv2d_dgrad");
 }
+static int wgrad_checked(int rc) {
+    if (rc != MV3D_OK) (void)wgrad_group_close(nullptr, false);
+    return rc;
+}
 int mv3d_conv2d_wgrad(const mv3d_conv_geom* g, const void* x, const void* dy, void* dw, void* db,
                       void* ws, size_t wsb, void* stream) {
-    return filtgrad(g, x, dy, dw, db, ws, wsb, stream, "mv3d_conv2d_wgrad");
+    return wgrad_checked(filtgrad(g, x, dy, dw, db, ws, wsb, stream, "mv3d_conv2d_wgrad"));
 }
 int mv3d_deconv2d_fwd(const mv3d_conv_geom* g, const void* x, const void* w, void* y, const mv3d_epilogue* epi,
                       void* ws, size_t wsb, void* stream) {
@@ -1561,7 +1566,16 @@
     return img2feat(g, dy, w, dx, epi, ws, wsb, stream, "mv3d_deconv2d_dgrad");
 }
 int mv3d_deconv2d_wgrad(const mv3d_conv_geom* g, const void* x, const void* dy, void* dw, void* ws, size_t wsb, void* stream) {
-    return filtgrad(g, dy, x, dw, nullptr, ws, wsb, stream, "mv3d_deconv2d_wgrad");
+    return wgrad_checked(filtgrad(g, dy, x, dw, nullptr, ws, wsb, stream, "mv3d_deconv2d_wgrad"));
+}
+int mv3d_conv_wgrad_group_begin(void) { return wgrad_group_open(); }
+int mv3d_conv_wgrad_group_end(void* stream) {
+    if (!wgrad_group_collecting()) return fail(MV3D_E_INVAL, "mv3d_conv_wgrad_group_end: no open collection");
+    return wgrad_group_close(stream, true);
+}
+int mv3d_conv_wgrad_group_key(const mv3d_conv_geom* g) {
+    if (!g || check_geom(g, "mv3d_conv_wgrad_group_key") != MV3D_OK) return 0;
+    return wgrad_group_key(g);
 }
 
 static bool filter_op_params(const mv3d_conv_geom* g, int op, const void* w, IgemmParams& p, const char* who) {
diff --git a/dynamic_multiview_3d_amd/csrc/core.hip b/dynamic_multiview_3d_amd/csrc/core.hip
--- a/dynamic_multiview_3d_amd/csrc/core.hip
+++ b/dynamic_multiview_3d_amd/csrc/core.hip
@@ -109,7 +109,10 @@
 }
 int mv3d_plan_end(void) {
     if (!mv3d::g_rec) return mv3d::fail(MV3D_E_INVAL, "mv3d_plan_end: nothing is recording");
+    const int lost = mv3d::wgrad_group_pending();
+    (void)mv3d::wgrad_group_close(nullptr, false);
     mv3d::g_rec = nullptr;
+    if (lost) return mv3d::fail(MV3D_E_INVAL, "mv3d_plan_end: %d filter-gradient job(s) were still queued (mv3d_conv_wgrad_group_end missing)", lost);
     return MV3D_OK;
 }
 int mv3d_plan_size(const mv3d_plan* p) { return p ? (int)p->ops.size() : 0; }
diff --git a/dynamic_multiview_3d_amd/csrc/elem.hip b/dynamic_multiview_3d_amd/csrc/elem.hip
--- a/dynamic_multiview_3d_amd/csrc/elem.hip
+++ b/dynamic_multiview_3d_amd/csrc/elem.hip
@@ -855,6 +855,7 @@
 int mv3d_grad_finalize_commit(void* table, size_t table_bytes, void* grads, void* params, void* adam_m, void* adam_v,
                               const void* adam_state, void* stream) {
     if (!finalize_collecting()) return fail(MV3D_E_INVAL, "mv3d_grad_finalize_commit: no open collection");
+    if (wgrad_group_pending()) { finalize_take(nullptr); (void)wgrad_group_close(nullptr, false); return fail(MV3D_E_INVAL, "mv3d_grad_finalize_commit: filter-gradient jobs are still queued (mv3d_conv_wgrad_group_end first)"); }
     const size_t need = mv3d_grad_finalize_table_bytes();
     std::vector<FinSegHost> segs;
     finalize_take(&segs);
@@ -867,6 +868,7 @@
 int mv3d_grad_finalize_commit_sgd(void* table, size_t table_bytes, void* grads, void* params, void* accum, const void* sgd_state,
                                   void* stream) {
     if (!finalize_collecting()) return fail(MV3D_E_INVAL, "mv3d_grad_finalize_commit_sgd: no open collection");
+    if (wgrad_group_pending()) { finalize_take(nullptr); (void)wgrad_group_close(nullptr, false); return fail(MV3D_E_INVAL, "mv3d_grad_finalize_commit_sgd: filter-gradient jobs are still queued (mv3d_conv_wgrad_group_end first)"); }
     const size_t need = mv3d_grad_finalize_table_bytes();
     std::vector<FinSegHost> segs;
     finalize_take(&segs);
diff --git a/dynamic_multiview_3d_amd/csrc/wgrad_tile.hip b/dynamic_multiview_3d_amd/csrc/wgrad_tile.hip
--- a/dynamic_multiview_3d_amd/csrc/wgrad_tile.hip
+++ b/dynamic_multiview_3d_amd/csrc/wgrad_tile.hip
@@ -201,9 +201,16 @@
     return __builtin_bit_cast(uint2, v);
 }
 
+constexpr int WG_MAXJ = 4;
+struct WgGroup {
+    int njobs;
+    int block_end[WG_MAXJ];
+    int gx[WG_MAXJ], gy[WG_MAXJ];
+    WgTileParams job[WG_MAXJ];
+};
+
 template <int TPW, int NKT, int NI>
-__global__ __launch_bounds__(512) void wgrad_b3_kernel(const WgTileParams p) {
-    extern __shared__ __attribute__((aligned(16))) unsigned char smb[];
+__device__ __forceinline__ void wgrad_b3_body(const WgTileParams& p, const int bx, const int by, const int bz, unsigned char* const smb) {
     constexpr int NF = 4;
     const int tid = threadIdx.x;
     const int lane = tid & 63;
@@ -213,9 +220,9 @@
     const int tg_per_kt = p.IW / NKT;
     const int kt_w = iw / tg_per_kt, tg = iw - kt_w * tg_per_kt;
     const int li = lane & 31, lh = lane >> 5;
-    const int ct = blockIdx.x % p.ctiles, kg = blockIdx.x / p.ctiles;
+    const int ct = bx % p.ctiles, kg = bx / p.ctiles;
     const int c0 = ct * 32, k0 = kg * 32 * NKT;
-    const int slab = blockIdx.y;
+    const int slab = by;
     const int tile_begin = slab * p.tiles_per_slab;
     const int tile_end = min(tile_begin + p.tiles_per_slab, p.ntiles_total);
 
@@ -227,7 +234,7 @@
 
     int tapoff[TPW], item_tap[TPW];
     bool item_ok[TPW];
-    const int tg_total = tg_per_kt * p.tsplit, tgi = (int)blockIdx.z * tg_per_kt + tg;
+    const int tg_total = tg_per_kt * p.tsplit, tgi = bz * tg_per_kt + tg;
     const int tap_lo = (p.ntaps * tgi) / tg_total, tap_n = (p.ntaps * (tgi + 1)) / tg_total - tap_lo;
 #pragma unroll
     for (int i = 0; i < TPW; ++i) {
@@ -253,7 +260,7 @@
     float4 bsum[NF];
 #pragma unroll
     for (int j = 0; j < NF; ++j) bsum[j] = make_float4(0.f, 0.f, 0.f, 0.f);
-    const bool do_bias = p.bias_out != nullptr && ct == 0 && blockIdx.z == 0;
+    const bool do_bias = p.bias_out != nullptr && ct == 0 && bz == 0;
     const int n_img4 = halo_pix * 8, n_feat4 = p.TPIX * NKT * 8;
     auto fetch = [&](int tile) {
         int b = tile;
@@ -409,6 +416,39 @@
             if (k < p.K) p.bias_out[(int64_t)slab * p.K + k] = t;
         }
     }
+}
+
+__device__ __forceinline__ WgTileParams wg_job_params(const WgTileParams& src) {
+    WgTileParams p = src;
+#define WG_PIN(f) asm volatile("" : "+s"(p.f))
+    WG_PIN(img); WG_PIN(feat); WG_PIN(out); WG_PIN(bias_out);
+    WG_PIN(N); WG_PIN(H); WG_PIN(W); WG_PIN(C); WG_PIN(img_ld);
+    WG_PIN(Ho); WG_PIN(Wo); WG_PIN(K); WG_PIN(feat_ld);
+    WG_PIN(sh); WG_PIN(sw); WG_PIN(pt); WG_PIN(pl); WG_PIN(kw);
+    WG_PIN(TH); WG_PIN(TW); WG_PIN(tw_shift); WG_PIN(tiles_h); WG_PIN(tiles_w); WG_PIN(HR); WG_PIN(HC);
+    WG_PIN(TPIX); WG_PIN(ntaps); WG_PIN(nitems); WG_PIN(ipw); WG_PIN(IW); WG_PIN(PH); WG_PIN(ctiles);
+    WG_PIN(ntiles_total); WG_PIN(tiles_per_slab); WG_PIN(b3); WG_PIN(inv_hc); WG_PIN(tpix8_shift);
+    WG_PIN(G); WG_PIN(img_shift); WG_PIN(HRi); WG_PIN(inv_hri); WG_PIN(tsplit);
+#undef WG_PIN
+    return p;
+}
+
+template <int TPW, int NKT>
+__global__ __launch_bounds__(512) void wgrad_b3_kernel(const WgGroup grp) {
+    extern __shared__ __attribute__((aligned(16))) unsigned char smb[];
+    int j = 0, first = 0;
+#pragma unroll
+    for (int i = 0; i + 1 < WG_MAXJ; ++i) {
+        const int e = grp.block_end[i];
+        if (i + 1 < grp.njobs && (int)blockIdx.x >= e) { j = i + 1; first = e; }
+    }
+    const int l = (int)blockIdx.x - first;
+    const int gx = grp.gx[j], gxy = gx * grp.gy[j];
+    const int bz = l / gxy, rem = l - bz * gxy;
+    const int by = rem / gx, bx = rem - by * gx;
+    const WgTileParams p = wg_job_params(grp.job[j]);
+    if (p.HR * p.HC * 8 <= 4 * 512) wgrad_b3_body<TPW, NKT, 4>(p, bx, by, bz, smb);
+    else wgrad_b3_body<TPW, NKT, 8>(p, bx, by, bz, smb);
 }
 
 struct CwParams {
@@ -745,20 +785,23 @@
     });
 }
 
-template <int TPW, int NKT, int NI>
-static int launch_wgb(const WgTileParams& p, dim3 grid, size_t lds, void* stream, const char* name, const char* who,
-                      double flops, double bytes) {
+template <int TPW, int NKT>
+static int launch_wgb(const WgGroup& grp, size_t lds, void* stream, const char* name, const char* who, double flops, double bytes) {
     static bool attr_set = false;
     if (!attr_set) {
-        (void)hipFuncSetAttribute(reinterpret_cast<const void*>(&wgrad_b3_kernel<TPW, NKT, NI>),
+        (void)hipFuncSetAttribute(reinterpret_cast<const void*>(&wgrad_b3_kernel<TPW, NKT>),
                                   hipFuncAttributeMaxDynamicSharedMemorySize, 160 * 1024);
         attr_set = true;
     }
+    const int blocks = grp.block_end[grp.njobs - 1];
     return dispatch(stream, OpInfo{name, flops, bytes}, [=](hipStream_t s) {
-        wgrad_b3_kernel<TPW, NKT, NI><<<grid, 512, lds, s>>>(p);
+        wgrad_b3_kernel<TPW, NKT><<<blocks, 512, lds, s>>>(grp);
         return launched(who);
     });
 }
+
+typedef int (*WgbLaunchFn)(const WgGroup&, size_t, void*, const char*, const char*, double, double);
+struct WgbInstance { WgbLaunchFn fn; const char* name; };
 
 bool wgrad_tile_plan(const mv3d_conv_geom* g, WgTileParams* out, int* nslab_out, int* cfg_out, size_t* lds_out) {
     if (disabled_paths() & 2) return false;
@@ -846,25 +889,93 @@
     return true;
 }
 
-int wgrad_tile_launch(const mv3d_conv_geom* g, WgTileParams p, int nslab, int cfg, size_t lds, void* stream, const char* who) {
-    const double flops = 2.0 * g->N * g->Ho * g->Wo * g->kh * g->kw * (double)g->C * g->K;
-    const double bytes = 4.0 * ((double)g->N * g->H * g->W * g->C + (double)g->N * g->Ho * g->Wo * g->K + (double)g->kh * g->kw * g->C * g->K);
+static WgbInstance wgb_instance(const WgTileParams& p, int cfg) {
+    if (p.tsplit == 2) {
+        if (cfg == 0) return {launch_wgb<4, 1>, "wgrad_b3<5x5,K32,taps/2>"};
+        if (cfg == 1) return {launch_wgb<4, 2>, "wgrad_b3<5x5,K64,taps/2>"};
+        if (cfg == 2) return {launch_wgb<3, 1>, "wgrad_b3<3x3,K32,taps/2>"};
+        return {launch_wgb<3, 2>, "wgrad_b3<3x3,K64,taps/2>"};
+    }
+    switch (cfg) {
+        case 0: return {launch_wgb<7, 1>, "wgrad_b3<5x5,K32>"};
+        case 1: return {launch_wgb<7, 2>, "wgrad_b3<5x5,K64>"};
+        case 2: return {launch_wgb<5, 1>, "wgrad_b3<3x3,K32>"};
+        default: return {launch_wgb<5, 2>, "wgrad_b3<3x3,K64>"};
+    }
+}
+
+struct WgQueue {
+    WgbInstance inst;
+    WgGroup grp;
+    size_t lds;
+    double flops, bytes;
+    const char* who;
+};
+static thread_local WgQueue* g_wgq = nullptr;
+
+static void wg_add(WgGroup& grp, const WgTileParams& p, dim3 grid) {
+    const int j = grp.njobs++;
+    grp.job[j] = p;
+    grp.gx[j] = (int)grid.x; grp.gy[j] = (int)grid.y;
+    grp.block_end[j] = (j ? grp.block_end[j - 1] : 0) + (int)(grid.x * grid.y * grid.z);
+    for (int i = j + 1; i < WG_MAXJ; ++i) { grp.block_end[i] = grp.block_end[j]; grp.gx[i] = grp.gy[i] = 1; }
+}
+
+static int wgq_flush(void* stream) {
+    WgQueue& q = *g_wgq;
+    if (q.grp.njobs == 0) return MV3D_OK;
+    const int rc = q.inst.fn(q.grp, q.lds, stream, q.inst.name, q.who, q.flops, q.bytes);
+    q.grp.njobs = 0;
+    return rc;
+}
+
+bool wgrad_group_collecting() { return g_wgq != nullptr; }
+int wgrad_group_pending() { return g_wgq ? g_wgq->grp.njobs : 0; }
+int wgrad_group_open() {
+    if (g_wgq) return fail(MV3D_E_INVAL, "mv3d_conv_wgrad_group_begin: a collection is already open on this thread");
+    g_wgq = new WgQueue();
+    return MV3D_OK;
+}
+int wgrad_group_close(void* stream, bool launch) {
+    if (!g_wgq) return MV3D_OK;
+    const int rc = launch ? wgq_flush(stream) : MV3D_OK;
+    delete g_wgq;
+    g_wgq = nullptr;
+    return rc;
+}
+
+static double wg_flops(const mv3d_conv_geom* g) { return 2.0 * g->N * g->Ho * g->Wo * g->kh * g->kw * (double)g->C * g->K; }
+static double wg_bytes(const mv3d_conv_geom* g) {
+    return 4.0 * ((double)g->N * g->H * g->W * g->C + (double)g->N * g->Ho * g->Wo * g->K + (double)g->kh * g->kw * g->C * g->K);
+}
+
+int wgrad_tile_launch(const mv3d_conv_geom* g, WgTileParams p, int nslab, int cfg, size_t lds, void* stream, const char* who, bool own_ws = false) {
+    const double flops = wg_flops(g), bytes = wg_bytes(g);
     const int NKTv = (cfg & 1) ? 2 : 1;
     dim3 grid(p.ctiles * cdiv(g->K, 32 * NKTv), nslab, p.b3 ? p.tsplit : 1);
     if (p.b3) {
-        const bool ni4 = p.HR * p.HC * 8 <= 4 * 512;
-        if (p.tsplit == 2) {
-            if (cfg == 0) return ni4 ? launch_wgb<4, 1, 4>(p, grid, lds, stream, "wgrad_b3<5x5,K32,taps/2>", who, flops, bytes) : launch_wgb<4, 1, 8>(p, grid, lds, stream, "wgrad_b3<5x5,K32,taps/2>", who, flops, bytes);
-            if (cfg == 1) return ni4 ? launch_wgb<4, 2, 4>(p, grid, lds, stream, "wgrad_b3<5x5,K64,taps/2>", who, flops, bytes) : launch_wgb<4, 2, 8>(p, grid, lds, stream, "wgrad_b3<5x5,K64,taps/2>", who, flops, bytes);
-            if (cfg == 2) return ni4 ? launch_wgb<3, 1, 4>(p, grid, lds, stream, "wgrad_b3<3x3,K32,taps/2>", who, flops, bytes) : launch_wgb<3, 1, 8>(p, grid, lds, stream, "wgrad_b3<3x3,K32,taps/2>", who, flops, bytes);
-            return ni4 ? launch_wgb<3, 2, 4>(p, grid, lds, stream, "wgrad_b3<3x3,K64,taps/2>", who, flops, bytes) : launch_wgb<3, 2, 8>(p, grid, lds, stream, "wgrad_b3<3x3,K64,taps/2>", who, flops, bytes);
-        }
-        switch (cfg) {
-            case 0: return ni4 ? launch_wgb<7, 1, 4>(p, grid, lds, stream, "wgrad_b3<5x5,K32>", who, flops, bytes) : launch_wgb<7, 1, 8>(p, grid, lds, stream, "wgrad_b3<5x5,K32>", who, flops, bytes);
-            case 1: return ni4 ? launch_wgb<7, 2, 4>(p, grid, lds, stream, "wgrad_b3<5x5,K64>", who, flops, bytes) : launch_wgb<7, 2, 8>(p, grid, lds, stream, "wgrad_b3<5x5,K64>", who, flops, bytes);
-            case 2: return ni4 ? launch_wgb<5, 1, 4>(p, grid, lds, stream, "wgrad_b3<3x3,K32>", who, flops, bytes) : launch_wgb<5, 1, 8>(p, grid, lds, stream, "wgrad_b3<3x3,K32>", who, flops, bytes);
-            default: return ni4 ? launch_wgb<5, 2, 4>(p, grid, lds, stream, "wgrad_b3<3x3,K64>", who, flops, bytes) : launch_wgb<5, 2, 8>(p, grid, lds, stream, "wgrad_b3<3x3,K64>", who, flops, bytes);
-        }
+        const WgbInstance inst = wgb_instance(p, cfg);
+        if (g_wgq && own_ws) {
+            WgQueue& q = *g_wgq;
+            if (q.grp.njobs > 0 && q.inst.fn != inst.fn) {
+                const int rc = wgq_flush(stream);
+                if (rc != MV3D_OK) { wgrad_group_close(stream, false); return rc; }
+            }
+            for (int i = 0; i < q.grp.njobs; ++i)
+                if (q.grp.job[i].out == p.out) { wgrad_group_close(stream, false); return fail(MV3D_E_INVAL, "%s: a queued filter-gradient job writes the same partial-filter region (one workspace per layer)", who); }
+            if (q.grp.njobs == 0) { q.inst = inst; q.lds = 0; q.flops = q.bytes = 0.0; }
+            wg_add(q.grp, p, grid);
+            q.lds = std::max(q.lds, lds);
+            q.flops += flops; q.bytes += bytes; q.who = who;
+            if (q.grp.njobs == WG_MAXJ) {
+                const int rc = wgq_flush(stream);
+                if (rc != MV3D_OK) { wgrad_group_close(stream, false); return rc; }
+            }
+            return MV3D_OK;
+        }
+        WgGroup one = {};
+        wg_add(one, p, grid);
+        return inst.fn(one, lds, stream, inst.name, who, flops, bytes);
     }
     switch (cfg) {
         case 0: return launch_wgt<7, 1>(p, grid, lds, stream, "wgrad_tile<5x5,K32>", who, flops, bytes);
@@ -880,8 +991,15 @@
     return wgrad_tile_plan(g, &p, &nslab, &cfg, &lds) ? nslab : 0;
 }
 
+int wgrad_group_key(const mv3d_conv_geom* g) {
+    { CwParams cp; if (cwgrad_plan(g, &cp) > 0) return 0; }
+    WgTileParams p; int nslab, cfg; size_t lds;
+    if (!wgrad_tile_plan(g, &p, &nslab, &cfg, &lds) || !p.b3) return 0;
+    return 1 + cfg * 2 + (p.tsplit == 2 ? 1 : 0);
+}
+
 int wgrad_tile_launch_erased(const mv3d_conv_geom* g, const void* img, const void* feat, void* out, void* bias_out, void* stream,
-                             const char* who, int* nslab_out) {
+                             const char* who, int* nslab_out, bool own_ws) {
     {
         CwParams cp;
         const int ns = cwgrad_plan(g, &cp);
@@ -895,7 +1013,7 @@
     if (!wgrad_tile_plan(g, &p, &nslab, &cfg, &lds)) return fail(MV3D_E_INVAL, "%s: tiled wgrad not applicable", who);
     p.img = (const float*)img; p.feat = (const float*)feat; p.out = (float*)out; p.bias_out = (float*)bias_out;
     *nslab_out = nslab;
-    return wgrad_tile_launch(g, p, nslab, cfg, lds, stream, who);
+    return wgrad_tile_launch(g, p, nslab, cfg, lds, stream, who, own_ws);
 }
 
 }
diff --git a/dynamic_multiview_3d_amd/graph.py b/dynamic_multiview_3d_amd/graph.py
--- a/dynamic_multiview_3d_amd/graph.py
+++ b/dynamic_multiview_3d_amd/graph.py
@@ -1,5 +1,6 @@
 import ctypes as C
 import os
+import sys
 import math
 from collections import OrderedDict
 
@@ -512,6 +513,8 @@
         self._finalizing = False
         self._finalized_in_plan = False
         self._part_arena = self._fin_table = None
+        self.wg_group = os.environ.get('MV3D_WG_GROUP', '1') != '0'
+        self._wg_open = False
         self._fused_vars = []
         self.pipeline_fc = os.environ.get('MV3D_PIPELINE_FCADAM', '1') != '0'
         self.pipeline_dp = os.environ.get('MV3D_PIPELINE_DP', '1') != '0'
@@ -876,14 +879,26 @@
             self._fusing = True
             pending = list(self._smooth_deferred)
             try:
+                wg_keys = self._wgrad_group_keys() if self._finalizing else {}
+                wg_key = 0
                 for n in reversed(self.nodes):
+                    key = wg_keys.get(id(n), 0)
+                    if wg_key and key != wg_key:
+                        self._wgrad_group_close()
+                        wg_key = 0
+                    if key and not wg_key:
+                        lib.conv_wgrad_group_begin()
+                        self._wg_open, wg_key = True, key
                     self._backward_node(n, pending)
                     if self._finalizing and isinstance(n, ConvNode) and n.w.has_grad:
                         self._fin_pending += n._part_bytes
                         self._fin_vars += [n.w] + ([n.b] if n.b is not None else [])
                         if self._fin_pending >= self.finalize_chunk_bytes:
+                            self._wgrad_group_close()
+                            wg_key = 0
                             self._finalize_commit()
                             lib.grad_finalize_begin()
+                self._wgrad_group_close()
                 self._smooth_all_placed(pending)
                 for n in self._fused_nodes:
                     n.record_fused_update(self)
@@ -897,10 +912,14 @@
                     self._finalized_in_plan = True
             finally:
                 self._fusing = False
+                self._wg_open = False
                 if self._finalizing:
                     lib.grad_finalize_abort()
                     self._finalizing = False
-                lib.plan_end()
+                if sys.exc_info()[0] is None:
+                    lib.plan_end()
+                else:
+                    lib.raw_plan_end()
             if self._fused_vars:
                 self.plan_bwd_fused = plan
                 self.n_launch_bwd_fused = lib.plan_size(plan)
@@ -928,6 +947,22 @@
                 lib.plan_destroy(plan)
         self.upload_optimizer_state()
         return self
+
+    def _wgrad_group_keys(self):
+        if not self.wg_group:
+            return {}
+        convs = [n for n in reversed(self.nodes) if isinstance(n, ConvNode)]
+        return {id(n): int(self.lib.conv_wgrad_group_key(C.byref(n.geom()))) for n in convs[:-2]}
+
+    def _wgrad_group_close(self):
+        if not self._wg_open:
+            return
+        self._wg_open = False
+        self.begin_side()
+        try:
+            self.lib.conv_wgrad_group_end(self.stream)
+        finally:
+            self.end_side()
 
     def _finalize_commit(self):
         lib = self.lib
diff --git a/include/mv3d_hip.h b/include/mv3d_hip.h
--- a/include/mv3d_hip.h
+++ b/include/mv3d_hip.h
@@ -61,6 +61,9 @@
                         void* workspace, size_t workspace_bytes, void* stream);
 size_t mv3d_conv_workspace_bytes(const mv3d_conv_geom* g);
 size_t mv3d_conv_wgrad_workspace_bytes(const mv3d_conv_geom* g);
+int mv3d_conv_wgrad_group_begin(void);
+int mv3d_conv_wgrad_group_end(void* stream);
+int mv3d_conv_wgrad_group_key(const mv3d_conv_geom* g);
 
 enum { MV3D_FILTER_CONV_FWD = 0, MV3D_FILTER_CONV_DGRAD = 1, MV3D_FILTER_DECONV_FWD = 2, MV3D_FILTER_DECONV_DGRAD = 3 };
 size_t mv3d_filter_prepared_bytes(const mv3d_conv_geom* g, int op);
```

Result: slower. 39640 images/sec (-1.1%).
